# NightShade99/Self-Supervised-Vision

Hardware: AMD Instinct MI355X
Metric: images/sec (whole node) SimCLR ResNet-50 two-view train step (higher is better)
Workload: dtype f32; 1 GPU; SimCLR resnet50 (7x7/2 stem) synthetic 3x224x224, bs=512/GPU, global batch 512, NT-Xent(normalize, T=0.5) over the global batch, SGD-Nesterov; per_gpu_batch=512, global_batch=512, params=27971008, parallelism=single, view_streams=2, library=self-supervised-vision_amd/csrc/libssv_hip.so

## Files before the change

self-supervised-vision_amd/_lib.py:

```python
import ctypes as C
import os

import torch

_HERE = os.path.dirname(os.path.abspath(__file__))
LIB_PATH = os.environ.get("SSV_HIP_LIB") or os.path.join(_HERE, "csrc", "libssv_hip.so")

ABI_VERSION = 124
PROF_CLASSES = ("conv_fwd", "conv_dgrad", "conv_wgrad", "bn_fwd", "bn_bwd", "pool", "loss", "optim", "aug", "misc", "attn", "norm")


class SsvError(RuntimeError):
    pass


ARITH_F32_MFMA, ARITH_BF16X3 = 0, 6
BLUR_MAX_PIXELS, BLUR_MAX_SIGMA = 81920, 1000.0
KMEANS_MAX_K, KMEANS_MAX_D = 4096, 8192
KNN_MAX_K, KNN_MAX_D, KNN_MAX_CLASSES, KNN_MAX_TOPN = 1024, 8192, 4096, 8
NN_LOOKUP_MAX_M, NN_LOOKUP_FUSED_MAX_D, NN_LOOKUP_SLICE, NN_LOOKUP_MAX_SLICES = 8192, 1024, 512, 4096
WHITEN_MAX_D, WHITEN_MAX_W, WMSE_PERM_MAX_N, WMSE_PERM_MAX_VIEWS, WMSE_PERM_MAX_ITERS = 128, 1024, 4096, 8, 16
PROTO_NCE_MAX_M, PROTO_NCE_MAX_SEGS, PROTO_NCE_FUSED_MAX_D, PROTO_NCE_SLICE, PROTO_NCE_MAX_SLICES = 8192, 8, 128, 256, 32
DENSE_MATCH_MAX_S, DENSE_MATCH_MAX_C = 256, 8192
QUEUE_NCE_MAX_M, QUEUE_NCE_FUSED_MAX_D, QUEUE_NCE_SLICE, QUEUE_NCE_MAX_SLICES, QUEUE_NCE_TARGET_WGS = 131072, 128, 256, 32, 256
VICREG_MAX_D = KNN_MAX_D


class ConvDesc(C.Structure):
    _fields_ = [(n, C.c_int32) for n in ("N", "H", "W", "C", "K", "R", "S", "stride", "pad", "Ho", "Wo", "arithmetic", "reserved")] + [("w_planes", C.c_void_p)]


class BnGate(C.Structure):
    _fields_ = [(n, C.c_void_p) for n in ("x", "scale", "shift", "mask", "mean", "invstd", "psum_g", "psum_gx", "x2", "mean2", "invstd2", "psum_gx2")]


class BnDyin(C.Structure):
    _fields_ = [(n, C.c_void_p) for n in ("x", "coef")]


class AugCfg(C.Structure):
    _fields_ = [(n, C.c_double) for n in ("brightness", "contrast", "saturation", "hue", "p_jitter", "p_gray", "p_flip",
                                          "scale_min", "scale_max", "ratio_min", "ratio_max")]


_vp, _i32, _i64, _f32, _sz = C.c_void_p, C.c_int32, C.c_int64, C.c_float, C.c_size_t
_u64 = C.c_uint64
_f3 = C.POINTER(C.c_float)
_cd = C.POINTER(ConvDesc)

SIGNATURES = {
    "ssv_version": (C.c_int, []),
    "ssv_last_error": (C.c_char_p, []),
    "ssv_source_sha16": (C.c_char_p, []),
    "ssv_device_cus": (C.c_int, []),
    "ssv_conv2d_fwd": (C.c_int, [_cd, _vp, _vp, _vp, _vp, _vp, _vp]),
    "ssv_pad_channels": (C.c_int, [_i64, _i32, _i32, _vp, _vp, _i32, _vp]),
    "ssv_group_expand": (C.c_int, [_i32, _i32, _i32, _i32, _i32, _vp, _vp, _vp]),
    "ssv_group_extract": (C.c_int, [_i32, _i32, _i32, _i32, _i32, _vp, _vp, _i32, _vp]),
    "ssv_conv2d_fwd_stats_groups": (_i64, [_cd]),
    "ssv_conv2d_fwd_stats": (C.c_int, [_cd, _vp, _vp, _vp, _vp, _vp, _vp]),
    "ssv_conv2d_fwd_bnrelu_in_stats": (C.c_int, [_cd, _vp, _vp, _vp, _vp, _vp, _vp, _vp, _vp]),
    "ssv_conv2d_fwd_sumin_stats": (C.c_int, [_cd] + [_vp] * 13),
    "ssv_conv2d_wgrad_bnrelu_in": (C.c_int, [_cd, _vp, _vp, _vp, _vp, _vp, C.c_int, _vp, _sz, _vp]),
    "ssv_bn_stats_finalize": (C.c_int, [_i64, _i32, _vp, _vp, _i32, _vp, _vp, _f32, _f32, _vp, _vp, _vp, _vp, _vp, _vp, _vp, _vp, _sz, _vp]),
    "ssv_bn_apply": (C.c_int, [_i64, _i32, _vp, _vp, _vp, _vp, _vp, _vp, C.c_int, _vp, _vp, _vp]),
    "ssv_bn_relu_bwd_affine": (C.c_int, [_i64, _i32, _vp, _vp, _vp, _vp, _vp, _vp, _vp, _vp, _vp, _vp, C.c_int, _vp, _sz, _vp]),
    "ssv_bn_train_fwd_partials": (C.c_int, [_i64, _i32, _vp, _vp, _vp, _i32, _vp, _vp, _vp, C.c_int, _f32, _f32, _vp, _vp, _vp, _vp, _vp, _vp, _vp, _vp, _sz, _vp]),
    "ssv_filter_transpose": (C.c_int, [_i32, _i32, _i32, _i32, _vp, _vp, _vp]),
    "ssv_conv2d_dgrad": (C.c_int, [_cd, _vp, _vp, _vp, _vp, _vp]),
    "ssv_conv2d_fwd_gate_groups": (_i64, [_cd]),
    "ssv_conv2d_fwd_gated": (C.c_int, [_cd, _vp, _vp, _vp, _vp, C.POINTER(BnGate), _vp]),
    "ssv_conv2d_fwd_gated_s2add": (C.c_int, [_cd, _vp, _vp, _vp, _i32, _i32, _vp, C.POINTER(BnGate), _vp]),
    "ssv_conv2d_fwd_dyin_s2add": (C.c_int, [_cd, _vp, C.POINTER(BnDyin), _vp, _vp, _i32, _i32, _vp, C.POINTER(BnGate), _vp]),
    "ssv_conv2d_dgrad_gate_groups": (_i64, [_cd]),
    "ssv_conv2d_dgrad_gated": (C.c_int, [_cd, _vp, _vp, _vp, _vp, C.POINTER(BnGate), _vp]),
    "ssv_bn_bwd_from_partials": (C.c_int, [_i64, _i32, _vp, _vp, _vp, _vp, _vp, _vp, _vp, _i64, _vp, _vp, _vp, C.c_int, _vp, _sz, _vp]),
    "ssv_bn_bwd_coef": (C.c_int, [_i64, _i32, _vp, _vp, _vp, _vp, _vp, _i64, _vp, _vp, _vp, C.c_int, _vp, _sz, _vp]),
    "ssv_conv2d_fwd_dyin": (C.c_int, [_cd, _vp, C.POINTER(BnDyin), _vp, _vp, _vp, C.POINTER(BnGate), _vp]),
    "ssv_conv2d_wgrad_dyin": (C.c_int, [_cd, _vp, _vp, _vp, _vp, C.POINTER(BnDyin), _vp, C.c_int, _vp, _sz, _vp]),
    "ssv_conv2d_wgrad_workspace_bytes": (_sz, [_cd]),
    "ssv_conv2d_fwd_grouped": (C.c_int, [_cd, _i32, _vp, _vp, _vp, _vp, _vp, _vp]),
    "ssv_conv2d_dgrad_grouped": (C.c_int, [_cd, _i32, _vp, _vp, _vp, _vp, _vp]),
    "ssv_conv2d_wgrad_grouped_workspace_bytes": (_sz, [_cd, _i32]),
    "ssv_conv2d_wgrad_grouped": (C.c_int, [_cd, _i32, _vp, _vp, _vp, C.c_int, _vp, _sz, _vp]),
    "ssv_conv2d_wgrad": (C.c_int, [_cd, _vp, _vp, _vp, C.c_int, _vp, _sz, _vp]),
    "ssv_conv2d_wgrad_bias_workspace_bytes": (_sz, [_cd]),
    "ssv_conv2d_wgrad_bias": (C.c_int, [_cd, _vp, _vp, _vp, _vp, C.c_int, _vp, _sz, _vp]),
    "ssv_stem_conv_fwd": (C.c_int, [_cd, _vp, _vp, _vp, _vp, _vp, _vp]),
    "ssv_stem_conv_fwd_stats_rows_per_group": (_i64, [_cd]),
    "ssv_stem_conv_wgrad_rows_per_group": (_i64, [_cd]),
    "ssv_stem_conv_wgrad_workspace_bytes": (_sz, [_cd]),
    "ssv_stem_conv_wgrad": (C.c_int, [_cd, _vp, _vp, _vp, _vp, _sz, _vp]),
    "ssv_wino_tiles": (_i64, [_i32, _i32, _i32]),
    "ssv_wino_groups": (_i64, [_i32, _i32, _i32]),
    "ssv_wino_stats_rows_per_group": (_i32, [_i32, _i32, _i32]),
    "ssv_wino_filter_transform": (C.c_int, [_i32, _i32, _vp, _vp, _vp]),
    "ssv_wino_filter_grad": (C.c_int, [_i32, _i32, _vp, _vp, C.c_int, _vp]),
    "ssv_wino_input_transform": (C.c_int, [_i32, _i32, _i32, _i32, _vp, _vp, _vp, _vp, _vp]),
    "ssv_wino_dy_transform": (C.c_int, [_i32, _i32, _i32, _i32, _vp, _vp, _vp]),
    "ssv_wino_output_transform": (C.c_int, [_i32, _i32, _i32, _i32, _vp, _vp, _vp, _vp, C.POINTER(BnGate), _vp]),
    "ssv_wino44_tiles": (_i64, [_i32, _i32, _i32]),
    "ssv_wino44_groups": (_i64, [_i32, _i32, _i32, _i32]),
    "ssv_wino44_stats_rows_per_group": (_i64, [_i32, _i32, _i32]),
    "ssv_wino44_filter_transform": (C.c_int, [_i32, _i32, _vp, _vp, _vp]),
    "ssv_wino44_input_transform": (C.c_int, [_i32, _i32, _i32, _i32, _vp, _vp, _vp, _vp, _vp, _vp]),
    "ssv_wino44_output_transform": (C.c_int, [_i32, _i32, _i32, _i32, _vp, _vp, _vp, _vp, C.POINTER(BnGate), _vp]),
    "ssv_wino44_dy_transform": (C.c_int, [_i32, _i32, _i32, _i32, _vp, _vp, _vp]),
    "ssv_wino44_filter_grad": (C.c_int, [_i32, _i32, _vp, _vp, C.c_int, _vp]),
    "ssv_wino44_dy_transform_both": (C.c_int, [_i32, _i32, _i32, _i32, _vp, C.POINTER(BnDyin), _vp, _vp, _vp]),
    "ssv_gemm_batched": (C.c_int, [_i32, _i64, _i32, _i32, _vp, _vp, _vp, _vp]),
    "ssv_gemm_batched_split": (C.c_int, [_i32, _i64, _i32, _i32, _vp, _vp, _vp, _vp, _vp, _vp]),
    "ssv_gemm_batched_wgrad_split": (C.c_int, [_i32, _i64, _i32, _i32, _vp, _vp, _vp, _i32, _i32, _vp, _sz, _vp]),
    "ssv_split_planes": (C.c_int, [_i64, _vp, _vp, _vp]),
    "ssv_conv_arithmetic": (C.c_int, [_cd, _i32]),
    "ssv_gemm_batched_wgrad_workspace_bytes": (_sz, [_i32, _i64, _i32, _i32]),
    "ssv_gemm_batched_wgrad": (C.c_int, [_i32, _i64, _i32, _i32, _vp, _vp, _vp, _vp, _sz, _vp]),
    "ssv_gemm_batched_wgrad_blocked_workspace_bytes": (_sz, [_i32, _i64, _i32, _i32, _i32]),
    "ssv_gemm_batched_wgrad_blocked": (C.c_int, [_i32, _i64, _i32, _i32, _vp, _vp, _vp, _i32, _i32, _vp, _sz, _vp]),
    "ssv_bn_workspace_bytes": (_sz, [_i64, _i32]),
    "ssv_bn_train_fwd": (C.c_int, [_i64, _i32, _vp, _vp, _vp, _vp, C.c_int, _f32, _f32, _vp, _vp, _vp, _vp, _vp, _vp, _vp, _vp, _sz, _vp]),
    "ssv_bn_train_bwd": (C.c_int, [_i64, _i32, _vp, _vp, _vp, _vp, _vp, _vp, _vp, C.c_int, _vp, _vp, _vp, _vp, C.c_int, _vp, _sz, _vp]),
    "ssv_bn_relu_maxpool_fwd": (C.c_int, [_i32, _i32, _i32, _i32, _vp, _vp, _vp, _vp, _vp, _vp, _vp]),
    "ssv_bn_relu_maxpool_bwd": (C.c_int, [_i32, _i32, _i32, _i32, _vp, _vp, _vp, _vp, _vp, _vp, _vp, _vp, _vp, _vp, _vp, _vp, C.c_int, _vp, _sz, _vp]),
    "ssv_colsum": (C.c_int, [_i64, _i32, _vp, _vp, C.c_int, _vp, _sz, _vp]),
    "ssv_maxpool3x3s2_fwd": (C.c_int, [_i32, _i32, _i32, _i32, _vp, _vp, _vp, _vp]),
    "ssv_maxpool3x3s2_bwd": (C.c_int, [_i32, _i32, _i32, _i32, _vp, _vp, _vp, _vp]),
    "ssv_gap_fwd": (C.c_int, [_i32, _i32, _i32, _vp, _vp, _vp]),
    "ssv_gap_bwd": (C.c_int, [_i32, _i32, _i32, _vp, _vp, _vp]),
    "ssv_nchw_to_nhwc": (C.c_int, [_i32, _i32, _i32, _i32, _vp, _vp, _vp]),
    "ssv_nhwc_to_nchw": (C.c_int, [_i32, _i32, _i32, _i32, _vp, _vp, _vp]),
    "ssv_l2norm_fwd": (C.c_int, [_i32, _i32, _vp, _i32, _f32, _vp, _i32, _vp, _vp]),
    "ssv_l2norm_bwd": (C.c_int, [_i32, _i32, _vp, _i32, _vp, _vp, _i32, _i32, _vp, _vp]),
    "ssv_ntxent_fwd": (C.c_int, [_i32, _i32, _i32, _i32, _vp, _f32, _vp, _vp, _vp]),
    "ssv_ntxent_loss": (C.c_int, [_i32, _vp, _vp, _f32, _vp, _vp]),
    "ssv_ntxent_bwd": (C.c_int, [_i32, _i32, _i32, _i32, _vp, _vp, _f32, _f32, _vp, _vp]),
    "ssv_ntxent_default_splits": (_i64, [_i32, _i32]),
    "ssv_ntxent_split_workspace_bytes": (_sz, [_i32, _i32, _i32]),
    "ssv_ntxent_fwd_split": (C.c_int, [_i32, _i32, _i32, _i32, _vp, _f32, _vp, _vp, _i32, _vp, _sz, _vp]),
    "ssv_ntxent_bwd_split": (C.c_int, [_i32, _i32, _i32, _i32, _vp, _vp, _f32, _f32, _vp, _i32, _vp, _sz, _vp]),
    "ssv_ntxent_gram_fwd": (C.c_int, [_i32, _i32, _i32, _i32, _vp, _f32, _vp, _vp, _vp]),
    "ssv_ntxent_gram_weights": (C.c_int, [_i32, _i32, _i32, _i32, _vp, _vp, _f32, _f32, _vp]),
    "ssv_reduce_workspace_bytes": (_sz, [_i64]),
    "ssv_mse_pair_fwd_bwd": (C.c_int, [_i64, _vp, _vp, _vp, _vp, _f32, _vp, _vp, _vp, _vp, _sz, _vp]),
    "ssv_scale": (C.c_int, [_i64, _vp, _vp, _vp]),
    "ssv_barlow_cgrad": (C.c_int, [_i32, _vp, _f32, _f32, _vp, _vp, _vp, _sz, _vp]),
    "ssv_vicreg_workspace_bytes": (_sz, [_i32, _i32]),
    "ssv_vicreg_prep": (C.c_int, [_i32, _i32, _vp, _vp, _f32, _f32, _f32, _f32, _vp, _vp, _vp, _vp, _vp, _sz, _vp]),
    "ssv_vicreg_cgrad": (C.c_int, [_i32, _i32, _vp, _f32, _vp, _vp, _vp, _sz, _vp]),
    "ssv_sgd_nesterov": (C.c_int, [_i64, _vp, _vp, _vp, _vp, _f32, _f32, _f32, C.c_int, _vp]),
    "ssv_sgd_nesterov_dev": (C.c_int, [_i64, _vp, _vp, _vp, _vp, _vp, _vp]),
    "ssv_lars_chunk_floats": (_i64, []),
    "ssv_lars_plan_chunks": (_i64, [_i32, _vp]),
    "ssv_lars_plan_bytes": (_sz, [_i32, _vp]),
    "ssv_lars_plan_build": (C.c_int, [_i32, _vp, _vp, _vp, _vp, _vp, _sz]),
    "ssv_lars_workspace_bytes": (_sz, [_i64]),
    "ssv_lars_step": (C.c_int, [_i64, _i32, _i64, _vp, _vp, _vp, _vp, _vp, _vp, _vp, _vp, _sz, _vp]),
    "ssv_ema": (C.c_int, [_i64, _vp, _vp, _f32, _vp]),
    "ssv_fill": (C.c_int, [_i64, _vp, _f32, _vp]),
    "ssv_add": (C.c_int, [_i64, _vp, _vp, _vp]),
    "ssv_augment_params": (C.c_int, [_i32, _i32, _i32, _i32, C.POINTER(AugCfg), _u64, _u64, _vp, _i64, _vp, _vp]),
    "ssv_augment_workspace_bytes": (_sz, [_i32, _i32, _i32, _i32]),
    "ssv_augment_views": (C.c_int, [_i32, _i32, _i32, _i32, _i32, _i32, _vp, _vp, _vp, _f3, _f3, _vp, _vp, _sz, _vp]),
    "ssv_augment_params_blur": (C.c_int, [_i32, _i32, _i32, _i32, C.POINTER(AugCfg), _u64, _u64, _vp, _i64, C.c_double, C.c_double, C.c_double, _vp, _vp]),
    "ssv_augment_blur_workspace_bytes": (_sz, [_i32, _i32, _i32, _i32]),
    "ssv_augment_views_blur": (C.c_int, [_i32, _i32, _i32, _i32, _i32, _i32, _vp, _vp, _vp, _f3, _f3, _vp, _vp, _sz, _vp]),
    "ssv_blur_scalars": (C.c_int, [_i64, _vp, _vp, _vp]),
    "ssv_center_view": (C.c_int, [_i32, _i32, _i32, _i32, _i32, _vp, _vp, _f3, _f3, _vp, _vp]),
    "ssv_knn_workspace_bytes": (_sz, [_i64]),
    "ssv_knn_label_agreement": (C.c_int, [_i64, _i32, _vp, _vp, _i32, _vp, _vp, _sz, _vp]),
    "ssv_knn_workspace_bytes_arith": (_sz, [_i64, _i32, _i32]),
    "ssv_knn_label_agreement_arith": (C.c_int, [_i64, _i32, _vp, _vp, _i32, _vp, _i32, _vp, _sz, _vp]),
    "ssv_kmeans_prep_bytes": (_sz, [_i32, _i32]),
    "ssv_kmeans_workspace_bytes": (_sz, [_i64, _i32, _i32, _i32]),
    "ssv_kmeans_assign": (C.c_int, [_i64, _i32, _i32, _vp, _vp, _vp, _i32, _vp, _vp, _vp, _vp, _i32, _vp, _sz, _vp]),
    "ssv_kmeans_update": (C.c_int, [_i64, _i32, _i32, _vp, _vp, _vp, _vp, _vp, _i32, _vp, _sz, _vp]),
    "ssv_cluster_votes": (C.c_int, [_i64, _vp, _vp, _i32, _i32, _vp, _vp, _vp]),
    "ssv_knn_search_workspace_bytes": (_sz, [_i64, _i64, _i32, _i32, _i32, _i32, _i32]),
    "ssv_knn_search": (C.c_int, [_i64, _i64, _i32, _i32, _vp, _vp, _vp, _vp, _i32, _i32, _i32, _vp, _sz, _vp]),
    "ssv_knn_vote": (C.c_int, [_i64, _i32, _i64, _i32, _i32, _vp, _vp, _vp, _f32, _vp, _vp, _vp, _vp]),
    "ssv_nn_lookup_workspace_bytes": (_sz, [_i32, _i64, _i32, _i32]),
    "ssv_nn_lookup": (C.c_int, [_i32, _i64, _i32, _vp, _vp, _f32, _vp, _vp, _vp, _i32, _vp, _sz, _vp]),
    "ssv_whiten_workspace_bytes": (_sz, [_i32, _i32, _i32]),
    "ssv_whiten_fwd": (C.c_int, [_i32, _i32, _i32, _i64, _vp, _vp, _f32, _vp, _vp, _vp, _vp, _vp, _sz, _vp]),
    "ssv_whiten_bwd": (C.c_int, [_i32, _i32, _i32, _i64, _vp, _vp, _f32, _vp, _vp, _vp, _vp, _vp, _sz, _vp]),
    "ssv_wmse_perm": (C.c_int, [_i32, _i32, _i32, _u64, _u64, _vp, _vp, _vp]),
    "ssv_proto_nce_workspace_bytes": (_sz, [_i32, _i64, _i32, _i32, _i32]),
    "ssv_proto_nce": (C.c_int, [_i32, _i32, _i32, C.POINTER(C.c_int64), _vp, _vp, _vp, _vp, _vp, _vp, _vp, _vp, _i32, _vp, _sz, _vp]),
    "ssv_dense_match": (C.c_int, [_i32, _i32, _i32, _vp, _vp, _f32, _vp, _vp, _i32, _vp]),
    "ssv_queue_nce_workspace_bytes": (_sz, [_i32, _i64, _i32, _i32]),
    "ssv_queue_nce": (C.c_int, [_i32, _i32, _i64, _i64, _vp, _vp, _vp, _vp, _f32, _vp, _vp, _vp, _vp, _i32, _vp, _sz, _vp]),
    "ssv_vit_embed_fwd": (C.c_int, [_i32, _i32, _i32, _i32, _i32, _vp, _vp, _vp, _vp, _vp]),
    "ssv_vit_embed_bwd": (C.c_int, [_i32, _i32, _i32, _i32, _vp, _vp, _vp, _i32, _vp]),
    "ssv_layernorm_fwd": (C.c_int, [_i64, _i32, _vp, _vp, _vp, _vp, _f32, _vp, _vp, _vp, _vp]),
    "ssv_layernorm_workspace_bytes": (_sz, [_i64, _i32]),
    "ssv_layernorm_bwd": (C.c_int, [_i64, _i32, _vp, _vp, _vp, _vp, _vp, _vp, _vp, _vp, _vp, _i32, _vp, _sz, _vp]),
    "ssv_linear_gelu_fwd": (C.c_int, [_cd, _vp, _vp, _vp, _vp, _vp, _vp]),
    "ssv_conv2d_dgrad_gelu": (C.c_int, [_cd, _vp, _vp, _vp, _vp, _vp, _vp]),
    "ssv_linear_fwd_gelugrad": (C.c_int, [_cd, _vp, _vp, _vp, _vp, _vp, _vp]),
    "ssv_linear_gelu_fwd_dact": (C.c_int, [_cd, _vp, _vp, _vp, _vp, _vp, _vp]),
    "ssv_linear_fwd_mulgrad": (C.c_int, [_cd, _vp, _vp, _vp, _vp, _vp, _vp]),
    "ssv_gelu_fwd": (C.c_int, [_i64, _vp, _vp, _vp]),
    "ssv_gelu_bwd": (C.c_int, [_i64, _vp, _vp, _vp, _vp]),
    "ssv_attention_fwd": (C.c_int, [_i32, _i32, _i32, _i32, _vp, _vp, _vp, _i32, _f32, _vp, _i32, _vp, _vp]),
    "ssv_attention_fwd_arith": (C.c_int, [_i32, _i32, _i32, _i32, _vp, _vp, _vp, _i32, _f32, _vp, _i32, _vp, _i32, _vp]),
    "ssv_attention_bwd": (C.c_int, [_i32, _i32, _i32, _i32, _vp, _vp, _vp, _i32, _f32, _vp, _vp, _i32, _vp, _vp, _vp, _vp, _vp, _i32, _vp]),
    "ssv_weightnorm_fwd": (C.c_int, [_i32, _i32, _vp, _vp, _vp, _vp, _vp]),
    "ssv_weightnorm_bwd": (C.c_int, [_i32, _i32, _vp, _vp, _vp, _vp, _vp, _vp, _i32, _vp]),
    "ssv_dino_loss_workspace_bytes": (_sz, [_i32, _i32, _i32]),
    "ssv_dino_loss": (C.c_int, [_i32, _i32, _i32, _vp, _vp, _vp, _f32, _f32, _f32, _vp, _i32, _vp, _vp, _sz, _vp]),
    "ssv_dino_center_update": (C.c_int, [_i32, _i32, _vp, _i32, _vp, _f32, _vp, _vp]),
    "ssv_adamw": (C.c_int, [_i64, _vp, _vp, _vp, _vp, _vp, _f32, _f32, _f32, _f32, _f32, _i64, _f32, _vp]),
    "ssv_adamw_counted": (C.c_int, [_i64, _vp, _vp, _vp, _vp, _vp, _f32, _f32, _f32, _f32, _f32, _vp, _vp, _f32, _vp]),
    "ssv_adamw_counted_dev": (C.c_int, [_i64, _vp, _vp, _vp, _vp, _vp, _f32, _f32, _f32, _vp, _vp, _f32, _vp]),
    "ssv_multicrop_params": (C.c_int, [_i32, _i32, _i32, _i32, _i32, C.c_double, C.c_double, C.c_uint64, C.c_uint64, _vp, _i64, _vp, _vp]),
    "ssv_multicrop": (C.c_int, [_i32, _i32, _i32, _vp, _i32, _vp, _i32, _i32, _vp, _vp]),
    "ssv_negdot_pair_fwd_bwd": (C.c_int, [_i64, _vp, _vp, _vp, _vp, _f32, _vp, _vp, _vp, _vp, _sz, _vp]),
    "ssv_relic_kl_workspace_bytes": (_sz, [_i32]),
    "ssv_relic_kl_fwd_bwd": (C.c_int, [_i32, _i32, _vp, _vp, _vp, _f32, _f32, _vp, _i32, _vp, _vp, _vp, _vp, _sz, _vp]),
    "ssv_moco_loss_fwd_bwd": (C.c_int, [_i32, _i32, _i32, _i32, _vp, _vp, _vp, _f32, _vp, _vp, _vp, _sz, _vp]),
    "ssv_queue_push": (C.c_int, [_i32, _i32, _vp, _i32, _i32, _vp, _f32, _vp]),
    "ssv_queue_push_counted": (C.c_int, [_i32, _i32, _vp, _vp, _i32, _vp, _f32, _vp]),
    "ssv_pirl_default_splits": (_i64, [_i32, _i32]),
    "ssv_pirl_loss_workspace_bytes": (_sz, [_i32, _i32]),
    "ssv_pirl_loss_fwd_bwd": (C.c_int, [_i64, _i32, _i32, _i32, _vp, _vp, _vp, _vp, _vp, _i32, _f32, _f32, _i32, _vp, _vp, _vp, _vp, _sz, _vp]),
    "ssv_bank_momentum_update": (C.c_int, [_i64, _i32, _vp, _i32, _vp, _vp, _f32, _f32, _vp]),
    "ssv_patch_split": (C.c_int, [_i32, _i32, _i32, _i32, _i32, _vp, _vp, _vp]),
    "ssv_softmax_ce_workspace_bytes": (_sz, [_i32]),
    "ssv_softmax_ce_fwd_bwd": (C.c_int, [_i32, _i32, _i32, _vp, _vp, _vp, _vp, _vp, _sz, _vp]),
    "ssv_sgd": (C.c_int, [_i64, _vp, _vp, _vp, _f32, _f32, _f32, C.c_int, C.c_int, _vp]),
    "ssv_prof_enable": (C.c_int, [C.c_int]),
    "ssv_prof_reset": (C.c_int, []),
    "ssv_prof_collect": (C.c_int, [C.POINTER(C.c_double), C.POINTER(C.c_int64)]),
}

_lib = None


def load():
    global _lib
    if _lib is not None:
        return _lib
    if not os.path.exists(LIB_PATH):
        raise SsvError(f"{LIB_PATH} not found: build it with `python -c 'import __graft_entry__ as g; g.build()'` "
                       f"(or `make -C {os.path.dirname(LIB_PATH)}`); there is no CPU fallback")
    lib = C.CDLL(LIB_PATH)
    for name, (res, args) in SIGNATURES.items():
        fn = getattr(lib, name)
        fn.restype, fn.argtypes = res, args
    if lib.ssv_version() < ABI_VERSION:
        raise SsvError(f"{LIB_PATH} is ABI version {lib.ssv_version()}, this package binds version {ABI_VERSION}: rebuild it (make -C {os.path.dirname(LIB_PATH)})")
    _lib = lib
    return lib


def source_sha16():
    return load().ssv_source_sha16().decode()


def lib_sha16(path=None):
    import hashlib
    h = hashlib.sha256()
    with open(path or LIB_PATH, "rb") as fh:
        for chunk in iter(lambda: fh.read(1 << 20), b""):
            h.update(chunk)
    return h.hexdigest()[:16]


def _check(rc, what):
    if rc != 0:
        raise SsvError(f"{what} failed ({rc}): {load().ssv_last_error().decode()}")


def ptr(t):
    return 0 if t is None else t.data_ptr()


_raw_stream = getattr(torch._C, "_cuda_getCurrentRawStream", None)
_raw_device = getattr(torch._C, "_cuda_getDevice", None)


def stream():
    if _raw_stream is not None and _raw_device is not None:
        return _raw_stream(_raw_device())
    return torch.cuda.current_stream().cuda_stream


def _dev(*ts):
    for t in ts:
        if t is not None and not t.is_cuda:
            raise SsvError("libssv_hip operates on device tensors only (got a CPU tensor); there is no CPU fallback")


def call(name, *args):
    _check(getattr(load(), name)(*args), name)


class _Workspace:

    def __init__(self):
        self.buf = {}

    def get(self, nbytes, device):
        key = (device, (_raw_stream(device.index if device.index is not None else _raw_device()) if _raw_stream is not None else torch.cuda.current_stream(device).cuda_stream)
               if device.type == "cuda" else 0)
        b = self.buf.get(key)
        if b is None or b.numel() < nbytes:
            b = torch.empty(max(int(nbytes), 1 << 20), dtype=torch.uint8, device=device)
            self.buf[key] = b
        return b


workspace = _Workspace()


def prof_enable(on=True):
    call("ssv_prof_enable", int(bool(on)))


def prof_reset():
    call("ssv_prof_reset")


def prof_collect():
    ms = (C.c_double * len(PROF_CLASSES))()
    n = (C.c_int64 * len(PROF_CLASSES))()
    call("ssv_prof_collect", ms, n)
    return {k: (ms[i], n[i]) for i, k in enumerate(PROF_CLASSES)}
```

self-supervised-vision_amd/csrc/conv_mfma.hip:

```cpp
#include "common.h"
#include "split_bf16.h"
#include <string.h>
#include <type_traits>

namespace {

constexpr int GBK = 16;

__device__ __forceinline__ int xcd_remap(int orig, int nwg) {
  const int q = nwg >> 3, r = nwg & 7, xcd = orig & 7;
  return (xcd < r ? xcd * (q + 1) : r * (q + 1) + (xcd - r) * q) + (orig >> 3);
}

struct ConvKP {
  int N, H, W, C, K, R, S, stride, pad, Ho, Wo;
  int M;
  int RSC;
  FastDiv dHoWo, dWo, dC, dS, dWp;
  float* aux_out;
  float* aux_out2;
  const float* aux_in;
  const float* xf_scale;
  const float* xf_shift;
  ssv_bn_gate gate;
  const float* dyin_x;
  const float* dyin_coef;
  const float* sum_res; const float* sum_scale; const float* sum_shift; const float* sum_rscale; const float* sum_rshift;
  float* sum_out; uint8_t* sum_mask;
  long long bs_a, bs_b, bs_o;
  int add_H2, add_W2;
  int Cg, Kg;
  const unsigned short* w_planes;
  long long wp_stride;
};

__device__ __forceinline__ void group_span(int n0, int n1, int og, int ig, int bk, int ctot, int& lo, int& hi) {
  const int glo = n0 / og, ghi = (n1 - 1) / og;
  lo = glo * ig / bk * bk;
  hi = min(ctot, ((ghi + 1) * ig + bk - 1) / bk * bk);
}

constexpr int XF_MAXC = 1024;

__device__ __forceinline__ float gelu_f(float v) { return ssv_gelu(v); }
__device__ __forceinline__ float gelu_grad_f(float v) { return ssv_gelu_grad(v); }

using rsrc_t = __amdgpu_buffer_rsrc_t;
constexpr int OOB_OFF = (int)0x80000000u;
__device__ __forceinline__ rsrc_t make_rsrc(const void* base, unsigned bytes) {
  return __builtin_amdgcn_make_buffer_rsrc((void*)base, 0, bytes, 0x00020000);
}
__device__ __forceinline__ f32x4 bload4(rsrc_t rs, int voff_bytes, int soff_bytes) {
  typedef unsigned int u32x4_ __attribute__((ext_vector_type(4)));
  return __builtin_bit_cast(f32x4, (u32x4_)__builtin_amdgcn_raw_buffer_load_b128(rs, voff_bytes, soff_bytes, 0));
}

__device__ __forceinline__ int straddle_off(int off, int bytes, int& rot) {
  rot = 0;
  if (off == OOB_OFF) return OOB_OFF;
  if (off <= -16 || off >= bytes) return OOB_OFF;
  const int c = off < 0 ? 0 : (off > bytes - 16 ? bytes - 16 : off);
  rot = (off - c) >> 2;
  return c;
}
__device__ __forceinline__ f32x4 straddle_fix(f32x4 v, int rot) {
  f32x4 o;
#pragma unroll
  for (int e = 0; e < 4; ++e) {
    const int sidx = e + rot;
    float t = 0.f;
#pragma unroll
    for (int q = 0; q < 4; ++q) t = sidx == q ? v[q] : t;
    o[e] = t;
  }
  return o;
}

template <int TM, int TN, bool A_ROWK, bool B_ROWK, int LDA, int LDB, int BK>
__device__ __forceinline__ void mma_ktile(const float* __restrict__ As, const float* __restrict__ Bs,
                                          int wr0, int wc0, int lane, f32x16 (&acc)[TM][TN]) {
  const int l31 = lane & 31, h = lane >> 5;
#pragma unroll
  for (int ks = 0; ks < BK / 8; ++ks) {
    float a[TM][4], b[TN][4];
#pragma unroll
    for (int tm = 0; tm < TM; ++tm) {
      if constexpr (A_ROWK) {
        const f32x4 v = *reinterpret_cast<const f32x4*>(&As[(wr0 + tm * 32 + l31) * LDA + ks * 8 + 4 * h]);
        a[tm][0] = v[0]; a[tm][1] = v[1]; a[tm][2] = v[2]; a[tm][3] = v[3];
      } else {
#pragma unroll
        for (int t = 0; t < 4; ++t) a[tm][t] = As[(ks * 8 + 4 * h + t) * LDA + wr0 + tm * 32 + l31];
      }
    }
#pragma unroll
    for (int tn = 0; tn < TN; ++tn) {
      if constexpr (B_ROWK) {
        const f32x4 v = *reinterpret_cast<const f32x4*>(&Bs[(wc0 + tn * 32 + l31) * LDB + ks * 8 + 4 * h]);
        b[tn][0] = v[0]; b[tn][1] = v[1]; b[tn][2] = v[2]; b[tn][3] = v[3];
      } else {
#pragma unroll
        for (int t = 0; t < 4; ++t) b[tn][t] = Bs[(ks * 8 + 4 * h + t) * LDB + wc0 + tn * 32 + l31];
      }
    }
#pragma unroll
    for (int t = 0; t < 4; ++t)
#pragma unroll
      for (int tm = 0; tm < TM; ++tm)
#pragma unroll
        for (int tn = 0; tn < TN; ++tn)
          acc[tm][tn] = __builtin_amdgcn_mfma_f32_32x32x2f32(a[tm][t], b[tn][t], acc[tm][tn], 0, 0, 0);
  }
}

template <int TM, int TN>
__device__ __forceinline__ void zero_acc(f32x16 (&acc)[TM][TN]) {
#pragma unroll
  for (int i = 0; i < TM; ++i)
#pragma unroll
    for (int j = 0; j < TN; ++j)
#pragma unroll
      for (int r = 0; r < 16; ++r) acc[i][j][r] = 0.f;
}

template <int TM, int TN> struct Frags { float a[TM][4], b[TN][4]; };

template <int TM, int TN, bool A_ROWK, bool B_ROWK, int LDA, int LDB>
__device__ __forceinline__ void load_frags(Frags<TM, TN>& f, const float* __restrict__ As, const float* __restrict__ Bs,
                                           int wr0, int wc0, int lane, int ks) {
  const int l31 = lane & 31, h = lane >> 5;
#pragma unroll
  for (int tm = 0; tm < TM; ++tm) {
    if constexpr (A_ROWK) {
      const f32x4 v = *reinterpret_cast<const f32x4*>(&As[(wr0 + tm * 32 + l31) * LDA + ks * 8 + 4 * h]);
      f.a[tm][0] = v[0]; f.a[tm][1] = v[1]; f.a[tm][2] = v[2]; f.a[tm][3] = v[3];
    } else {
#pragma unroll
      for (int t = 0; t < 4; ++t) f.a[tm][t] = As[(ks * 8 + 4 * h + t) * LDA + wr0 + tm * 32 + l31];
    }
  }
#pragma unroll
  for (int tn = 0; tn < TN; ++tn) {
    if constexpr (B_ROWK) {
      const f32x4 v = *reinterpret_cast<const f32x4*>(&Bs[(wc0 + tn * 32 + l31) * LDB + ks * 8 + 4 * h]);
      f.b[tn][0] = v[0]; f.b[tn][1] = v[1]; f.b[tn][2] = v[2]; f.b[tn][3] = v[3];
    } else {
#pragma unroll
      for (int t = 0; t < 4; ++t) f.b[tn][t] = Bs[(ks * 8 + 4 * h + t) * LDB + wc0 + tn * 32 + l31];
    }
  }
}

template <int TM, int TN>
__device__ __forceinline__ void mma_frags(const Frags<TM, TN>& f, f32x16 (&acc)[TM][TN]) {
#pragma unroll
  for (int t = 0; t < 4; ++t)
#pragma unroll
    for (int tm = 0; tm < TM; ++tm)
#pragma unroll
      for (int tn = 0; tn < TN; ++tn)
        acc[tm][tn] = __builtin_amdgcn_mfma_f32_32x32x2f32(f.a[tm][t], f.b[tn][t], acc[tm][tn], 0, 0, 0);
}

#define SSV_INTERLEAVE(NMFMA, NMEM, MASK)                                            \
  do {                                                                               \
    _Pragma("unroll") for (int i_ = 0; i_ < (NMEM) && i_ < (NMFMA); ++i_) {         \
      __builtin_amdgcn_sched_group_barrier(0x8, 1, 0);                               \
      __builtin_amdgcn_sched_group_barrier((MASK), 1, 0);                            \
    }                                                                                \
    if ((NMFMA) > (NMEM)) __builtin_amdgcn_sched_group_barrier(0x8, (NMFMA) - (NMEM), 0); \
  } while (0)

struct NoXform { __device__ __forceinline__ void operator()() const {} };
template <int TM, int TN, bool A_ROWK, bool B_ROWK, int LDA, int LDB, int BK, int NLD, int FLUSH = 0, class LoadTile, class StoreTile, class Xform = NoXform>
__device__ __forceinline__ void k_loop(int nkt, const float* As, const float* Bs, int wr0, int wc0, int lane,
                                       f32x16 (&acc)[TM][TN], LoadTile&& load_tile, StoreTile&& store_tile, Xform&& xform_tile = NoXform()) {
  if (nkt <= 0) return;
  f32x16 hi[FLUSH > 0 ? TM : 1][FLUSH > 0 ? TN : 1];
  if constexpr (FLUSH > 0) zero_acc<TM, TN>(hi);
  constexpr int NS = BK / 8;
  constexpr int NM = 4 * TM * TN;
  load_tile();
  xform_tile();
  store_tile();
  __syncthreads();
  Frags<TM, TN> fr;
  for (int kt = 0; kt < nkt; ++kt) {
    __builtin_amdgcn_sched_barrier(0);
    load_frags<TM, TN, A_ROWK, B_ROWK, LDA, LDB>(fr, As, Bs, wr0, wc0, lane, 0);
    load_tile();
    mma_frags<TM, TN>(fr, acc);
    if (NLD > 0) {
      __builtin_amdgcn_sched_group_barrier(0x100, A_ROWK && B_ROWK ? TM + TN : (A_ROWK ? TM + 4 * TN : 4 * (TM + TN)), 0);
      SSV_INTERLEAVE(NM, NLD, 0x20);
    }
    __builtin_amdgcn_sched_barrier(0);
#pragma unroll
    for (int ks = 1; ks < NS; ++ks) {
      load_frags<TM, TN, A_ROWK, B_ROWK, LDA, LDB>(fr, As, Bs, wr0, wc0, lane, ks);
      mma_frags<TM, TN>(fr, acc);
    }
    if constexpr (FLUSH > 0) {
      if ((kt + 1) % FLUSH == 0) {
#pragma unroll
        for (int tm = 0; tm < TM; ++tm)
#pragma unroll
          for (int tn = 0; tn < TN; ++tn) {
            hi[tm][tn] += acc[tm][tn];
#pragma unroll
            for (int j = 0; j < 16; ++j) acc[tm][tn][j] = 0.f;
          }
      }
    }
    __syncthreads();
    if (kt + 1 < nkt) { xform_tile(); store_tile(); __syncthreads(); }
  }
  if constexpr (FLUSH > 0) {
#pragma unroll
    for (int tm = 0; tm < TM; ++tm)
#pragma unroll
      for (int tn = 0; tn < TN; ++tn) acc[tm][tn] = hi[tm][tn] + acc[tm][tn];
  }
}

template <int TM16, int TN16, bool KROWA, bool KROWB, int RBA, int RBB, int FLUSH = 0, int JSPLIT = 1, bool DUAL = false, class LoadTile, class StoreTile, class Xform = NoXform>
__device__ __forceinline__ void k_loop_split(int nkt, const unsigned char* As, int a_plane, const unsigned char* Bs, int b_plane, int wr0, int wc0, int lane,
                                             f32x4 (&acc)[TM16][TN16], LoadTile&& load_tile, StoreTile&& store_tile, Xform&& xform_tile = NoXform()) {
  if (nkt <= 0) return;
  f32x4 hi[FLUSH > 0 ? TM16 : 1][FLUSH > 0 ? TN16 : 1];
  if constexpr (FLUSH > 0) {
#pragma unroll
    for (int i = 0; i < TM16; ++i)
#pragma unroll
      for (int j = 0; j < TN16; ++j) hi[i][j] = f32x4{0.f, 0.f, 0.f, 0.f};
  }
  f32x4 lo[DUAL ? TM16 : 1][DUAL ? TN16 : 1];
  if constexpr (DUAL) {
#pragma unroll
    for (int i = 0; i < TM16; ++i)
#pragma unroll
      for (int j = 0; j < TN16; ++j) lo[i][j] = f32x4{0.f, 0.f, 0.f, 0.f};
  }
  load_tile();
  xform_tile();
  store_tile();
  __syncthreads();
  for (int kt = 0; kt < nkt; ++kt) {
    load_tile();
    constexpr int TJ = TN16 / JSPLIT;
    static_assert(TN16 % JSPLIT == 0, "column tiles per group");
#pragma unroll
    for (int jg = 0; jg < JSPLIT; ++jg) {
      bf16x8 fb[TJ][3];
#pragma unroll
      for (int j = 0; j < TJ; ++j)
#pragma unroll
        for (int q = 0; q < 3; ++q) {
          if constexpr (KROWB) fb[j][q] = splitbf::krow_frag<RBB>(Bs + q * b_plane, wc0 + 16 * (jg * TJ + j), lane);
          else fb[j][q] = splitbf::rowk_frag(Bs + q * b_plane, wc0 + 16 * (jg * TJ + j), lane);
        }
#pragma unroll
      for (int i = 0; i < TM16; ++i) {
        bf16x8 fa[3];
#pragma unroll
        for (int q = 0; q < 3; ++q) {
          if constexpr (KROWA) fa[q] = splitbf::krow_frag<RBA>(As + q * a_plane, wr0 + 16 * i, lane);
          else fa[q] = splitbf::rowk_frag(As + q * a_plane, wr0 + 16 * i, lane);
        }
#pragma unroll
        for (int j = 0; j < TJ; ++j) {
          if constexpr (DUAL) splitbf::mma6x2(acc[i][jg * TJ + j], lo[i][jg * TJ + j], fb[j], fa);
          else splitbf::mma6(acc[i][jg * TJ + j], fb[j], fa);
        }
      }
    }
    if constexpr (FLUSH > 0) {
      if ((kt + 1) % FLUSH == 0) {
#pragma unroll
        for (int i = 0; i < TM16; ++i)
#pragma unroll
          for (int j = 0; j < TN16; ++j) { hi[i][j] += acc[i][j]; acc[i][j] = f32x4{0.f, 0.f, 0.f, 0.f}; }
      }
    }
    __syncthreads();
    if (kt + 1 < nkt) { xform_tile(); store_tile(); __syncthreads(); }
  }
#pragma unroll
  for (int i = 0; i < TM16; ++i)
#pragma unroll
    for (int j = 0; j < TN16; ++j) {
      if constexpr (FLUSH > 0) acc[i][j] = hi[i][j] + acc[i][j];
      if constexpr (DUAL) acc[i][j] += lo[i][j];
    }
}

__device__ __forceinline__ void bstore4(rsrc_t rs, int voff_bytes, f32x4 v) {
  typedef unsigned int u32x4_ __attribute__((ext_vector_type(4)));
  __builtin_amdgcn_raw_buffer_store_b128(__builtin_bit_cast(u32x4_, v), rs, voff_bytes, 0, 0);
}

struct SameOff {};
template <int TM, int TN>
__device__ __forceinline__ void stage_slab(const f32x16 (&acc)[TM][TN], float* __restrict__ ep, int tm, int lane) {
  constexpr int LDE = TN * 32 + 4;
  const int l31 = lane & 31, h = lane >> 5;
#pragma unroll
  for (int tn = 0; tn < TN; ++tn)
#pragma unroll
    for (int j = 0; j < 16; ++j) ep[((j & 3) + 8 * (j >> 2) + 4 * h) * LDE + tn * 32 + l31] = acc[tm][tn][j];
}
template <int TM, int TN>
__device__ __forceinline__ void stage_slab(const f32x4 (&acc)[2 * TM][2 * TN], float* __restrict__ ep, int tm, int lane) {
  constexpr int LDE = TN * 32 + 4;
  const int fr = lane & 15, kg = lane >> 4;
#pragma unroll
  for (int ii = 0; ii < 2; ++ii)
#pragma unroll
    for (int jj = 0; jj < 2 * TN; ++jj) *reinterpret_cast<f32x4*>(&ep[(16 * ii + fr) * LDE + 16 * jj + 4 * kg]) = acc[2 * tm + ii][jj];
}
template <bool SP, class A, class B> __device__ __forceinline__ auto& sel_acc(A& a, B& b) { if constexpr (SP) return b; else return a; }

template <int TM, int TN, int EPI = 0, bool STATS = false, int GATE = 0, class Acc, class RowOff, class AddOff = SameOff>
__device__ __forceinline__ void epilogue_vec(const Acc& acc, float* __restrict__ ep, int lane, int col0, int ncols,
                                             const float* __restrict__ bias, const float* addend, float* out, long long out_elems, RowOff&& row_off,
                                             float* out_act = nullptr, const float* gate = nullptr,
                                             float* pmean = nullptr, float* pm2 = nullptr, int group_rows = 0,
                                             const ssv_bn_gate* bn = nullptr, long long group = 0, AddOff add_off = AddOff(), long long add_elems = 0) {
  constexpr int LDE = TN * 32 + 4, C4 = TN * 8, RPI = 64 / C4, NP = 32 / RPI;
  constexpr bool GMASK = GATE >= 2, GX2 = GATE == 3;
  constexpr int HB0 = GATE == 1 ? 2 : 4;
  constexpr int HB = NP < HB0 ? NP : HB0;
  const int r_in = lane / C4, c4 = lane % C4;
  const int gcol = col0 + c4 * 4;
  const bool cok = gcol < ncols && r_in < RPI;
  const unsigned bytes = (unsigned)(out_elems * 4);
  const rsrc_t r_out = make_rsrc(out, bytes);
  f32x4 b4 = {0.f, 0.f, 0.f, 0.f};
  f32x4 st_p = {0.f, 0.f, 0.f, 0.f}, st_s1 = {0.f, 0.f, 0.f, 0.f}, st_s2 = {0.f, 0.f, 0.f, 0.f};
  f32x4 g_mu = {0.f, 0.f, 0.f, 0.f}, g_is = {0.f, 0.f, 0.f, 0.f}, g_sc = {0.f, 0.f, 0.f, 0.f}, g_sh = {0.f, 0.f, 0.f, 0.f};
  f32x4 g_mu2 = {0.f, 0.f, 0.f, 0.f}, g_is2 = {0.f, 0.f, 0.f, 0.f}, st_s3 = {0.f, 0.f, 0.f, 0.f};
  if constexpr (GATE != 0) {
    if (cok) {
      g_mu = *reinterpret_cast<const f32x4*>(bn->mean + gcol); g_is = *reinterpret_cast<const f32x4*>(bn->invstd + gcol);
      if constexpr (GATE == 1) { g_sc = *reinterpret_cast<const f32x4*>(bn->scale + gcol); g_sh = *reinterpret_cast<const f32x4*>(bn->shift + gcol); }
      if constexpr (GX2) { g_mu2 = *reinterpret_cast<const f32x4*>(bn->mean2 + gcol); g_is2 = *reinterpret_cast<const f32x4*>(bn->invstd2 + gcol); }
    }
  }
  if (bias && cok) b4 = *reinterpret_cast<const f32x4*>(bias + gcol);

  const bool ADD = addend != nullptr;
  auto rows = [&](auto add_tag) {
    constexpr int ADDM = decltype(add_tag)::value;
    constexpr bool ADD_SAME = std::is_same<AddOff, SameOff>::value;
    const rsrc_t r_add = make_rsrc(ADD ? addend : out, ADD_SAME ? bytes : (unsigned)(add_elems * 4));
    const rsrc_t r_gx = make_rsrc(GATE != 0 ? bn->x : out, bytes);
    const rsrc_t r_gm = make_rsrc(GMASK ? reinterpret_cast<const float*>(bn->mask) : out, bytes / 16);
    const rsrc_t r_gx2 = make_rsrc(GX2 ? bn->x2 : out, bytes);
    const rsrc_t r_gate = make_rsrc((EPI == 2 || EPI == 5) ? gate : out, bytes);
    const rsrc_t r_act = make_rsrc((EPI == 1 || EPI == 4) ? out_act : out, bytes);
#pragma unroll
    for (int tm = 0; tm < TM; ++tm) {
      stage_slab<TM, TN>(acc, ep, tm, lane);
      if constexpr (STATS) { if (tm == 0) st_p = *reinterpret_cast<const f32x4*>(&ep[c4 * 4]); }
      constexpr int HP = HB;
      constexpr int NSTEP = NP / HP;
      int voff[1][HP];
      f32x4 av[1][HP], xv[1][HP], gv[1][HP], xv2[1][GX2 ? HP : 1];
      unsigned mb[1][HP];
      auto issue = [&](int st, int sl) {
#pragma unroll
        for (int i = 0; i < HP; ++i) {
          const long long off = row_off(tm * 32 + (st * HP + i) * RPI + r_in);
          voff[sl][i] = (off >= 0 && cok) ? (int)(off + gcol) * 4 : OOB_OFF;
          int aoff = voff[sl][i];
          if constexpr (!ADD_SAME) {
            const long long ao = add_off(tm * 32 + (st * HP + i) * RPI + r_in);
            aoff = (ao >= 0 && voff[sl][i] != OOB_OFF) ? (int)(ao + gcol) * 4 : OOB_OFF;
          }
          if constexpr (ADDM == 2) { if (ADD) av[sl][i] = bload4(r_add, aoff, 0); else av[sl][i] = f32x4{0.f, 0.f, 0.f, 0.f}; }
          else if constexpr (ADDM == 1) av[sl][i] = bload4(r_add, aoff, 0);
          else av[sl][i] = f32x4{0.f, 0.f, 0.f, 0.f};
          if constexpr (EPI == 2 || EPI == 5) gv[sl][i] = bload4(r_gate, voff[sl][i], 0);
          if constexpr (GATE != 0) xv[sl][i] = bload4(r_gx, voff[sl][i], 0);
          if constexpr (GMASK) mb[sl][i] = __builtin_amdgcn_raw_buffer_load_b8(r_gm, voff[sl][i] == OOB_OFF ? OOB_OFF : voff[sl][i] >> 4, 0, 0);
          if constexpr (GX2) xv2[sl][i] = bload4(r_gx2, voff[sl][i], 0);
        }
      };
      auto finish = [&](int st, int sl) {
#pragma unroll
        for (int i = 0; i < HP; ++i) {
          const int r = (st * HP + i) * RPI + r_in;
          f32x4 v = *reinterpret_cast<const f32x4*>(&ep[r * LDE + c4 * 4]);
          const bool ok = voff[sl][i] != OOB_OFF;
          if constexpr (STATS) {
            f32x4 dv = v - st_p;
            dv[0] = ok ? dv[0] : 0.f; dv[1] = ok ? dv[1] : 0.f; dv[2] = ok ? dv[2] : 0.f; dv[3] = ok ? dv[3] : 0.f;
            st_s1 += dv; st_s2 += dv * dv;
          }
          v += b4;
          if constexpr (EPI == 2) {
#pragma unroll
            for (int e = 0; e < 4; ++e) v[e] *= gelu_grad_f(gv[sl][i][e]);
          }
          if constexpr (EPI == 5) v *= gv[sl][i];
          v += av[sl][i];
          if constexpr (GATE != 0) {
            if constexpr (GATE == 1) {
#pragma unroll
              for (int e = 0; e < 4; ++e) v[e] = __builtin_fmaf(xv[sl][i][e], g_sc[e], g_sh[e]) > 0.f ? v[e] : 0.f;
            } else {
#pragma unroll
              for (int e = 0; e < 4; ++e) v[e] = (mb[sl][i] >> e) & 1u ? v[e] : 0.f;
            }
            f32x4 gvv = v;
            if constexpr (GATE == 1) { gvv[0] = ok ? v[0] : 0.f; gvv[1] = ok ? v[1] : 0.f; gvv[2] = ok ? v[2] : 0.f; gvv[3] = ok ? v[3] : 0.f; }
            st_s1 += gvv;
            st_s2 += gvv * ((xv[sl][i] - g_mu) * g_is);
            if constexpr (GX2) st_s3 += gvv * ((xv2[sl][i] - g_mu2) * g_is2);
          }
          if constexpr (EPI == 3) {
#pragma unroll
            for (int e = 0; e < 4; ++e) v[e] = gelu_f(v[e]);
          }
          if constexpr (EPI == 4) {
            f32x4 a;
#pragma unroll
            for (int e = 0; e < 4; ++e) {
              const float cdf = ssv_norm_cdf(v[e]);
              a[e] = 0.5f * v[e] * (2.f * cdf);
              v[e] = cdf + v[e] * ssv_norm_pdf(v[e]);
            }
            bstore4(r_act, voff[sl][i], a);
          }
          bstore4(r_out, voff[sl][i], v);
          if constexpr (EPI == 1) {
            f32x4 a;
#pragma unroll
            for (int e = 0; e < 4; ++e) a[e] = gelu_f(v[e]);
            bstore4(r_act, voff[sl][i], a);
          }
        }
      };
      {
#pragma unroll
        for (int st = 0; st < NSTEP; ++st) {
          __builtin_amdgcn_sched_barrier(0);
          issue(st, 0);
          finish(st, 0);
        }
      }
    }
  };
  if constexpr (GATE != 0 || EPI == 2 || EPI == 5) rows(std::integral_constant<int, 2>{});
  else if (ADD) rows(std::integral_constant<int, 1>{});
  else rows(std::integral_constant<int, 0>{});

  if constexpr (STATS) {
#pragma unroll
    for (int o = C4; o < 64; o <<= 1) {
#pragma unroll
      for (int e = 0; e < 4; ++e) { st_s1[e] += __shfl_xor(st_s1[e], o, 64); st_s2[e] += __shfl_xor(st_s2[e], o, 64); }
    }
    if (r_in == 0 && cok && group_rows > 0) {
      const float n = (float)group_rows;
      *reinterpret_cast<f32x4*>(pmean + gcol) = st_p + st_s1 / n;
      *reinterpret_cast<f32x4*>(pm2 + gcol) = st_s2 - st_s1 * st_s1 / n;
    }
  }
  if constexpr (GATE != 0) {
#pragma unroll
    for (int o = C4; o < 64; o <<= 1) {
#pragma unroll
      for (int e = 0; e < 4; ++e) {
        st_s1[e] += __shfl_xor(st_s1[e], o, 64); st_s2[e] += __shfl_xor(st_s2[e], o, 64);
        if constexpr (GX2) st_s3[e] += __shfl_xor(st_s3[e], o, 64);
      }
    }
    if (r_in == 0 && cok) {
      *reinterpret_cast<f32x4*>(bn->psum_g + group * ncols + gcol) = st_s1;
      *reinterpret_cast<f32x4*>(bn->psum_gx + group * ncols + gcol) = st_s2;
      if constexpr (GX2) *reinterpret_cast<f32x4*>(bn->psum_gx2 + group * ncols + gcol) = st_s3;
    }
  }
}

template <int BM, int BN, int WGM, int WGN, int BK, bool VEC, int EPI = 0, bool STATS = false, int C4 = 0, bool XF = false, int GATE = 0, int OPM = 0, bool ADDS2 = false, int SP = 0>
__global__ void __launch_bounds__(256, (SP ? (OPM != 0 || GATE == 3 || (SP == 2 && BN == 128))
                                          : (OPM == 2 || GATE == 3 || (OPM == 1 && !(BM == 128 && BN == 128)))) ? 2 : 3)
conv_fwd_k(ConvKP p, const float* __restrict__ x, const float* __restrict__ w, const float* __restrict__ bias,
           const float* addend, float* y) {
  constexpr int TM = BM / WGM / 32, TN = BN / WGN / 32;
  constexpr int LDT = BK + 4;
  constexpr int STAGE = (BM + BN) * LDT;
  static_assert(!XF || (VEC && C4 == 0), "the fused-input variant is the float4 path");
  constexpr bool DYF = OPM == 1, SUM = OPM == 2;
  static_assert(OPM == 0 || (VEC && C4 == 0 && !XF), "the formed-on-load operands are the float4 path");
  constexpr int EP_FLOATS = 4 * 32 * (TN * 32 + 4);
  static_assert(!SP || (VEC && C4 == 0 && BK == 32), "the bf16-piece variants are the float4 path with K-step 32");
  constexpr int SP_FLOATS = (BM + BN) * 48;
  constexpr int SMEM = SP ? (SP_FLOATS > EP_FLOATS ? SP_FLOATS : EP_FLOATS)
                          : ((VEC && (EPI || STATS || GATE != 0 || OPM != 0) && EP_FLOATS > STAGE) ? EP_FLOATS : STAGE);
  __shared__ __attribute__((aligned(16))) float smem[SMEM];
  __shared__ __attribute__((aligned(16))) float xfs[(XF && !SP) ? 2 * XF_MAXC : 4];
  float* As = smem;
  float* Bs = smem + BM * LDT;
  const int tid = threadIdx.x, lane = tid & 63, wave = tid >> 6;
  const int wr0 = (wave / WGN) * (BM / WGM), wc0 = (wave % WGN) * (BN / WGN);
  const int NT = (p.K + BN - 1) / BN;
  const int bid = xcd_remap(blockIdx.x, gridDim.x);
  const int mt = bid / NT, nt = bid - mt * NT;
  const int m0 = mt * BM, n0 = nt * BN;
  x += (size_t)blockIdx.y * p.bs_a; w += (size_t)blockIdx.y * p.bs_b; y += (size_t)blockIdx.y * p.bs_o;
  if (addend) addend += (size_t)blockIdx.y * p.bs_o;

  f32x16 acc[SP ? 1 : TM][SP ? 1 : TN];
  f32x4 acc16[SP ? 2 * TM : 1][SP ? 2 * TN : 1];
  if constexpr (SP) {
#pragma unroll
    for (int i = 0; i < 2 * TM; ++i)
#pragma unroll
      for (int j = 0; j < 2 * TN; ++j) acc16[i][j] = f32x4{0.f, 0.f, 0.f, 0.f};
  } else zero_acc<SP ? 1 : TM, SP ? 1 : TN>(acc);

  if constexpr (VEC && C4 == 2) {
    static_assert(BK == 24 && BM == 256, "one staged output row per thread, six float4 per row");
    constexpr int CHN = BK / 4;
    constexpr int BF = (BN * CHN + 255) / 256;
    const rsrc_t rx = make_rsrc(x, (unsigned)p.N * p.H * p.W * 12u);
    const rsrc_t rw = make_rsrc(w, (unsigned)p.K * p.R * BK * 4u);
    int hi0, rowbase;
    unsigned wmask = 0;
    {
      const int m = m0 + tid;
      const bool ok = m < p.M;
      const uint32_t mm = ok ? (uint32_t)m : 0u;
      const uint32_t n = fdiv(mm, p.dHoWo);
      const uint32_t rem = mm - n * (uint32_t)(p.Ho * p.Wo);
      const uint32_t ho = fdiv(rem, p.dWo);
      const uint32_t wo = rem - ho * (uint32_t)p.Wo;
      hi0 = ok ? (int)ho * p.stride - p.pad : -(1 << 20);
      const int wi0 = (int)wo * p.stride - p.pad;
      rowbase = ok ? (((int)n * p.H + hi0) * p.W + wi0) * 12 : 0;
#pragma unroll
      for (int px = 0; px < 8; ++px) wmask |= (unsigned)((px < p.S) & ((unsigned)(wi0 + px) < (unsigned)p.W)) << px;
    }
    int boff[BF];
#pragma unroll
    for (int i = 0; i < BF; ++i) {
      const int f = tid + 256 * i, kf = f / CHN, ch = f - kf * CHN;
      boff[i] = (f < BN * CHN && n0 + kf < p.K) ? ((n0 + kf) * p.R * BK + ch * 4) * 4 : OOB_OFF;
    }
    int lr = 0;
    f32x4 ra[CHN], rb[BF];
    const int xbytes = p.N * p.H * p.W * 12;
    int rots = 0;
    auto load_tile = [&]() {
      const bool hv = (unsigned)(hi0 + lr) < (unsigned)p.H;
      const int base = rowbase + lr * p.W * 12;
      rots = 0;
#pragma unroll
      for (int j = 0; j < CHN; ++j) {
        int rot;
        ra[j] = bload4(rx, straddle_off((hv && lr < p.R) ? base + j * 16 : OOB_OFF, xbytes, rot), 0);
        rots |= (rot != 0 ? rot + 8 : 0) << (4 * j);
      }
#pragma unroll
      for (int i = 0; i < BF; ++i) rb[i] = bload4(rw, (lr < p.R) ? boff[i] : OOB_OFF, lr * BK * 4);
      lr += 1;
    };
    auto xform_tile = [&]() {
      if (rots != 0) {
#pragma unroll
        for (int j = 0; j < CHN; ++j) { const int q = (rots >> (4 * j)) & 15; if (q) ra[j] = straddle_fix(ra[j], q - 8); }
      }
#pragma unroll
      for (int j = 0; j < CHN; ++j)
#pragma unroll
        for (int e = 0; e < 4; ++e) ra[j][e] = ((wmask >> ((4 * j + e) / 3)) & 1u) ? ra[j][e] : 0.f;
    };
    auto store_tile = [&]() {
#pragma unroll
      for (int j = 0; j < CHN; ++j) *reinterpret_cast<f32x4*>(&As[tid * LDT + 4 * j]) = ra[j];
#pragma unroll
      for (int i = 0; i < BF; ++i) {
        const int f = tid + 256 * i, kf = f / CHN, ch = f - kf * CHN;
        if (f < BN * CHN) *reinterpret_cast<f32x4*>(&Bs[kf * LDT + ch * 4]) = rb[i];
      }
    };
    k_loop<TM, TN, true, true, LDT, LDT, BK, CHN + BF>(p.R, As, Bs, wr0, wc0, lane, acc, load_tile, store_tile, xform_tile);
  } else if constexpr (VEC && C4 == 1) {
    constexpr int CH = BK / 4, RPP = 256 / CH;
    constexpr int AP = BM / RPP, BP = BN / RPP;
    const int tl = tid % CH, rsub = tid / CH;
    const rsrc_t rx = make_rsrc(x, (unsigned)p.N * p.H * p.W * 16u);
    const rsrc_t rw = make_rsrc(w, (unsigned)p.K * p.RSC * 4u);
    int hi0[AP], wi0[AP], aoff[AP];
#pragma unroll
    for (int i = 0; i < AP; ++i) {
      const int m = m0 + rsub + RPP * i;
      const bool ok = m < p.M;
      const uint32_t mm = ok ? (uint32_t)m : 0u;
      const uint32_t n = fdiv(mm, p.dHoWo);
      const uint32_t rem = mm - n * (uint32_t)(p.Ho * p.Wo);
      const uint32_t ho = fdiv(rem, p.dWo);
      const uint32_t wo = rem - ho * (uint32_t)p.Wo;
      hi0[i] = ok ? (int)ho * p.stride - p.pad : -(1 << 20);
      wi0[i] = (int)wo * p.stride - p.pad;
      aoff[i] = (((int)n * p.H + hi0[i]) * p.W + wi0[i]) * 16;
    }
    int boff[BP];
#pragma unroll
    for (int i = 0; i < BP; ++i) {
      const int ko = n0 + rsub + RPP * i;
      boff[i] = ko < p.K ? ko * p.RSC * 4 : OOB_OFF;
    }
    const int ntap = p.R * p.S;
    int lt = tl;
    f32x4 ra[AP], rb[BP];
    auto load_tile = [&]() {
      const bool tv = lt < ntap;
      const int r = (int)fdiv((uint32_t)(tv ? lt : 0), p.dS);
      const int sx = (tv ? lt : 0) - r * p.S;
      const int toff_x = (r * p.W + sx) * 16, toff_w = lt * 16;
#pragma unroll
      for (int i = 0; i < AP; ++i) {
        const bool ok = tv & ((unsigned)(hi0[i] + r) < (unsigned)p.H) & ((unsigned)(wi0[i] + sx) < (unsigned)p.W);
        ra[i] = bload4(rx, ok ? aoff[i] + toff_x : OOB_OFF, 0);
      }
#pragma unroll
      for (int i = 0; i < BP; ++i) rb[i] = bload4(rw, (tv && boff[i] != OOB_OFF) ? boff[i] + toff_w : OOB_OFF, 0);
      lt += CH;
    };
    auto store_tile = [&]() {
#pragma unroll
      for (int i = 0; i < AP; ++i) *reinterpret_cast<f32x4*>(&As[(rsub + RPP * i) * LDT + tl * 4]) = ra[i];
#pragma unroll
      for (int i = 0; i < BP; ++i) *reinterpret_cast<f32x4*>(&Bs[(rsub + RPP * i) * LDT + tl * 4]) = rb[i];
    };
    k_loop<TM, TN, true, true, LDT, LDT, BK, AP + BP>((ntap + CH - 1) / CH, As, Bs, wr0, wc0, lane, acc, load_tile, store_tile);
  } else if constexpr (VEC) {
    constexpr int CH = BK / 4, RPP = 256 / CH;
    constexpr int AP = BM / RPP, BP = BN / RPP;
    const int chunk = (tid % CH) * 4, rsub = tid / CH;
    const rsrc_t rx = make_rsrc(x, (unsigned)p.N * p.H * p.W * p.C * 4u);
    const rsrc_t rw = make_rsrc(w, (unsigned)p.K * p.RSC * 4u);
    int hi0[AP], wi0[AP], aoff[AP];
#pragma unroll
    for (int i = 0; i < AP; ++i) {
      const int m = m0 + rsub + RPP * i;
      const bool ok = m < p.M;
      const uint32_t mm = ok ? (uint32_t)m : 0u;
      const uint32_t n = fdiv(mm, p.dHoWo);
      const uint32_t rem = mm - n * (uint32_t)(p.Ho * p.Wo);
      const uint32_t ho = fdiv(rem, p.dWo);
      const uint32_t wo = rem - ho * (uint32_t)p.Wo;
      hi0[i] = ok ? (int)ho * p.stride - p.pad : -(1 << 20);
      wi0[i] = (int)wo * p.stride - p.pad;
      aoff[i] = ((((int)n * p.H + hi0[i]) * p.W + wi0[i]) * p.C + chunk) * 4;
      if (!ok) aoff[i] = OOB_OFF;
    }
    int boff[BP];
#pragma unroll
    for (int i = 0; i < BP; ++i) {
      const int ko = n0 + rsub + RPP * i;
      boff[i] = ko < p.K ? (ko * p.RSC + chunk) * 4 : OOB_OFF;
    }
    const bool inb = p.pad == 0 && p.R == 1 && p.S == 1;
    int lr = 0, ls = 0, lc0 = 0;
    int ktiles = p.RSC / BK;
    if constexpr (!XF && OPM == 0) {
      if (p.Kg != 0) {
        int c_hi;
        group_span(n0, min(n0 + BN, p.K), p.Kg, p.Cg, BK, p.C, lc0, c_hi);
        ktiles = p.R * p.S * ((c_hi - lc0) / BK);
      }
    }
    f32x4 ra[AP], rb[SP ? 1 : BP];
    f32x4 ra2[OPM ? AP : 1], co[(OPM || (XF && SP)) ? 4 : 1];
    constexpr int BPP = SP ? (BN * 4 + 255) / 256 : 1;
    u32x4 rbp[SP ? 3 : 1][BPP];
    int boffp[BPP], bldsp[BPP];
    const long long wplane = p.wp_stride;
    const rsrc_t rwp = make_rsrc(SP ? (const void*)(p.w_planes + (size_t)blockIdx.y * p.bs_b) : (const void*)w, SP ? (unsigned)((2 * wplane + (long long)p.K * p.RSC) * 2) : 16u);
    if constexpr (SP) {
#pragma unroll
      for (int i = 0; i < BPP; ++i) {
        const int idx = tid + 256 * i, br = idx >> 2, k8 = idx & 3;
        boffp[i] = (idx < BN * 4 && n0 + br < p.K) ? ((n0 + br) * p.RSC + k8 * 8) * 2 : OOB_OFF;
        bldsp[i] = splitbf::rowk_off(br, k8);
      }
    }
    const rsrc_t rxs0 = make_rsrc((XF && SP) ? p.xf_scale : x, (XF && SP) ? (unsigned)p.C * 4u : 16u), rxs1 = make_rsrc((XF && SP) ? p.xf_shift : x, (XF && SP) ? (unsigned)p.C * 4u : 16u);
    const rsrc_t rx2 = make_rsrc(DYF ? p.dyin_x : (SUM ? p.sum_res : x), (unsigned)p.N * p.H * p.W * p.C * 4u);
    const rsrc_t rco = make_rsrc(DYF ? p.dyin_coef : x, DYF ? (unsigned)p.C * 16u : 16u);
    const rsrc_t rs0 = make_rsrc(SUM ? p.sum_scale : x, (unsigned)p.C * 4u), rs1 = make_rsrc(SUM ? p.sum_shift : x, (unsigned)p.C * 4u);
    const bool raff = SUM && p.sum_rscale != nullptr;
    const rsrc_t rs2 = make_rsrc(raff ? p.sum_rscale : x, (unsigned)p.C * 4u), rs3 = make_rsrc(raff ? p.sum_rshift : x, (unsigned)p.C * 4u);
    const rsrc_t rso = make_rsrc(SUM ? p.sum_out : y, (unsigned)p.N * p.H * p.W * p.C * 4u);
    const rsrc_t rsm = make_rsrc(SUM && p.sum_mask ? reinterpret_cast<float*>(p.sum_mask) : y, (unsigned)p.N * p.H * p.W * (p.C / 4));
    int st_off = 0;
    int xf_ok = 0, xf_c = 0;
    if constexpr (XF && !SP) {
      for (int c = tid; c < p.C; c += 256) { xfs[c] = p.xf_scale[c]; xfs[XF_MAXC + c] = p.xf_shift[c]; }
      __syncthreads();
    }
    auto load_tile = [&]() {
      const int toff_x = ((lr * p.W + ls) * p.C + lc0) * 4;
      const int toff_w = ((lr * p.S + ls) * p.C + lc0) * 4;
      if constexpr (XF) { xf_ok = 0; xf_c = lc0 + chunk; }
      if constexpr (XF && SP) { co[0] = bload4(rxs0, chunk * 4, lc0 * 4); co[1] = bload4(rxs1, chunk * 4, lc0 * 4); }
#pragma unroll
      for (int i = 0; i < AP; ++i) {
        const bool ok = inb | (((unsigned)(hi0[i] + lr) < (unsigned)p.H) & ((unsigned)(wi0[i] + ls) < (unsigned)p.W));
        ra[i] = bload4(rx, ok ? aoff[i] + toff_x : OOB_OFF, 0);
        if constexpr (OPM != 0) ra2[i] = bload4(rx2, ok ? aoff[i] + toff_x : OOB_OFF, 0);
        if constexpr (XF) xf_ok |= (int)ok << i;
      }
      if constexpr (DYF) {
#pragma unroll
        for (int j = 0; j < 4; ++j) co[j] = bload4(rco, (j * p.C + chunk) * 4, lc0 * 4);
      }
      if constexpr (SUM) {
        st_off = toff_x;
        co[0] = bload4(rs0, chunk * 4, lc0 * 4); co[1] = bload4(rs1, chunk * 4, lc0 * 4);
        if (raff) { co[2] = bload4(rs2, chunk * 4, lc0 * 4); co[3] = bload4(rs3, chunk * 4, lc0 * 4); }
        else { co[2] = f32x4{1.f, 1.f, 1.f, 1.f}; co[3] = f32x4{0.f, 0.f, 0.f, 0.f}; }
      }
      if constexpr (SP) {
#pragma unroll
        for (int q = 0; q < 3; ++q)
#pragma unroll
          for (int i = 0; i < BPP; ++i)
            rbp[q][i] = (u32x4)__builtin_amdgcn_raw_buffer_load_b128(rwp, boffp[i] == OOB_OFF ? OOB_OFF : boffp[i] + q * (int)(wplane * 2), toff_w >> 1, 0);
      } else {
#pragma unroll
        for (int i = 0; i < BP; ++i) rb[i] = bload4(rw, boff[i], toff_w);
      }
      ls += 1;
      const bool w1 = ls == p.S;
      ls = w1 ? 0 : ls;
      lr += w1 ? 1 : 0;
      const bool w2 = lr == p.R;
      lr = w2 ? 0 : lr;
      lc0 += w2 ? BK : 0;
    };
    auto xform_tile = [&]() {
      if constexpr (XF) {
        f32x4 sc, sh;
        if constexpr (SP) { sc = co[0]; sh = co[1]; }
        else { sc = *reinterpret_cast<const f32x4*>(&xfs[xf_c]); sh = *reinterpret_cast<const f32x4*>(&xfs[XF_MAXC + xf_c]); }
#pragma unroll
        for (int i = 0; i < AP; ++i) {
          const float cap = (inb || ((xf_ok >> i) & 1)) ? __builtin_inff() : 0.f;
#pragma unroll
          for (int e = 0; e < 4; ++e) ra[i][e] = __builtin_amdgcn_fmed3f(__builtin_fmaf(ra[i][e], sc[e], sh[e]), 0.f, cap);
        }
      } else if constexpr (DYF) {
#pragma unroll
        for (int i = 0; i < AP; ++i) {
#pragma unroll
          for (int e = 0; e < 4; ++e) ra[i][e] = __builtin_fmaf(ra[i][e], co[0][e], __builtin_fmaf(ra2[i][e] - co[1][e], co[2][e], co[3][e]));
        }
      } else if constexpr (SUM) {
        const bool wr = nt == 0;
#pragma unroll
        for (int i = 0; i < AP; ++i) {
          f32x4 v;
          unsigned bits = 0;
#pragma unroll
          for (int e = 0; e < 4; ++e) {
            v[e] = __builtin_fmaf(ra[i][e], co[0][e], co[1][e]) + __builtin_fmaf(ra2[i][e], co[2][e], co[3][e]);
            bits |= (v[e] > 0.f ? 1u : 0u) << e;
            v[e] = fmaxf(v[e], 0.f);
          }
          ra[i] = v;
          if (wr) {
            const int off = aoff[i] == OOB_OFF ? OOB_OFF : aoff[i] + st_off;
            bstore4(rso, off, v);
            if (p.sum_mask) __builtin_amdgcn_raw_buffer_store_b8((unsigned char)bits, rsm, off == OOB_OFF ? OOB_OFF : off >> 4, 0, 0);
          }
        }
      }
    };
    constexpr int A_PLANE = BM * splitbf::ROWB, B_PLANE = BN * splitbf::ROWB;
    unsigned char* const Asb = reinterpret_cast<unsigned char*>(smem);
    unsigned char* const Bsb = Asb + 3 * A_PLANE;
    auto store_tile = [&]() {
      if constexpr (SP) {
#pragma unroll
        for (int i = 0; i < AP; ++i) splitbf::rowk_store(Asb, A_PLANE, rsub + RPP * i, tid % CH, ra[i]);
#pragma unroll
        for (int q = 0; q < 3; ++q)
#pragma unroll
          for (int i = 0; i < BPP; ++i)
            if (BN * 4 % 256 == 0 || tid + 256 * i < BN * 4) *reinterpret_cast<u32x4*>(Bsb + q * B_PLANE + bldsp[i]) = rbp[q][i];
        return;
      }
#pragma unroll
      for (int i = 0; i < AP; ++i) *reinterpret_cast<f32x4*>(&As[(rsub + RPP * i) * LDT + chunk]) = ra[i];
#pragma unroll
      for (int i = 0; i < BP; ++i) *reinterpret_cast<f32x4*>(&Bs[(rsub + RPP * i) * LDT + chunk]) = rb[i];
    };
    if constexpr (SP) k_loop_split<2 * TM, 2 * TN, false, false, 128, 128, 0, 1, SP == 2>(ktiles, Asb, A_PLANE, Bsb, B_PLANE, wr0, wc0, lane, acc16, load_tile, store_tile, xform_tile);
    else k_loop<TM, TN, true, true, LDT, LDT, BK, AP + BP + (OPM ? AP + 4 : 0)>(ktiles, As, Bs, wr0, wc0, lane, acc, load_tile, store_tile, xform_tile);
  } else {
    static_assert(BK == GBK, "generic path is BK=16");
    constexpr int AE = BM / 16, BE = BN / 16;
    const int kk = tid & 15, rsub = tid >> 4;
    int hw0[AE];
    int nimg[AE];
#pragma unroll
    for (int i = 0; i < AE; ++i) {
      const int m = m0 + rsub + 16 * i;
      if (m < p.M) {
        const uint32_t n = fdiv((uint32_t)m, p.dHoWo);
        const uint32_t rem = (uint32_t)m - n * (uint32_t)(p.Ho * p.Wo);
        const uint32_t ho = fdiv(rem, p.dWo);
        const uint32_t wo = rem - ho * (uint32_t)p.Wo;
        const int h0 = (int)ho * p.stride - p.pad, w0 = (int)wo * p.stride - p.pad;
        hw0[i] = (h0 & 0xffff) | (w0 << 16);
        nimg[i] = (int)n;
      } else { hw0[i] = 0; nimg[i] = -1; }
    }
    float ra[AE], rb[BE];
    int lk = kk;
    auto load_tile = [&]() {
      const bool kok = lk < p.RSC;
      const uint32_t tap = fdiv((uint32_t)(kok ? lk : 0), p.dC);
      const int c = (kok ? lk : 0) - (int)tap * p.C;
      const uint32_t r = fdiv(tap, p.dS);
      const int s = (int)tap - (int)r * p.S;
#pragma unroll
      for (int i = 0; i < AE; ++i) {
        const int hi = (int)(short)(hw0[i] & 0xffff) + (int)r, wi = (hw0[i] >> 16) + s;
        float v = 0.f;
        if (kok && nimg[i] >= 0 && (unsigned)hi < (unsigned)p.H && (unsigned)wi < (unsigned)p.W)
          v = x[(((size_t)nimg[i] * p.H + hi) * p.W + wi) * p.C + c];
        ra[i] = v;
      }
#pragma unroll
      for (int i = 0; i < BE; ++i) {
        const int ko = n0 + rsub + 16 * i;
        rb[i] = (kok && ko < p.K) ? w[(size_t)ko * p.RSC + lk] : 0.f;
      }
      lk += BK;
    };
    auto store_tile = [&]() {
#pragma unroll
      for (int i = 0; i < AE; ++i) As[(rsub + 16 * i) * LDT + kk] = ra[i];
#pragma unroll
      for (int i = 0; i < BE; ++i) Bs[(rsub + 16 * i) * LDT + kk] = rb[i];
    };
    const int nkt = (p.RSC + BK - 1) / BK;
    load_tile();
    store_tile();
    __syncthreads();
    for (int kt = 0; kt < nkt; ++kt) {
      const bool more = kt + 1 < nkt;
      if (more) load_tile();
      mma_ktile<TM, TN, true, true, LDT, LDT, BK>(As, Bs, wr0, wc0, lane, acc);
      __syncthreads();
      if (more) { store_tile(); __syncthreads(); }
    }
  }

  static_assert(!(EPI || STATS) || (VEC && EP_FLOATS <= SMEM), "the fused-activation / statistics forward needs the vectorised epilogue");
  if constexpr (VEC && EP_FLOATS <= SMEM) {
    if ((p.K & 3) == 0) {
      const int rbase = m0 + wr0;
      if constexpr (STATS) {
        constexpr int GR = TM * 32;
        const int g = rbase / GR;
        const int valid = min(GR, p.M - rbase);
        epilogue_vec<TM, TN, 0, true>(sel_acc<(SP != 0)>(acc, acc16), smem + wave * (32 * (TN * 32 + 4)), lane, n0 + wc0, p.K, bias, addend, y, (long long)p.M * p.K,
                                          [&](int r) -> long long { const int m = rbase + r; return m < p.M ? (long long)m * p.K : -1; },
                                          nullptr, nullptr, p.aux_out + (size_t)g * p.K, p.aux_out2 + (size_t)g * p.K, valid > 0 ? valid : 0);
      } else if constexpr (GATE != 0) {
        static_assert(BM / WGM == 64, "gate partials are per 64 output rows");
        auto row_off = [&](int r) -> long long { const int m = rbase + r; return m < p.M ? (long long)m * p.K : -1; };
        if constexpr (ADDS2) {
          static_assert(GATE != 0, "the compact stride-2 addend rides on the gated epilogues");
          auto add_off = [&](int r) -> long long {
            const int m = rbase + r;
            if (m >= p.M) return -1;
            const uint32_t n = fdiv((uint32_t)m, p.dHoWo);
            const uint32_t rem = (uint32_t)m - n * (uint32_t)(p.Ho * p.Wo);
            const uint32_t ho = fdiv(rem, p.dWo);
            const uint32_t wo = rem - ho * (uint32_t)p.Wo;
            if ((ho | wo) & 1u) return -1;
            return ((long long)((int)n * p.add_H2 + (int)(ho >> 1)) * p.add_W2 + (int)(wo >> 1)) * p.K;
          };
          epilogue_vec<TM, TN, 0, false, GATE>(sel_acc<(SP != 0)>(acc, acc16), smem + wave * (32 * (TN * 32 + 4)), lane, n0 + wc0, p.K, bias, addend, y, (long long)p.M * p.K, row_off,
                                                   nullptr, nullptr, nullptr, nullptr, 0, &p.gate, (long long)(rbase / 64), add_off,
                                                   (long long)p.N * p.add_H2 * p.add_W2 * p.K);
        } else {
          epilogue_vec<TM, TN, 0, false, GATE>(sel_acc<(SP != 0)>(acc, acc16), smem + wave * (32 * (TN * 32 + 4)), lane, n0 + wc0, p.K, bias, addend, y, (long long)p.M * p.K, row_off,
                                                   nullptr, nullptr, nullptr, nullptr, 0, &p.gate, (long long)(rbase / 64));
        }
      } else {
        epilogue_vec<TM, TN, EPI>(sel_acc<(SP != 0)>(acc, acc16), smem + wave * (32 * (TN * 32 + 4)), lane, n0 + wc0, p.K, bias, addend, y, (long long)p.M * p.K,
                                  [&](int r) -> long long { const int m = rbase + r; return m < p.M ? (long long)m * p.K : -1; },
                                  (EPI == 1 || EPI == 4) ? p.aux_out : nullptr, (EPI == 2 || EPI == 5) ? p.aux_in : nullptr);
      }
      return;
    }
  }
  static_assert(GATE == 0 || (VEC && EP_FLOATS <= SMEM), "the gated epilogue is the vectorised one");
  if constexpr (SP) return;
  const int l31 = lane & 31, h = lane >> 5;
#pragma unroll
  for (int tn = 0; tn < TN; ++tn) {
    const int col = n0 + wc0 + tn * 32 + l31;
    if (col >= p.K) continue;
    const float bv = bias ? bias[col] : 0.f;
#pragma unroll
    for (int tm = 0; tm < TM; ++tm) {
#pragma unroll
      for (int j = 0; j < 16; ++j) {
        const int row = m0 + wr0 + tm * 32 + (j & 3) + 8 * (j >> 2) + 4 * h;
        if (row < p.M) {
          const size_t o = (size_t)row * p.K + col;
          float v = acc[tm][tn][j] + bv;
          if (addend) v += addend[o];
          y[o] = v;
        }
      }
    }
  }
}

template <int BM, int BN, int WGM, int WGN, int BK, bool EPI = false, int GATE = 0, bool SP = false>
__global__ void __launch_bounds__(256, SP ? 2 : 3)
conv_dgrad_k(ConvKP p, const float* __restrict__ dy, const float* __restrict__ w, const float* addend, float* dx) {
  constexpr int TM = BM / WGM / 32, TN = BN / WGN / 32;
  constexpr int LDT = BK + 4;
  static_assert(!SP || (BK == 32 && BN == 128), "the bf16-piece data gradient: K-step 32, 128 input channels per tile");
  constexpr int A_FLOATS = BM * LDT, B_FLOATS = BK * BN, STAGE = SP ? 48 * (BM + BN) : A_FLOATS + B_FLOATS;
  __shared__ __attribute__((aligned(16))) float smem[STAGE];
  __shared__ unsigned rowpix[BM];
  __shared__ int taps[64 * 3];
  __shared__ int ntaps_s;
  float* As = smem;
  float* Bs = smem + A_FLOATS;
  const int tid = threadIdx.x, lane = tid & 63, wave = tid >> 6;
  const int wr0 = (wave / WGN) * (BM / WGM), wc0 = (wave % WGN) * (BN / WGN);
  const int st = p.stride;
  const int ph = blockIdx.y / st, pw = blockIdx.y - ph * st;
  const int Hq = ph < p.H ? (p.H - ph + st - 1) / st : 0;
  const int Wq = pw < p.W ? (p.W - pw + st - 1) / st : 0;
  const int Mc = p.N * Hq * Wq;
  const int NT = (p.C + BN - 1) / BN;
  const int bid = xcd_remap(blockIdx.x, gridDim.x);
  const int mt = bid / NT, nt = bid - mt * NT;
  const int m0 = mt * BM, n0 = nt * BN;
  if (m0 >= Mc) {
    if constexpr (GATE != 0) {
      const long long grp = ((long long)blockIdx.y * (gridDim.x / NT) + mt) * (BM / 64) + (wr0 / 64);
      const int col = n0 + wc0 + lane;
      for (int c = col; c < min(n0 + wc0 + BN / WGN, p.C); c += 64) { p.gate.psum_g[grp * p.C + c] = 0.f; p.gate.psum_gx[grp * p.C + c] = 0.f; }
    }
    return;
  }

  if (tid == 0) {
    int n = 0;
    for (int r = 0; r < p.R; ++r) {
      const int dr = ph + p.pad - r;
      if (((dr % st) + st) % st != 0) continue;
      for (int s = 0; s < p.S; ++s) {
        const int ds = pw + p.pad - s;
        if (((ds % st) + st) % st != 0) continue;
        taps[3 * n + 0] = dr >= 0 ? dr / st : -((-dr) / st);
        taps[3 * n + 1] = ds >= 0 ? ds / st : -((-ds) / st);
        taps[3 * n + 2] = (r * p.S + s) * p.C;
        ++n;
      }
    }
    ntaps_s = n;
  }
  for (int r = tid; r < BM; r += 256) {
    const int m = m0 + r;
    unsigned pix = 0xffffffffu;
    if (m < Mc) {
      const int n = m / (Hq * Wq);
      const int rem = m - n * Hq * Wq;
      const int hq = rem / Wq, wq = rem - hq * Wq;
      pix = (unsigned)((n * p.H + hq * st + ph) * p.W + wq * st + pw);
    }
    rowpix[r] = pix;
  }
  __syncthreads();
  const int ntaps = ntaps_s;

  f32x16 acc[SP ? 1 : TM][SP ? 1 : TN];
  f32x4 acc16[SP ? 2 * TM : 1][SP ? 2 * TN : 1];
  if constexpr (SP) {
#pragma unroll
    for (int i = 0; i < 2 * TM; ++i)
#pragma unroll
      for (int j = 0; j < 2 * TN; ++j) acc16[i][j] = f32x4{0.f, 0.f, 0.f, 0.f};
  } else zero_acc<SP ? 1 : TM, SP ? 1 : TN>(acc);

  constexpr int CH = BK / 4, RPP = 256 / CH;
  constexpr int AP = BM / RPP;
  constexpr int BCV = BN / 4;
  constexpr int BRP = 256 / BCV;
  constexpr int BP = BK / BRP;
  const int chunk = (tid % CH) * 4, rsub = tid / CH;
  const rsrc_t rdy = make_rsrc(dy, (unsigned)p.N * p.Ho * p.Wo * p.K * 4u);
  const rsrc_t rw = make_rsrc(w, (unsigned)p.K * p.RSC * 4u);
  int hq_[AP], wq_[AP], aoff[AP];
#pragma unroll
  for (int i = 0; i < AP; ++i) {
    const int m = m0 + rsub + RPP * i;
    const bool ok = m < Mc;
    const int mm = ok ? m : 0;
    const int n = mm / (Hq * Wq);
    const int rem = mm - n * Hq * Wq;
    hq_[i] = ok ? rem / Wq : -(1 << 20);
    wq_[i] = rem - (rem / Wq) * Wq;
    aoff[i] = ok ? (((n * p.Ho + hq_[i]) * p.Wo + wq_[i]) * p.K + chunk) * 4 : OOB_OFF;
  }
  const int bcol = (tid % BCV) * 4, brow = tid / BCV;
  const int boff = n0 + bcol < p.C ? (brow * p.RSC + n0 + bcol) * 4 : OOB_OFF;
  const bool inb = p.pad == 0 && p.R == 1 && p.S == 1;

  int ti = 0, lk0 = 0;
  int kspan = p.K;
  if (p.Cg != 0) {
    int k_hi;
    group_span(n0, min(n0 + BN, p.C), p.Cg, p.Kg, BK, p.K, lk0, k_hi);
    kspan = k_hi - lk0;
  }
  int dho = 0, dwo = 0, tapoff = 0;
  if (ntaps > 0) { dho = taps[0]; dwo = taps[1]; tapoff = taps[2]; }
  f32x4 ra[AP], rb[SP ? 1 : BP];
  constexpr int BPP = SP ? 32 * (BN / 8) / 256 : 1;
  u32x4 rbp[SP ? 3 : 1][BPP];
  int boffp[BPP], bldsp[BPP];
  const rsrc_t rwp = make_rsrc(SP ? (const void*)p.w_planes : (const void*)w, SP ? (unsigned)(3 * p.wp_stride * 2) : 16u);
  if constexpr (SP) {
#pragma unroll
    for (int i = 0; i < BPP; ++i) {
      const int idx = tid + 256 * i, kr = idx / (BN / 8), c8 = idx % (BN / 8);
      boffp[i] = n0 + c8 * 8 < p.C ? (kr * p.RSC + n0 + c8 * 8) * 2 : OOB_OFF;
      bldsp[i] = splitbf::krow_off<BN * 2>(kr, c8);
    }
  }
  auto load_tile = [&]() {
    const int toff_a = ((dho * p.Wo + dwo) * p.K + lk0) * 4;
    const int toff_b = (lk0 * p.RSC + tapoff) * 4;
#pragma unroll
    for (int i = 0; i < AP; ++i) {
      const bool ok = inb | (((unsigned)(hq_[i] + dho) < (unsigned)p.Ho) & ((unsigned)(wq_[i] + dwo) < (unsigned)p.Wo));
      ra[i] = bload4(rdy, ok ? aoff[i] + toff_a : OOB_OFF, 0);
    }
    if constexpr (SP) {
#pragma unroll
      for (int q = 0; q < 3; ++q)
#pragma unroll
        for (int i = 0; i < BPP; ++i)
          rbp[q][i] = (u32x4)__builtin_amdgcn_raw_buffer_load_b128(rwp, boffp[i] == OOB_OFF ? OOB_OFF : boffp[i] + q * (int)(p.wp_stride * 2), toff_b >> 1, 0);
    } else {
#pragma unroll
      for (int i = 0; i < BP; ++i) rb[i] = bload4(rw, boff + BRP * i * p.RSC * 4, toff_b);
    }
    ti += 1;
    const bool w1 = ti >= ntaps;
    ti = w1 ? 0 : ti;
    lk0 += w1 ? BK : 0;
    dho = taps[3 * ti]; dwo = taps[3 * ti + 1]; tapoff = taps[3 * ti + 2];
  };
  constexpr int A_PLANE = BM * splitbf::ROWB, B_PLANE = 32 * BN * 2;
  unsigned char* const Asb = reinterpret_cast<unsigned char*>(smem);
  unsigned char* const Bsb = Asb + 3 * A_PLANE;
  auto store_tile = [&]() {
    if constexpr (SP) {
#pragma unroll
      for (int i = 0; i < AP; ++i) splitbf::rowk_store(Asb, A_PLANE, rsub + RPP * i, tid % CH, ra[i]);
#pragma unroll
      for (int q = 0; q < 3; ++q)
#pragma unroll
        for (int i = 0; i < BPP; ++i) *reinterpret_cast<u32x4*>(Bsb + q * B_PLANE + bldsp[i]) = rbp[q][i];
      return;
    }
#pragma unroll
    for (int i = 0; i < AP; ++i) *reinterpret_cast<f32x4*>(&As[(rsub + RPP * i) * LDT + chunk]) = ra[i];
#pragma unroll
    for (int i = 0; i < BP; ++i) *reinterpret_cast<f32x4*>(&Bs[(brow + BRP * i) * BN + bcol]) = rb[i];
  };
  if constexpr (SP) k_loop_split<2 * TM, 2 * TN, false, true, 128, BN * 2>(ntaps * (kspan / BK), Asb, A_PLANE, Bsb, B_PLANE, wr0, wc0, lane, acc16, load_tile, store_tile);
  else k_loop<TM, TN, true, false, LDT, BN, BK, AP + BP>(ntaps * (kspan / BK), As, Bs, wr0, wc0, lane, acc, load_tile, store_tile);

  constexpr int EP_FLOATS = 4 * 32 * (TN * 32 + 4);
  static_assert(!EPI || EP_FLOATS <= STAGE, "the fused-activation dgrad needs the vectorised epilogue");
  static_assert(GATE == 0 || (EP_FLOATS <= STAGE && BM / WGM == 64), "the gated epilogue is the vectorised one, partials per 64 rows");
  if constexpr (EP_FLOATS <= STAGE) {
    if constexpr (GATE != 0) {
      const long long grp = ((long long)blockIdx.y * (gridDim.x / NT) + mt) * (BM / 64) + (wr0 / 64);
      epilogue_vec<TM, TN, 0, false, GATE>(sel_acc<SP>(acc, acc16), smem + wave * (32 * (TN * 32 + 4)), lane, n0 + wc0, p.C, nullptr, addend, dx, (long long)p.N * p.H * p.W * p.C,
                                               [&](int r) -> long long { const unsigned pix = rowpix[wr0 + r]; return pix != 0xffffffffu ? (long long)pix * p.C : -1; },
                                               nullptr, nullptr, nullptr, nullptr, 0, &p.gate, grp);
    } else {
      epilogue_vec<TM, TN, EPI ? 2 : 0>(sel_acc<SP>(acc, acc16), smem + wave * (32 * (TN * 32 + 4)), lane, n0 + wc0, p.C, nullptr, addend, dx, (long long)p.N * p.H * p.W * p.C,
                                        [&](int r) -> long long { const unsigned pix = rowpix[wr0 + r]; return pix != 0xffffffffu ? (long long)pix * p.C : -1; },
                                        nullptr, EPI ? p.aux_in : nullptr);
    }
    return;
  }
  if constexpr (SP) return;
  const int l31 = lane & 31, h = lane >> 5;
#pragma unroll
  for (int tn = 0; tn < TN; ++tn) {
    const int col = n0 + wc0 + tn * 32 + l31;
    if (col >= p.C) continue;
#pragma unroll
    for (int tm = 0; tm < TM; ++tm) {
#pragma unroll
      for (int j = 0; j < 16; ++j) {
        const unsigned pix = rowpix[wr0 + tm * 32 + (j & 3) + 8 * (j >> 2) + 4 * h];
        if (pix != 0xffffffffu) {
          const size_t o = (size_t)pix * p.C + col;
          float v = acc[tm][tn][j];
          if (addend) v += addend[o];
          dx[o] = v;
        }
      }
    }
  }
}

template <int BM, int BN, int WGM, int WGN, int BK, bool VECB, int GATHER, bool XF = false, bool DYF = false, bool BIAS = false, int FLUSH = 0, bool SP = false>
__global__ void __launch_bounds__(256, (SP && BM == 128 && BN == 128) ? 2 : 1)
conv_wgrad_k(ConvKP p, const float* __restrict__ x, const float* __restrict__ dy, float* __restrict__ partial, int chunk_rows, int tiles) {
  constexpr int TM = BM / WGM / 32, TN = BN / WGN / 32;
  static_assert(!SP || (VECB && GATHER != 3 && BK == 32), "the bf16-piece variants: float4 gathers, K-step 32");
  constexpr int STAGE = SP ? 48 * (BM + BN) : BK * (BM + BN);
  constexpr int EP_FLOATS = 4 * 32 * (TN * 32 + 4);
  static_assert(!XF || VECB, "the fused-input variant is the float4 path");
  static_assert(!DYF || (VECB && GATHER == 1), "the BatchNorm-backward operand: 1x1 / stride 1 layers");
  __shared__ __attribute__((aligned(16))) float smem[STAGE > EP_FLOATS ? STAGE : EP_FLOATS];
  float* As = smem;
  float* Bs = smem + BK * BM;
  const int tid = threadIdx.x, lane = tid & 63, wave = tid >> 6;
  const int wr0 = (wave / WGN) * (BM / WGM), wc0 = (wave % WGN) * (BN / WGN);
  const int NCOL = GATHER == 3 ? p.R * 24 : p.RSC;
  const int JT = (NCOL + BN - 1) / BN;
  const int bid = xcd_remap(blockIdx.x, gridDim.x);
  const int split = bid / tiles, tile = bid - split * tiles;
  const int it = tile / JT, jt = tile - it * JT;
  const int i0 = it * BM, j0 = jt * BN;
  const int ms = split * chunk_rows;
  const int me = min(ms + chunk_rows, p.M);
  x += (size_t)blockIdx.y * p.bs_a; dy += (size_t)blockIdx.y * p.bs_b; partial += (size_t)blockIdx.y * p.bs_o;
  if constexpr (GATHER != 3) {
    if (p.Kg != 0 && j0 / p.C == (min(j0 + BN, NCOL) - 1) / p.C) {
      const int c0 = j0 % p.C, c1 = c0 + min(BN, NCOL - j0);
      if ((min(i0 + BM, p.K) - 1) / p.Kg < c0 / p.Cg || (c1 - 1) / p.Cg < i0 / p.Kg) return;
    }
  }

  f32x16 acc[SP ? 1 : TM][SP ? 1 : TN];
  f32x4 acc16[SP ? 2 * TM : 1][SP ? 2 * TN : 1];
  if constexpr (SP) {
#pragma unroll
    for (int i = 0; i < 2 * TM; ++i)
#pragma unroll
      for (int j = 0; j < 2 * TN; ++j) acc16[i][j] = f32x4{0.f, 0.f, 0.f, 0.f};
  } else zero_acc<SP ? 1 : TM, SP ? 1 : TN>(acc);

  constexpr int ACV = BM / 4, ARP = 256 / ACV, AP = BK / ARP;
  const int acol = (tid % ACV) * 4, arow = tid / ACV;
  const bool acok = i0 + acol < p.K;
  constexpr int BCV = VECB ? BN / 4 : BN, BRP = GATHER == 3 ? 1 : 256 / BCV, BP = GATHER == 3 ? (BK * BCV + 255) / 256 : BK / BRP;
  const int bcol = VECB ? (tid % BCV) * 4 : (tid % BCV), brow = tid / BCV;
  const int j = j0 + bcol;
  const bool jok = j < p.RSC;
  const uint32_t tap = fdiv((uint32_t)(jok ? j : 0), p.dC);
  const int cj = (jok ? j : 0) - (int)tap * p.C;
  const int rj = (int)fdiv(tap, p.dS);
  const int sj = (int)tap - rj * p.S;

  const rsrc_t rdy = make_rsrc(dy, (unsigned)p.M * p.K * 4u);
  const rsrc_t rx = make_rsrc(x, (unsigned)p.N * p.H * p.W * p.C * 4u);
  int mcur = ms;
  f32x4 ra[AP];
  f32x4 bsum = {0.f, 0.f, 0.f, 0.f};
  f32x4 rbv[VECB ? BP : 1];
  float rbs[VECB ? 1 : BP];
  int avoff[AP], bvoff[BP];
  f32x4 ra2[DYF ? AP : 1], dco[DYF ? 4 : 1];
  const rsrc_t rdx = make_rsrc(DYF ? p.dyin_x : dy, (unsigned)p.M * p.K * 4u);
  int a_ok = 0;
  if constexpr (DYF) {
#pragma unroll
    for (int j = 0; j < 4; ++j) dco[j] = acok ? *reinterpret_cast<const f32x4*>(p.dyin_coef + (size_t)j * p.K + i0 + acol) : f32x4{0.f, 0.f, 0.f, 0.f};
  }
  int xf_ok = 0;
  f32x4 xsc = {0.f, 0.f, 0.f, 0.f}, xsh = {0.f, 0.f, 0.f, 0.f};
  if constexpr (XF) { if (jok) { xsc = *reinterpret_cast<const f32x4*>(p.xf_scale + cj); xsh = *reinterpret_cast<const f32x4*>(p.xf_shift + cj); } }
#pragma unroll
  for (int i = 0; i < AP; ++i) avoff[i] = acok ? ((arow + ARP * i) * p.K + i0 + acol) * 4 : OOB_OFF;
#pragma unroll
  for (int i = 0; i < BP; ++i) bvoff[i] = jok ? ((brow + BRP * i) * p.C + cj) * 4 : OOB_OFF;
  int s1_ho[BP], s1_wo[BP], s1_base[BP];
  const int s1_qw = BK / p.Wo, s1_rw = BK - s1_qw * p.Wo;
  if constexpr (GATHER == 2) {
#pragma unroll
    for (int i = 0; i < BP; ++i) {
      const uint32_t mm = (uint32_t)min(ms + brow + BRP * i, p.M - 1);
      const uint32_t n = fdiv(mm, p.dHoWo);
      const uint32_t rem = mm - n * (uint32_t)(p.Ho * p.Wo);
      s1_ho[i] = (int)fdiv(rem, p.dWo);
      s1_wo[i] = (int)rem - s1_ho[i] * p.Wo;
      s1_base[i] = ((brow + BRP * i + (rj - p.pad) * p.W + (sj - p.pad)) * p.C + cj) * 4;
    }
  }
  int rw_row[GATHER == 3 ? BP : 1], rw_r[GATHER == 3 ? BP : 1], rw_e0[GATHER == 3 ? BP : 1];
  unsigned rw_mask[GATHER == 3 ? BP : 1];
  int rw_rot[GATHER == 3 ? BP : 1];
  if constexpr (GATHER == 3) {
#pragma unroll
    for (int i = 0; i < BP; ++i) {
      const int f = tid + 256 * i, col = j0 + (f % BCV) * 4;
      rw_row[i] = f / BCV;
      rw_r[i] = col / 24;
      rw_e0[i] = col - rw_r[i] * 24;
      if (f >= BK * BCV || col >= NCOL) rw_r[i] = -1;
      rw_mask[i] = 0;
      rw_rot[i] = 0;
    }
  }
  auto load_tile = [&]() {
    const int soff_a = mcur * p.K * 4;
#pragma unroll
    for (int i = 0; i < AP; ++i) ra[i] = bload4(rdy, avoff[i], soff_a);
    if constexpr (GATHER == 3) {
#pragma unroll
      for (int i = 0; i < BP; ++i) {
        const int m = mcur + rw_row[i];
        bool ok = rw_r[i] >= 0 && m < p.M;
        const uint32_t mm = ok ? (uint32_t)m : 0u;
        const uint32_t n = fdiv(mm, p.dHoWo);
        const uint32_t rem = mm - n * (uint32_t)(p.Ho * p.Wo);
        const uint32_t ho = fdiv(rem, p.dWo);
        const uint32_t wo = rem - ho * (uint32_t)p.Wo;
        const int hi = (int)ho * p.stride - p.pad + rw_r[i], wi0 = (int)wo * p.stride - p.pad;
        ok = ok & ((unsigned)hi < (unsigned)p.H);
        int rot;
        rbv[i] = bload4(rx, straddle_off(ok ? (((int)n * p.H + hi) * p.W + wi0) * 12 + rw_e0[i] * 4 : OOB_OFF, p.N * p.H * p.W * 12, rot), 0);
        rw_rot[i] = rot;
        unsigned mk = 0;
#pragma unroll
        for (int e = 0; e < 4; ++e) { const int px = (rw_e0[i] + e) / 3; mk |= (unsigned)((px < p.S) & ((unsigned)(wi0 + px) < (unsigned)p.W)) << e; }
        rw_mask[i] = mk;
      }
      mcur += BK;
      return;
    }
    if constexpr (DYF) {
      a_ok = 0;
#pragma unroll
      for (int i = 0; i < AP; ++i) { ra2[i] = bload4(rdx, avoff[i], soff_a); a_ok |= (int)(mcur + arow + ARP * i < p.M) << i; }
    }
    if constexpr (GATHER == 1) {
      const int soff_b = mcur * p.C * 4;
#pragma unroll
      for (int i = 0; i < BP; ++i) {
        if constexpr (VECB) rbv[i] = bload4(rx, bvoff[i], soff_b);
        else rbs[i] = __builtin_bit_cast(float, __builtin_amdgcn_raw_buffer_load_b32(rx, bvoff[i], soff_b, 0));
      }
    } else if constexpr (GATHER == 2) {
      const int moff = mcur * p.C * 4;
      if constexpr (XF) xf_ok = 0;
#pragma unroll
      for (int i = 0; i < BP; ++i) {
        const int m = mcur + brow + BRP * i;
        const bool ok = jok & (m < p.M) & ((unsigned)(s1_ho[i] + rj - p.pad) < (unsigned)p.H) & ((unsigned)(s1_wo[i] + sj - p.pad) < (unsigned)p.W);
        if constexpr (XF) xf_ok |= (int)ok << i;
        const int off = ok ? s1_base[i] + moff : OOB_OFF;
        if constexpr (VECB) rbv[i] = bload4(rx, off, 0);
        else rbs[i] = __builtin_bit_cast(float, __builtin_amdgcn_raw_buffer_load_b32(rx, off, 0, 0));
        int wo = s1_wo[i] + s1_rw;
        const int carry = wo >= p.Wo ? 1 : 0;
        wo -= carry ? p.Wo : 0;
        int ho = s1_ho[i] + s1_qw + carry;
        ho -= ho >= p.Ho ? p.Ho : 0;
        s1_wo[i] = wo; s1_ho[i] = ho;
      }
    } else {
      if constexpr (XF) xf_ok = 0;
#pragma unroll
      for (int i = 0; i < BP; ++i) {
        const int m = mcur + brow + BRP * i;
        bool ok = jok & (m < p.M);
        const uint32_t mm = ok ? (uint32_t)m : 0u;
        const uint32_t n = fdiv(mm, p.dHoWo);
        const uint32_t rem = mm - n * (uint32_t)(p.Ho * p.Wo);
        const uint32_t ho = fdiv(rem, p.dWo);
        const uint32_t wo = rem - ho * (uint32_t)p.Wo;
        const int hi = (int)ho * p.stride - p.pad + rj, wi = (int)wo * p.stride - p.pad + sj;
        ok = ok & ((unsigned)hi < (unsigned)p.H) & ((unsigned)wi < (unsigned)p.W);
        if constexpr (XF) xf_ok |= (int)ok << i;
        const int off = ok ? ((((int)n * p.H + hi) * p.W + wi) * p.C + cj) * 4 : OOB_OFF;
        if constexpr (VECB) rbv[i] = bload4(rx, off, 0);
        else rbs[i] = __builtin_bit_cast(float, __builtin_amdgcn_raw_buffer_load_b32(rx, off, 0, 0));
      }
    }
    mcur += BK;
  };
  auto xform_tile = [&]() {
    if constexpr (GATHER == 3) {
#pragma unroll
      for (int i = 0; i < BP; ++i) {
        if (rw_rot[i] != 0) rbv[i] = straddle_fix(rbv[i], rw_rot[i]);
#pragma unroll
        for (int e = 0; e < 4; ++e) rbv[i][e] = ((rw_mask[i] >> e) & 1u) ? rbv[i][e] : 0.f;
      }
    }
    if constexpr (DYF) {
#pragma unroll
      for (int i = 0; i < AP; ++i) {
        const bool ok = (a_ok >> i) & 1;
#pragma unroll
        for (int e = 0; e < 4; ++e) ra[i][e] = ok ? __builtin_fmaf(ra[i][e], dco[0][e], __builtin_fmaf(ra2[i][e] - dco[1][e], dco[2][e], dco[3][e])) : 0.f;
      }
    }
    if constexpr (XF) {
#pragma unroll
      for (int i = 0; i < BP; ++i) {
        const float cap = (GATHER == 1 || ((xf_ok >> i) & 1)) ? __builtin_inff() : 0.f;
#pragma unroll
        for (int e = 0; e < 4; ++e) rbv[i][e] = __builtin_amdgcn_fmed3f(__builtin_fmaf(rbv[i][e], xsc[e], xsh[e]), 0.f, cap);
      }
    }
  };
  constexpr int A_PLANE = 32 * BM * 2, B_PLANE = 32 * BN * 2;
  unsigned char* const Asb = reinterpret_cast<unsigned char*>(smem);
  unsigned char* const Bsb = Asb + 3 * A_PLANE;
  auto store_tile = [&]() {
#pragma unroll
    for (int i = 0; i < AP; ++i) {
      if constexpr (SP) splitbf::krow_store<BM * 2>(Asb, A_PLANE, arow + ARP * i, acol, ra[i]);
      else *reinterpret_cast<f32x4*>(&As[(arow + ARP * i) * BM + acol]) = ra[i];
    }
    if constexpr (BIAS) {
      if (jt == 0) {
#pragma unroll
        for (int i = 0; i < AP; ++i) bsum += ra[i];
      }
    }
#pragma unroll
    for (int i = 0; i < BP; ++i) {
      if constexpr (GATHER == 3) {
        const int f = tid + 256 * i;
        if (f < BK * BCV) *reinterpret_cast<f32x4*>(&Bs[(f / BCV) * BN + (f % BCV) * 4]) = rbv[i];
      } else if constexpr (SP) splitbf::krow_store<BN * 2>(Bsb, B_PLANE, brow + BRP * i, bcol, rbv[i]);
      else if constexpr (VECB) *reinterpret_cast<f32x4*>(&Bs[(brow + BRP * i) * BN + bcol]) = rbv[i];
      else Bs[(brow + BRP * i) * BN + bcol] = rbs[i];
    }
  };
  if constexpr (SP) k_loop_split<2 * TM, 2 * TN, true, true, BM * 2, BN * 2, FLUSH, 1, true>((me - ms + BK - 1) / BK, Asb, A_PLANE, Bsb, B_PLANE, wr0, wc0, lane, acc16, load_tile, store_tile, xform_tile);
  else k_loop<TM, TN, false, false, BM, BN, BK, (VECB ? AP + BP + (DYF ? AP : 0) : 0), FLUSH>((me - ms + BK - 1) / BK, As, Bs, wr0, wc0, lane, acc, load_tile, store_tile, xform_tile);

  if constexpr (BIAS) {
    static_assert(STAGE >= (256 / (BM / 4)) * BM, "the bias partials are folded through the stage buffer");
    if (jt == 0) {
      __syncthreads();
      *reinterpret_cast<f32x4*>(&smem[arow * BM + acol]) = bsum;
      __syncthreads();
      if (tid < BM && i0 + tid < p.K) {
        float t = 0.f;
#pragma unroll
        for (int r = 0; r < ARP; ++r) t += smem[r * BM + tid];
        p.aux_out[(size_t)split * p.K + i0 + tid] = t;
      }
      __syncthreads();
    }
  }
  float* out = partial + (size_t)split * p.K * NCOL;
  if ((NCOL & 3) == 0) {
    const int rbase = i0 + wr0;
    epilogue_vec<TM, TN>(sel_acc<SP>(acc, acc16), smem + wave * (32 * (TN * 32 + 4)), lane, j0 + wc0, NCOL, nullptr, nullptr, out, (long long)p.K * NCOL,
                         [&](int r) -> long long { const int row = rbase + r; return row < p.K ? (long long)row * NCOL : -1; });
    return;
  }
  if constexpr (SP) return;
  const int l31 = lane & 31, h = lane >> 5;
#pragma unroll
  for (int tn = 0; tn < TN; ++tn) {
    const int col = j0 + wc0 + tn * 32 + l31;
    if (col >= p.RSC) continue;
#pragma unroll
    for (int tm = 0; tm < TM; ++tm) {
#pragma unroll
      for (int jj = 0; jj < 16; ++jj) {
        const int row = i0 + wr0 + tm * 32 + (jj & 3) + 8 * (jj >> 2) + 4 * h;
        if (row < p.K) out[(size_t)row * p.RSC + col] = acc[tm][tn][jj];
      }
    }
  }
}

__global__ void __launch_bounds__(256)
wgrad_reduce_k(const float* __restrict__ partial, int nsplit, int64_t n, float* __restrict__ dw, int accumulate) {
  __shared__ float sm[4][64];
  const int e = threadIdx.x & 63, grp = threadIdx.x >> 6;
  const int64_t i = (int64_t)blockIdx.x * 64 + e;
  partial += (size_t)blockIdx.y * nsplit * n; dw += (size_t)blockIdx.y * n;
  const int per = (nsplit + 3) / 4;
  const int k0 = grp * per, k1 = min(k0 + per, nsplit);
  float s = 0.f;
  if (i < n) {
    int k = k0;
    for (; k + 3 < k1; k += 4) {
      const float a = partial[(size_t)k * n + i], b = partial[(size_t)(k + 1) * n + i];
      const float c = partial[(size_t)(k + 2) * n + i], d = partial[(size_t)(k + 3) * n + i];
      s += (a + b) + (c + d);
    }
    for (; k < k1; ++k) s += partial[(size_t)k * n + i];
  }
  sm[grp][e] = s;
  __syncthreads();
  if (grp == 0 && i < n) dw[i] = (accumulate ? dw[i] : 0.f) + ((sm[0][e] + sm[1][e]) + (sm[2][e] + sm[3][e]));
}

int check_desc(const ssv_conv_desc* d, const char* who) {
  SSV_REQUIRE(d != nullptr, "%s: null descriptor", who);
  SSV_REQUIRE(d->N > 0 && d->H > 0 && d->W > 0 && d->C > 0 && d->K > 0 && d->R > 0 && d->S > 0 && d->stride > 0 && d->pad >= 0,
              "%s: non-positive dimension", who);
  const int Ho = (d->H + 2 * d->pad - d->R) / d->stride + 1, Wo = (d->W + 2 * d->pad - d->S) / d->stride + 1;
  SSV_REQUIRE(Ho == d->Ho && Wo == d->Wo, "%s: Ho/Wo (%d,%d) inconsistent with input/filter/stride/pad (expect %d,%d)", who, d->Ho, d->Wo, Ho, Wo);
  SSV_REQUIRE((int64_t)d->N * d->H * d->W < (1ll << 31) && (int64_t)d->N * d->Ho * d->Wo < (1ll << 31), "%s: too many pixels", who);
  SSV_REQUIRE((int64_t)d->R * d->S * d->C < (1 << 24) && d->R * d->S <= 64 && d->H < 32768 && d->W < 32768, "%s: filter too large", who);
  SSV_REQUIRE((int64_t)d->N * d->H * d->W * d->C < (1ll << 29) - (1 << 22) && (int64_t)d->N * d->Ho * d->Wo * d->K < (1ll << 29) - (1 << 22) &&
              (int64_t)d->K * d->R * d->S * d->C < (1ll << 29), "%s: tensor of 2 GiB or more - split the batch", who);
  return SSV_OK;
}

ConvKP make_kp(const ssv_conv_desc* d) {
  ConvKP p;
  p.N = d->N; p.H = d->H; p.W = d->W; p.C = d->C; p.K = d->K; p.R = d->R; p.S = d->S;
  p.stride = d->stride; p.pad = d->pad; p.Ho = d->Ho; p.Wo = d->Wo;
  p.M = d->N * d->Ho * d->Wo;
  p.RSC = d->R * d->S * d->C;
  p.dHoWo = make_fastdiv((uint32_t)(d->Ho * d->Wo));
  p.dWo = make_fastdiv((uint32_t)d->Wo);
  p.dC = make_fastdiv((uint32_t)d->C);
  p.dS = make_fastdiv((uint32_t)d->S);
  p.dWp = make_fastdiv((uint32_t)d->W + 2u);
  p.aux_out = nullptr; p.aux_out2 = nullptr; p.aux_in = nullptr; p.xf_scale = nullptr; p.xf_shift = nullptr;
  memset(&p.gate, 0, sizeof(p.gate));
  p.dyin_x = nullptr; p.dyin_coef = nullptr;
  p.sum_res = p.sum_scale = p.sum_shift = p.sum_rscale = p.sum_rshift = nullptr; p.sum_out = nullptr; p.sum_mask = nullptr;
  p.bs_a = p.bs_b = p.bs_o = 0;
  p.add_H2 = p.add_W2 = 0;
  p.Cg = p.Kg = 0;
  p.w_planes = (const unsigned short*)d->w_planes;
  p.wp_stride = (long long)d->K * p.RSC;
  return p;
}

struct RowSplit { int nsplit, chunk; };
RowSplit wgrad_row_split(int bm, int64_t tiles, int64_t rows, int max_chunk = 0) {
  const int slots = bm == 128 ? 768 : 1024;
  int64_t ns = slots / tiles;
  const int64_t max_by_rows = cdiv64(rows, 256);
  if (ns > max_by_rows) ns = max_by_rows;
  if (ns < 1) ns = 1;
  int64_t chunk = cdiv64(cdiv64(rows, ns), 32) * 32;
  if (max_chunk > 0 && chunk > max_chunk) {
    const int64_t nb = cdiv64(rows, (int64_t)max_chunk);
    chunk = cdiv64(cdiv64(rows, nb), 32) * 32;
  }
  return {(int)cdiv64(rows, chunk), (int)chunk};
}

struct WgradPlan { int bm, bn, it, jt, nsplit, chunk; };
WgradPlan plan_wgrad(const ssv_conv_desc* d, int groups = 0) {
  WgradPlan w;
  const int RSC = d->R * d->S * d->C;
  const int64_t M = (int64_t)d->N * d->Ho * d->Wo;
  const bool bd = groups > 1 && d->C % 64 == 0;
  w.bm = (d->K >= 128 && !bd) ? 128 : 64;
  w.bn = (RSC <= 64 || bd) ? 64 : 128;
  w.it = cdiv(d->K, w.bm);
  w.jt = cdiv(RSC, w.bn);
  int tiles = w.it * w.jt;
  if (bd) {
    const int cg = d->C / groups, kg = d->K / groups;
    const int per_row = cdiv((cdiv(w.bm, kg) + 1) * cg, w.bn) + 1;
    tiles = w.it * d->R * d->S * (per_row < d->C / w.bn ? per_row : d->C / w.bn);
  }
  const RowSplit rs = wgrad_row_split(w.bm, tiles, M);
  w.chunk = rs.chunk; w.nsplit = rs.nsplit;
  return w;
}

}

namespace {

template <int V> using ic = std::integral_constant<int, V>;
template <int V0, int... Vs, class F>
inline void for_value(int v, F&& f) {
  if constexpr (sizeof...(Vs) == 0) f(ic<V0>{});
  else if (v == V0) f(ic<V0>{});
  else for_value<Vs...>(v, f);
}

inline bool sp_planes_fit(const ssv_conv_desc* d) {
  return (int64_t)d->K * d->R * d->S * d->C * 6 < (1ll << 31);
}
inline bool sp_fwd_ok(const ssv_conv_desc* d) {
  return d->arithmetic == SSV_ARITH_BF16X3 && d->w_planes != nullptr && (((uintptr_t)d->w_planes) & 15) == 0 && d->C % 32 == 0 && d->K % 4 == 0 &&
         sp_planes_fit(d);
}
constexpr int SP_DUAL_FROM = 1152;
inline int sp_fwd_mode(const ssv_conv_desc* d) {
  if (!sp_fwd_ok(d)) return 0;
  return (int64_t)d->R * d->S * d->C > SP_DUAL_FROM ? 2 : 1;
}
inline bool sp_dgrad_ok(const ssv_conv_desc* d) {
  return d->arithmetic == SSV_ARITH_BF16X3 && d->w_planes != nullptr && (((uintptr_t)d->w_planes) & 15) == 0 && d->K % 32 == 0 && d->C >= 128 && d->C % 8 == 0 &&
         sp_planes_fit(d);
}
inline bool sp_wgrad_ok(const ssv_conv_desc* d) {
  return d->arithmetic == SSV_ARITH_BF16X3 && d->C % 4 == 0 && d->K % 4 == 0;
}

struct FwdTile { int bm, bn, sp; unsigned grid_x; };
inline FwdTile fwd_tile(const ssv_conv_desc* d, int groups = 0) {
  FwdTile t;
  t.sp = sp_fwd_mode(d);
  const bool wide = d->K >= 128 && groups <= 1;
  t.bm = (wide || t.sp) ? 128 : 256;
  t.bn = wide ? 128 : 64;
  t.grid_x = (unsigned)(cdiv64((int64_t)d->N * d->Ho * d->Wo, t.bm) * cdiv(d->K, t.bn));
  return t;
}

enum { ARITH_ANY, ARITH_F32, ARITH_SPLIT };

struct FwdArgs { FwdTile t; unsigned batch; hipStream_t s; const ConvKP* p; const float* x; const float* w; const float* bias; const float* addend; float* y; };

template <int BK, int EPI = 0, bool STATS = false, int C4 = 0, bool XF = false, int GATE = 0, int OPM = 0, bool ADDS2 = false,
          int ARITH = (C4 != 0 || BK != 32) ? ARITH_F32 : ARITH_ANY>
inline void fwd_launch(const FwdArgs& a) {
  constexpr bool wide_only = ADDS2 || EPI != 0;
  auto arith = [&](auto SP) {
    auto tile = [&](auto BM, auto BN, auto WGM, auto WGN) {
      hipLaunchKernelGGL((conv_fwd_k<decltype(BM)::value, decltype(BN)::value, decltype(WGM)::value, decltype(WGN)::value, BK, true, EPI, STATS, C4, XF, GATE, OPM, ADDS2, decltype(SP)::value>),
                         dim3(a.t.grid_x, a.batch), dim3(256), 0, a.s, *a.p, a.x, a.w, a.bias, a.addend, a.y);
    };
    if (wide_only || a.t.bn == 128) tile(ic<128>{}, ic<128>{}, ic<2>{}, ic<2>{});
    else if constexpr (wide_only) {}
    else if constexpr (decltype(SP)::value != 0) tile(ic<128>{}, ic<64>{}, ic<2>{}, ic<2>{});
    else tile(ic<256>{}, ic<64>{}, ic<4>{}, ic<1>{});
  };
  if constexpr (ARITH == ARITH_F32) for_value<0>(a.t.sp, arith);
  else if constexpr (ARITH == ARITH_SPLIT) for_value<2, 1>(a.t.sp, arith);
  else for_value<2, 1, 0>(a.t.sp, arith);
}

int launch_fwd(const ssv_conv_desc* d, const float* x, const float* w, const float* bias, const float* addend, float* y,
               float* pmean, float* pm2, const float* in_scale, const float* in_shift, hipStream_t s, const ssv_bn_gate* gate = nullptr,
               int add_H2 = 0, int add_W2 = 0, int groups = 0) {
  ConvKP p = make_kp(d);
  p.add_H2 = add_H2; p.add_W2 = add_W2;
  p.aux_out = pmean; p.aux_out2 = pm2; p.xf_scale = in_scale; p.xf_shift = in_shift;
  if (groups > 1) { p.Cg = d->C / groups; p.Kg = d->K / groups; }
  if (gate) p.gate = *gate;
  const bool stats = pmean != nullptr, xf = in_scale != nullptr;
  const FwdArgs a = {fwd_tile(d, groups), 1, s, &p, x, w, bias, addend, y};
  if (gate) {
    const int gm = gate->x2 ? 3 : (gate->mask ? 2 : 1);
    if (add_H2 > 0) for_value<3, 2>(gm, [&](auto G) { fwd_launch<32, 0, false, 0, false, decltype(G)::value, 0, true>(a); });
    else for_value<3, 2, 1>(gm, [&](auto G) { fwd_launch<32, 0, false, 0, false, decltype(G)::value>(a); });
  }
  else if (stats && d->C == 4) fwd_launch<32, 0, true, 1>(a);
  else if (stats && xf) fwd_launch<32, 0, true, 0, true>(a);
  else if (stats) fwd_launch<32, 0, true>(a);
  else if (xf) fwd_launch<32, 0, false, 0, true>(a);
  else if (d->C == 4) fwd_launch<32, 0, false, 1>(a);
  else if (d->C % 32 == 0) fwd_launch<32>(a);
  else if (d->C % 16 == 0) fwd_launch<16>(a);
  else {
    const unsigned g2 = (unsigned)(cdiv(p.M, 128) * cdiv(d->K, 64));
    hipLaunchKernelGGL((conv_fwd_k<128, 64, 2, 2, GBK, false>), dim3(g2), dim3(256), 0, s, p, x, w, bias, addend, y);
  }
  return SSV_OK;
}

}

extern "C" int ssv_conv2d_fwd(const ssv_conv_desc* d, const float* x, const float* w, const float* bias,
                              const float* addend, float* y, void* stream) {
  if (int rc = check_desc(d, "ssv_conv2d_fwd")) return rc;
  SSV_REQUIRE(x && w && y, "ssv_conv2d_fwd: null pointer");
  SSV_REQUIRE((((uintptr_t)x | (uintptr_t)w | (uintptr_t)y) & 15) == 0, "ssv_conv2d_fwd: pointers must be 16-byte aligned");
  hipStream_t s = (hipStream_t)stream;
  ProfScope ps(SSV_PROF_CONV_FWD, s);
  launch_fwd(d, x, w, bias, addend, y, nullptr, nullptr, nullptr, nullptr, s);
  SSV_CHECK_LAUNCH("ssv_conv2d_fwd");
  return SSV_OK;
}

namespace {
int check_groups(const ssv_conv_desc* d, int groups, const char* who) {
  SSV_REQUIRE(groups >= 1 && d->C % groups == 0 && d->K % groups == 0, "%s: groups = %d must divide C = %d and K = %d", who, groups, d->C, d->K);
  return SSV_OK;
}
}

extern "C" int ssv_conv2d_fwd_grouped(const ssv_conv_desc* d, int32_t groups, const float* x, const float* wd, const float* bias,
                                      const float* addend, float* y, void* stream) {
  if (int rc = check_desc(d, "ssv_conv2d_fwd_grouped")) return rc;
  if (int rc = check_groups(d, groups, "ssv_conv2d_fwd_grouped")) return rc;
  SSV_REQUIRE(x && wd && y, "ssv_conv2d_fwd_grouped: null pointer");
  SSV_REQUIRE((((uintptr_t)x | (uintptr_t)wd | (uintptr_t)y) & 15) == 0, "ssv_conv2d_fwd_grouped: pointers must be 16-byte aligned");
  hipStream_t s = (hipStream_t)stream;
  ProfScope ps(SSV_PROF_CONV_FWD, s);
  launch_fwd(d, x, wd, bias, addend, y, nullptr, nullptr, nullptr, nullptr, s, nullptr, 0, 0, groups);
  SSV_CHECK_LAUNCH("ssv_conv2d_fwd_grouped");
  return SSV_OK;
}

namespace {
int check_gate(const ssv_bn_gate* g, const char* who) {
  SSV_REQUIRE(g && g->x && g->mean && g->invstd && g->psum_g && g->psum_gx, "%s: incomplete gate", who);
  SSV_REQUIRE((g->mask != nullptr) != (g->scale != nullptr && g->shift != nullptr) && (g->scale == nullptr) == (g->shift == nullptr),
              "%s: a gate carries either the byte mask or scale + shift", who);
  SSV_REQUIRE((((uintptr_t)g->x | (uintptr_t)g->mean | (uintptr_t)g->invstd | (uintptr_t)g->psum_g | (uintptr_t)g->psum_gx | (uintptr_t)g->scale | (uintptr_t)g->shift) & 15) == 0,
              "%s: gate pointers must be 16-byte aligned", who);
  if (g->x2 || g->mean2 || g->invstd2 || g->psum_gx2) {
    SSV_REQUIRE(g->x2 && g->mean2 && g->invstd2 && g->psum_gx2 && g->mask, "%s: the second reduction target needs x2, mean2, invstd2, psum_gx2 and the byte-mask gate", who);
    SSV_REQUIRE((((uintptr_t)g->x2 | (uintptr_t)g->mean2 | (uintptr_t)g->invstd2 | (uintptr_t)g->psum_gx2) & 15) == 0, "%s: gate pointers must be 16-byte aligned", who);
  }
  return SSV_OK;
}
}

extern "C" int64_t ssv_conv2d_fwd_gate_groups(const ssv_conv_desc* d) {
  if (!d || d->K <= 0) return 0;
  const int64_t M = (int64_t)d->N * d->Ho * d->Wo;
  const int bm = fwd_tile(d).bm;
  return cdiv64(M, bm) * (bm / 64);
}

extern "C" int ssv_conv2d_fwd_gated(const ssv_conv_desc* d, const float* x, const float* w, const float* addend, float* y,
                                    const ssv_bn_gate* gate, void* stream) {
  if (int rc = check_desc(d, "ssv_conv2d_fwd_gated")) return rc;
  if (int rc = check_gate(gate, "ssv_conv2d_fwd_gated")) return rc;
  SSV_REQUIRE(x && w && y, "ssv_conv2d_fwd_gated: null pointer");
  SSV_REQUIRE((((uintptr_t)x | (uintptr_t)w | (uintptr_t)y | (uintptr_t)addend) & 15) == 0, "ssv_conv2d_fwd_gated: pointers must be 16-byte aligned");
  SSV_REQUIRE(d->C % 32 == 0 && d->K % 4 == 0, "ssv_conv2d_fwd_gated: needs C %% 32 == 0 and K %% 4 == 0 (got C=%d K=%d)", d->C, d->K);
  hipStream_t s = (hipStream_t)stream;
  ProfScope ps(SSV_PROF_CONV_FWD, s);
  launch_fwd(d, x, w, nullptr, addend, y, nullptr, nullptr, nullptr, nullptr, s, gate);
  SSV_CHECK_LAUNCH("ssv_conv2d_fwd_gated");
  return SSV_OK;
}

extern "C" int ssv_conv2d_fwd_gated_s2add(const ssv_conv_desc* d, const float* x, const float* w, const float* addend, int32_t H2, int32_t W2, float* y,
                                          const ssv_bn_gate* gate, void* stream) {
  if (int rc = check_desc(d, "ssv_conv2d_fwd_gated_s2add")) return rc;
  if (int rc = check_gate(gate, "ssv_conv2d_fwd_gated_s2add")) return rc;
  SSV_REQUIRE(x && w && y && addend, "ssv_conv2d_fwd_gated_s2add: null pointer");
  SSV_REQUIRE((((uintptr_t)x | (uintptr_t)w | (uintptr_t)y | (uintptr_t)addend) & 15) == 0, "ssv_conv2d_fwd_gated_s2add: pointers must be 16-byte aligned");
  SSV_REQUIRE(d->C % 32 == 0 && d->K % 4 == 0 && d->K >= 128 && gate->mask, "ssv_conv2d_fwd_gated_s2add: needs C %% 32 == 0, K %% 4 == 0, K >= 128 and the byte-mask gate (got C=%d K=%d)", d->C, d->K);
  SSV_REQUIRE(H2 == (d->Ho + 1) / 2 && W2 == (d->Wo + 1) / 2, "ssv_conv2d_fwd_gated_s2add: the compact addend must be ceil(Ho/2) x ceil(Wo/2) (got %d x %d for %d x %d)", H2, W2, d->Ho, d->Wo);
  hipStream_t s = (hipStream_t)stream;
  ProfScope ps(SSV_PROF_CONV_FWD, s);
  launch_fwd(d, x, w, nullptr, addend, y, nullptr, nullptr, nullptr, nullptr, s, gate, H2, W2);
  SSV_CHECK_LAUNCH("ssv_conv2d_fwd_gated_s2add");
  return SSV_OK;
}

namespace {
int fwd_dyin_impl(const ssv_conv_desc* d, const float* g, const ssv_bn_dyin* dyin, const float* w, const float* addend, int add_H2, int add_W2, float* y,
                  const ssv_bn_gate* gate, void* stream) {
  if (int rc = check_desc(d, "ssv_conv2d_fwd_dyin")) return rc;
  if (gate) { if (int rc = check_gate(gate, "ssv_conv2d_fwd_dyin")) return rc; }
  SSV_REQUIRE(g && w && y && dyin && dyin->x && dyin->coef, "ssv_conv2d_fwd_dyin: null pointer");
  SSV_REQUIRE((((uintptr_t)g | (uintptr_t)w | (uintptr_t)y | (uintptr_t)addend | (uintptr_t)dyin->x | (uintptr_t)dyin->coef) & 15) == 0,
              "ssv_conv2d_fwd_dyin: pointers must be 16-byte aligned");
  SSV_REQUIRE(d->R == 1 && d->S == 1 && d->stride == 1 && d->pad == 0 && d->C % 32 == 0 && d->K % 4 == 0,
              "ssv_conv2d_fwd_dyin: a 1x1 / stride-1 / unpadded convolution with C %% 32 == 0 and K %% 4 == 0 (got %dx%d s%d p%d C=%d K=%d)",
              d->R, d->S, d->stride, d->pad, d->C, d->K);
  hipStream_t s = (hipStream_t)stream;
  ProfScope ps(SSV_PROF_CONV_FWD, s);
  ConvKP p = make_kp(d);
  p.dyin_x = dyin->x; p.dyin_coef = dyin->coef;
  p.add_H2 = add_H2; p.add_W2 = add_W2;
  if (gate) p.gate = *gate;
  const FwdArgs a = {fwd_tile(d), 1, s, &p, g, w, nullptr, addend, y};
  const int gm = gate ? (gate->x2 ? 3 : (gate->mask ? 2 : 1)) : 0;
  if (add_H2 > 0) for_value<3, 2>(gm, [&](auto G) { fwd_launch<32, 0, false, 0, false, decltype(G)::value, 1, true>(a); });
  else for_value<3, 2, 1, 0>(gm, [&](auto G) { fwd_launch<32, 0, false, 0, false, decltype(G)::value, 1>(a); });
  SSV_CHECK_LAUNCH("ssv_conv2d_fwd_dyin");
  return SSV_OK;
}
}

extern "C" int ssv_conv2d_fwd_dyin(const ssv_conv_desc* d, const float* g, const ssv_bn_dyin* dyin, const float* w, const float* addend, float* y,
                                   const ssv_bn_gate* gate, void* stream) {
  return fwd_dyin_impl(d, g, dyin, w, addend, 0, 0, y, gate, stream);
}

extern "C" int ssv_conv2d_fwd_dyin_s2add(const ssv_conv_desc* d, const float* g, const ssv_bn_dyin* dyin, const float* w, const float* addend,
                                         int32_t H2, int32_t W2, float* y, const ssv_bn_gate* gate, void* stream) {
  SSV_REQUIRE(d && gate && gate->mask && addend && d->K >= 128, "ssv_conv2d_fwd_dyin_s2add: needs the compact addend, the byte-mask gate and K >= 128");
  SSV_REQUIRE(H2 == (d->Ho + 1) / 2 && W2 == (d->Wo + 1) / 2, "ssv_conv2d_fwd_dyin_s2add: the compact addend must be ceil(Ho/2) x ceil(Wo/2) (got %d x %d for %d x %d)", H2, W2, d->Ho, d->Wo);
  return fwd_dyin_impl(d, g, dyin, w, addend, H2, W2, y, gate, stream);
}

extern "C" int ssv_conv2d_fwd_sumin_stats(const ssv_conv_desc* d, const float* x, const float* res, const float* scale, const float* shift,
                                          const float* rscale, const float* rshift, const float* w, float* y, float* pmean, float* pm2,
                                          float* a_out, uint8_t* mask_out, void* stream) {
  if (int rc = check_desc(d, "ssv_conv2d_fwd_sumin_stats")) return rc;
  SSV_REQUIRE(x && res && scale && shift && w && y && pmean && pm2 && a_out, "ssv_conv2d_fwd_sumin_stats: null pointer");
  SSV_REQUIRE((rscale == nullptr) == (rshift == nullptr), "ssv_conv2d_fwd_sumin_stats: rscale / rshift must both be given or both NULL");
  SSV_REQUIRE((((uintptr_t)x | (uintptr_t)res | (uintptr_t)scale | (uintptr_t)shift | (uintptr_t)rscale | (uintptr_t)rshift | (uintptr_t)w | (uintptr_t)y |
                (uintptr_t)pmean | (uintptr_t)pm2 | (uintptr_t)a_out) & 15) == 0, "ssv_conv2d_fwd_sumin_stats: pointers must be 16-byte aligned");
  SSV_REQUIRE(d->R == 1 && d->S == 1 && d->stride == 1 && d->pad == 0 && d->C % 32 == 0 && d->K % 4 == 0,
              "ssv_conv2d_fwd_sumin_stats: a 1x1 / stride-1 / unpadded convolution with C %% 32 == 0 and K %% 4 == 0 (got %dx%d s%d p%d C=%d K=%d)",
              d->R, d->S, d->stride, d->pad, d->C, d->K);
  hipStream_t s = (hipStream_t)stream;
  ProfScope ps(SSV_PROF_CONV_FWD, s);
  ConvKP p = make_kp(d);
  p.aux_out = pmean; p.aux_out2 = pm2;
  p.sum_res = res; p.sum_scale = scale; p.sum_shift = shift; p.sum_rscale = rscale; p.sum_rshift = rshift; p.sum_out = a_out; p.sum_mask = mask_out;
  fwd_launch<32, 0, true, 0, false, 0, 2>({fwd_tile(d), 1, s, &p, x, w, nullptr, nullptr, y});
  SSV_CHECK_LAUNCH("ssv_conv2d_fwd_sumin_stats");
  return SSV_OK;
}

extern "C" int64_t ssv_conv2d_fwd_stats_groups(const ssv_conv_desc* d) {
  return d ? cdiv64((int64_t)d->N * d->Ho * d->Wo, 64) : 0;
}

extern "C" int ssv_conv2d_fwd_stats(const ssv_conv_desc* d, const float* x, const float* w, float* y, float* pmean, float* pm2, void* stream) {
  return ssv_conv2d_fwd_bnrelu_in_stats(d, x, nullptr, nullptr, w, y, pmean, pm2, stream);
}

extern "C" int ssv_conv2d_fwd_bnrelu_in_stats(const ssv_conv_desc* d, const float* x, const float* in_scale, const float* in_shift,
                                              const float* w, float* y, float* pmean, float* pm2, void* stream) {
  if (int rc = check_desc(d, "ssv_conv2d_fwd_bnrelu_in_stats")) return rc;
  SSV_REQUIRE(x && w && y, "ssv_conv2d_fwd_bnrelu_in_stats: null pointer");
  SSV_REQUIRE((pmean == nullptr) == (pm2 == nullptr), "ssv_conv2d_fwd_bnrelu_in_stats: pmean / pm2 must both be given or both NULL");
  SSV_REQUIRE((in_scale == nullptr) == (in_shift == nullptr), "ssv_conv2d_fwd_bnrelu_in_stats: in_scale / in_shift must both be given or both NULL");
  SSV_REQUIRE(pmean || in_scale, "ssv_conv2d_fwd_bnrelu_in_stats: neither statistics nor a fused input requested - call ssv_conv2d_fwd");
  SSV_REQUIRE((((uintptr_t)x | (uintptr_t)w | (uintptr_t)y | (uintptr_t)pmean | (uintptr_t)pm2 | (uintptr_t)in_scale | (uintptr_t)in_shift) & 15) == 0,
              "ssv_conv2d_fwd_bnrelu_in_stats: pointers must be 16-byte aligned");
  SSV_REQUIRE((d->C % 32 == 0 || (d->C == 4 && !in_scale)) && d->K % 4 == 0,
              "ssv_conv2d_fwd_bnrelu_in_stats: needs C %% 32 == 0 (or the 4-channel stem, statistics only) and K %% 4 == 0 (got C=%d K=%d)", d->C, d->K);
  SSV_REQUIRE(!in_scale || d->C <= XF_MAXC, "ssv_conv2d_fwd_bnrelu_in_stats: a fused input supports at most %d channels (got %d)", XF_MAXC, d->C);
  hipStream_t s = (hipStream_t)stream;
  ProfScope ps(SSV_PROF_CONV_FWD, s);
  launch_fwd(d, x, w, nullptr, nullptr, y, pmean, pm2, in_scale, in_shift, s);
  SSV_CHECK_LAUNCH("ssv_conv2d_fwd_bnrelu_in_stats");
  return SSV_OK;
}

namespace {
struct DgradTile { int bm, bn, bk; bool sp; int64_t row_tiles; dim3 grid; };
inline DgradTile dgrad_tile(const ssv_conv_desc* d, int groups = 0) {
  DgradTile t;
  const bool wide = d->C >= 128 && groups <= 1;
  t.bm = wide ? 128 : 256;
  t.bn = wide ? 128 : 64;
  t.bk = d->K % 32 == 0 ? 32 : 16;
  t.sp = wide && t.bk == 32 && sp_dgrad_ok(d);
  const int st = d->stride;
  t.row_tiles = cdiv64((int64_t)d->N * cdiv(d->H, st) * cdiv(d->W, st), t.bm);
  t.grid = dim3((unsigned)(t.row_tiles * cdiv(d->C, t.bn)), (unsigned)(st * st));
  return t;
}

template <bool EPI, int GATE>
inline void dgrad_launch(const DgradTile& t, hipStream_t s, const ConvKP& p, const float* dy, const float* w, const float* addend, float* dx) {
  auto go = [&](auto BM, auto BN, auto WGM, auto WGN, auto BK, auto SP) {
    hipLaunchKernelGGL((conv_dgrad_k<decltype(BM)::value, decltype(BN)::value, decltype(WGM)::value, decltype(WGN)::value, decltype(BK)::value, EPI, GATE, decltype(SP)::value>),
                       t.grid, dim3(256), 0, s, p, dy, w, addend, dx);
  };
  if (t.bn == 128) {
    if (t.bk == 32 && !t.sp) go(ic<128>{}, ic<128>{}, ic<2>{}, ic<2>{}, ic<32>{}, std::false_type{});
    else if constexpr (!EPI) {
      if (t.sp) go(ic<128>{}, ic<128>{}, ic<2>{}, ic<2>{}, ic<32>{}, std::true_type{});
      else if constexpr (GATE == 0) go(ic<128>{}, ic<128>{}, ic<2>{}, ic<2>{}, ic<16>{}, std::false_type{});
    }
  } else if constexpr (!EPI) {
    if (t.bk == 32) go(ic<256>{}, ic<64>{}, ic<4>{}, ic<1>{}, ic<32>{}, std::false_type{});
    else if constexpr (GATE == 0) go(ic<256>{}, ic<64>{}, ic<4>{}, ic<1>{}, ic<16>{}, std::false_type{});
  }
}
}

extern "C" int ssv_linear_gelu_fwd(const ssv_conv_desc* d, const float* x, const float* w, const float* bias, float* h, float* act, void* stream) {
  if (int rc = check_desc(d, "ssv_linear_gelu_fwd")) return rc;
  SSV_REQUIRE(x && w && act, "ssv_linear_gelu_fwd: null pointer");
  SSV_REQUIRE((((uintptr_t)x | (uintptr_t)w | (uintptr_t)h | (uintptr_t)act) & 15) == 0, "ssv_linear_gelu_fwd: pointers must be 16-byte aligned");
  SSV_REQUIRE(d->C % 32 == 0 && d->K >= 128 && d->K % 4 == 0, "ssv_linear_gelu_fwd: needs C %% 32 == 0, K >= 128, K %% 4 == 0 (got C=%d K=%d)", d->C, d->K);
  hipStream_t s = (hipStream_t)stream;
  ProfScope ps(SSV_PROF_CONV_FWD, s);
  ConvKP p = make_kp(d);
  p.aux_out = act;
  if (h) fwd_launch<32, 1>({fwd_tile(d), 1, s, &p, x, w, bias, nullptr, h});
  else   fwd_launch<32, 3>({fwd_tile(d), 1, s, &p, x, w, bias, nullptr, act});
  SSV_CHECK_LAUNCH("ssv_linear_gelu_fwd");
  return SSV_OK;
}

extern "C" int ssv_conv2d_dgrad_gelu(const ssv_conv_desc* d, const float* dy, const float* w, const float* h, const float* addend,
                                     float* dx, void* stream) {
  if (int rc = check_desc(d, "ssv_conv2d_dgrad_gelu")) return rc;
  SSV_REQUIRE(dy && w && h && dx, "ssv_conv2d_dgrad_gelu: null pointer");
  SSV_REQUIRE((((uintptr_t)dy | (uintptr_t)w | (uintptr_t)h | (uintptr_t)dx) & 15) == 0, "ssv_conv2d_dgrad_gelu: pointers must be 16-byte aligned");
  SSV_REQUIRE(d->K % 32 == 0 && d->C % 4 == 0 && d->C >= 128 && d->stride == 1 && d->R == 1 && d->S == 1,
              "ssv_conv2d_dgrad_gelu: a Linear layer with K %% 32 == 0, C %% 4 == 0, C >= 128 (got K=%d C=%d)", d->K, d->C);
  hipStream_t s = (hipStream_t)stream;
  ProfScope ps(SSV_PROF_CONV_DGRAD, s);
  ConvKP p = make_kp(d);
  p.aux_in = h;
  DgradTile t = dgrad_tile(d);
  t.sp = false;
  dgrad_launch<true, 0>(t, s, p, dy, w, addend, dx);
  SSV_CHECK_LAUNCH("ssv_conv2d_dgrad_gelu");
  return SSV_OK;
}

extern "C" int ssv_linear_fwd_gelugrad(const ssv_conv_desc* d, const float* dy, const float* wt, const float* h, const float* addend,
                                       float* dh, void* stream) {
  if (int rc = check_desc(d, "ssv_linear_fwd_gelugrad")) return rc;
  SSV_REQUIRE(dy && wt && h && dh, "ssv_linear_fwd_gelugrad: null pointer");
  SSV_REQUIRE((((uintptr_t)dy | (uintptr_t)wt | (uintptr_t)h | (uintptr_t)dh | (uintptr_t)addend) & 15) == 0, "ssv_linear_fwd_gelugrad: pointers must be 16-byte aligned");
  SSV_REQUIRE(d->C % 32 == 0 && d->K % 4 == 0 && d->K >= 128 && d->stride == 1 && d->R == 1 && d->S == 1 && d->pad == 0,
              "ssv_linear_fwd_gelugrad: a Linear layer with C %% 32 == 0, K %% 4 == 0, K >= 128 (got C=%d K=%d)", d->C, d->K);
  hipStream_t s = (hipStream_t)stream;
  ProfScope ps(SSV_PROF_CONV_DGRAD, s);
  ConvKP p = make_kp(d);
  p.aux_in = h;
  fwd_launch<32, 2>({fwd_tile(d), 1, s, &p, dy, wt, nullptr, addend, dh});
  SSV_CHECK_LAUNCH("ssv_linear_fwd_gelugrad");
  return SSV_OK;
}

extern "C" int ssv_linear_gelu_fwd_dact(const ssv_conv_desc* d, const float* x, const float* w, const float* bias, float* dact, float* act, void* stream) {
  if (int rc = check_desc(d, "ssv_linear_gelu_fwd_dact")) return rc;
  SSV_REQUIRE(x && w && dact && act, "ssv_linear_gelu_fwd_dact: null pointer");
  SSV_REQUIRE((((uintptr_t)x | (uintptr_t)w | (uintptr_t)dact | (uintptr_t)act) & 15) == 0, "ssv_linear_gelu_fwd_dact: pointers must be 16-byte aligned");
  SSV_REQUIRE(d->C % 32 == 0 && d->K >= 128 && d->K % 4 == 0, "ssv_linear_gelu_fwd_dact: needs C %% 32 == 0, K >= 128, K %% 4 == 0 (got C=%d K=%d)", d->C, d->K);
  hipStream_t s = (hipStream_t)stream;
  ProfScope ps(SSV_PROF_CONV_FWD, s);
  ConvKP p = make_kp(d);
  p.aux_out = act;
  fwd_launch<32, 4>({fwd_tile(d), 1, s, &p, x, w, bias, nullptr, dact});
// ... 617 lines not shown
```

self-supervised-vision_amd/ops.py:

```python
import ctypes as C
import math
import os

import torch

from . import _lib
from ._lib import ConvDesc, call, ptr, stream, workspace

BN_EPS = 1e-5
BN_MOMENTUM = 0.1


def _empty(shape, like):
    return torch.empty(shape, dtype=torch.float32, device=like.device)


ARITHMETIC = os.environ.get("SSV_ARITHMETIC", "bf16x3")
if ARITHMETIC not in ("bf16x3", "f32"):
    raise _lib.SsvError(f"SSV_ARITHMETIC must be bf16x3 or f32 (got {ARITHMETIC!r})")


class arithmetic:

    def __init__(self, name):
        if name not in ("bf16x3", "f32"):
            raise _lib.SsvError(f"arithmetic must be bf16x3 or f32 (got {name!r})")
        self.name = name

    def __enter__(self):
        global ARITHMETIC
        self.prev, ARITHMETIC = ARITHMETIC, self.name
        invalidate_weight_caches()
        return self

    def __exit__(self, *exc):
        global ARITHMETIC
        ARITHMETIC = self.prev
        invalidate_weight_caches()
        return False


def conv_desc(x_shape, w_shape, stride, pad, w=None):
    n, h, w_, c = x_shape
    k, ci, r, s = w_shape
    if ci != c:
        raise _lib.SsvError(f"conv: input has {c} channels, filter expects {ci}")
    ho, wo = (h + 2 * pad - r) // stride + 1, (w_ + 2 * pad - s) // stride + 1
    d = ConvDesc(n, h, w_, c, k, r, s, stride, pad, ho, wo)
    if ARITHMETIC == "bf16x3":
        d.arithmetic = _lib.ARITH_BF16X3
        if w is not None and w.numel() % 8 == 0 and (c % 32 == 0 or k % 32 == 0):
            d.w_planes = ptr(_planes(w))
    return d


def _ohwi(w):
    if w.dim() == 2:
        if not w.is_contiguous():
            raise _lib.SsvError("linear weight must be contiguous")
        return w, (w.shape[0], w.shape[1], 1, 1)
    if not w.is_contiguous(memory_format=torch.channels_last):
        raise _lib.SsvError("conv filter must be in channels_last (OHWI) memory format")
    return w, tuple(w.shape)


_MAX_ELEMS = (1 << 29) - (1 << 22)


def _batch_chunks(n, per_sample_elems, rows_per_sample=None):
    worst = max(per_sample_elems)
    if n * worst < _MAX_ELEMS:
        return [(0, n)]
    nc = (_MAX_ELEMS - 1) // worst
    if nc < 1:
        raise _lib.SsvError("a single sample exceeds the 2 GiB per-launch tensor limit of the convolution kernels")
    if rows_per_sample is not None:
        q = 64 // math.gcd(rows_per_sample, 64)
        if nc // q * q < 1:
            raise _lib.SsvError(f"the statistics epilogue needs chunks of a multiple of {q} samples ({rows_per_sample} output rows per sample) but only "
                                f"{nc} sample(s) fit below the 2 GiB per-launch tensor limit: run this layer without the fused statistics "
                                f"(SSV_NO_BN_STATS_FUSION=1) or with smaller images")
        nc = nc // q * q
    return [(s0, min(s0 + nc, n)) for s0 in range(0, n, nc)]


def _sub(t, n0, n1):
    return None if t is None else t[n0:n1]


def conv2d_fwd(x, w, stride=1, pad=0, bias=None, addend=None, groups=1):
    _lib._dev(x, w, bias, addend)
    w, wshape = _ohwi(w)
    d = conv_desc(x.shape, wshape, stride, pad)
    y = _empty((d.N, d.Ho, d.Wo, d.K), x)
    for n0, n1 in _batch_chunks(d.N, (d.H * d.W * d.C, d.Ho * d.Wo * d.K)):
        dc = conv_desc((n1 - n0,) + tuple(x.shape[1:]), wshape, stride, pad, w=w)
        if groups > 1:
            call("ssv_conv2d_fwd_grouped", C.byref(dc), int(groups), ptr(x[n0:n1]), ptr(w), ptr(bias), ptr(_sub(addend, n0, n1)), ptr(y[n0:n1]), stream())
        else:
            call("ssv_conv2d_fwd", C.byref(dc), ptr(x[n0:n1]), ptr(w), ptr(bias), ptr(_sub(addend, n0, n1)), ptr(y[n0:n1]), stream())
    return y


def conv2d_fwd_stats(x, w, stride=1, pad=0, keep_v=False):
    _lib._dev(x, w)
    _, wshape = _ohwi(w)
    if (wshape[1] % 32 and wshape[1] != 4) or wshape[0] % 4:
        return None
    d = conv_desc(x.shape, wshape, stride, pad)
    try:
        _batch_chunks(d.N, (d.H * d.W * d.C, d.Ho * d.Wo * d.K), rows_per_sample=d.Ho * d.Wo)
    except _lib.SsvError:
        return None
    y, part = conv2d_fwd_fused(x, w, stride, pad, in_affine=None, want_stats=True, keep_v=keep_v)
    return (y,) + tuple(part)


def conv2d_fwd_fused(x, w, stride=1, pad=0, in_affine=None, want_stats=True, keep_v=False):
    _lib._dev(x, w)
    w, wshape = _ohwi(w)
    d = conv_desc(x.shape, wshape, stride, pad)
    if use_winograd(wshape, stride, pad, x.shape, want_stats):
        y, part, v = wino_conv2d_fwd(x, w, in_affine=in_affine, want_stats=want_stats, keep_v=keep_v)
        if v is not None:
            y._wino_v = v
        return y, part
    if in_affine is None and not want_stats:
        return conv2d_fwd(x, w, stride, pad), None
    y = _empty((d.N, d.Ho, d.Wo, d.K), x)
    lib = _lib.load()
    groups = int(lib.ssv_conv2d_fwd_stats_groups(C.byref(d)))
    part = _empty((2, groups, d.K), x) if want_stats else None
    sc, sh = in_affine if in_affine is not None else (None, None)
    g0 = 0
    for n0, n1 in _batch_chunks(d.N, (d.H * d.W * d.C, d.Ho * d.Wo * d.K), rows_per_sample=d.Ho * d.Wo if want_stats else None):
        dc = conv_desc((n1 - n0,) + tuple(x.shape[1:]), wshape, stride, pad, w=w)
        gc = int(lib.ssv_conv2d_fwd_stats_groups(C.byref(dc)))
        call("ssv_conv2d_fwd_bnrelu_in_stats", C.byref(dc), ptr(x[n0:n1]), ptr(sc), ptr(sh), ptr(w), ptr(y[n0:n1]),
             ptr(part[0][g0:g0 + gc]) if want_stats else None, ptr(part[1][g0:g0 + gc]) if want_stats else None, stream())
        g0 += gc
    return y, (None if part is None else (part[0], part[1]))


def can_form_closing_sum(w_shape, stride, pad, groups=1):
    k, c, r, s_ = w_shape
    return groups == 1 and r == 1 and s_ == 1 and stride == 1 and pad == 0 and c % 32 == 0 and k % 4 == 0


def conv2d_fwd_sumin(x, res, scale, shift, res_affine, w, want_mask=True):
    _lib._dev(x, res, w)
    w, wshape = _ohwi(w)
    d = conv_desc(x.shape, wshape, 1, 0)
    y = _empty((d.N, d.Ho, d.Wo, d.K), x)
    a = torch.empty_like(x)
    m, c = _rows(x)
    mask = torch.empty((m * c // 4,), dtype=torch.uint8, device=x.device) if want_mask else None
    lib = _lib.load()
    groups = int(lib.ssv_conv2d_fwd_stats_groups(C.byref(d)))
    part = _empty((2, groups, d.K), x)
    rs, rh = res_affine if res_affine is not None else (None, None)
    per = d.H * d.W * d.C
    g0 = 0
    for n0, n1 in _batch_chunks(d.N, (per, d.Ho * d.Wo * d.K), rows_per_sample=d.Ho * d.Wo):
        dc = conv_desc((n1 - n0,) + tuple(x.shape[1:]), wshape, 1, 0, w=w)
        gc = int(lib.ssv_conv2d_fwd_stats_groups(C.byref(dc)))
        call("ssv_conv2d_fwd_sumin_stats", C.byref(dc), ptr(x[n0:n1]), ptr(res[n0:n1]), ptr(scale), ptr(shift), ptr(rs), ptr(rh), ptr(w), ptr(y[n0:n1]),
             ptr(part[0][g0:g0 + gc]), ptr(part[1][g0:g0 + gc]), ptr(a[n0:n1]), None if mask is None else ptr(mask[n0 * per // 4:n1 * per // 4]), stream())
        g0 += gc
    return y, (part[0], part[1]), a, mask


def can_fuse_conv_input(cin, cout, groups=1):
    return groups == 1 and cin % 32 == 0 and cin <= 1024 and cout % 4 == 0


_WT_CACHE = {}
_WINO_U = {}
_PLANES = {}


def invalidate_weight_caches():
    _WT_CACHE.clear()
    _WINO_U.clear()
    _PLANES.clear()


def _planes(w):
    n = w.numel()
    key = (w.data_ptr(), stream(), n, w._version)
    hit = _PLANES.get(key)
    if hit is not None:
        return hit[1]
    if n % 8:
        raise _lib.SsvError(f"_planes: operand of {n} elements (needs a multiple of 8)")
    pl = torch.empty((3, n), dtype=torch.int16, device=w.device)
    call("ssv_split_planes", n, ptr(w), ptr(pl), stream())
    _PLANES[key] = (w.untyped_storage(), pl)
    return pl


def drop_planes(t):
    lo, hi = t.data_ptr(), t.data_ptr() + t.element_size() * t.numel()
    for key in [k for k in _PLANES if lo <= k[0] < hi]:
        del _PLANES[key]


def _transposed_filter(w, wshape):
    key = (w.data_ptr(), stream(), wshape, w._version)
    hit = _WT_CACHE.get(key)
    if hit is not None:
        return hit[1]
    k, c, r, s_ = wshape
    wt = torch.empty((c, r, s_, k), dtype=torch.float32, device=w.device)
    call("ssv_filter_transpose", k, r, s_, c, ptr(w), ptr(wt), stream())
    _WT_CACHE[key] = (w.untyped_storage(), wt)
    return wt


class BnGateCtx:
    __slots__ = ("x", "mean", "invstd", "mask", "scale", "shift", "x2", "mean2", "invstd2")

    def __init__(self, x, mean, invstd, mask=None, scale=None, shift=None, second=None):
        self.x, self.mean, self.invstd, self.mask, self.scale, self.shift = x, mean, invstd, mask, scale, shift
        self.x2, self.mean2, self.invstd2 = second if second is not None else (None, None, None)


class LazyGrad:
    __slots__ = ("g", "x", "coef", "wino_vd")

    def __init__(self, g, x, coef):
        self.g, self.x, self.coef = g, x, coef
        self.wino_vd = None

    @property
    def shape(self):
        return self.g.shape


class StridedGrad:
    __slots__ = ("t", "full_shape")

    def __init__(self, t, full_shape):
        self.t, self.full_shape = t, tuple(full_shape)

    @property
    def shape(self):
        return self.full_shape

    def materialize(self):
        full = fill_(torch.empty(self.full_shape, dtype=torch.float32, device=self.t.device), 0.0)
        full[:, ::2, ::2, :].copy_(self.t)
        return full


def compact_s2_dgrad(dy, w, x_shape):
    n, h, w_, c = x_shape
    ho, wo = dy.shape[1], dy.shape[2]
    if (ho, wo) != ((h + 1) // 2, (w_ + 1) // 2):
        raise _lib.SsvError("compact_s2_dgrad: output grid does not match a 1x1 / stride-2 convolution")
    return StridedGrad(conv2d_dgrad(dy, w, (n, ho, wo, c), 1, 0), x_shape)


def can_lazy_dy(w_shape, stride, pad):
    k, c, r, s_ = w_shape
    return r == 1 and s_ == 1 and stride == 1 and pad == 0 and k % 32 == 0 and c % 4 == 0


def _dyin_struct(lg, n0, n1):
    return _lib.BnDyin(ptr(lg.x[n0:n1]), ptr(lg.coef))


def _gate_struct(gate, groups, channels, like, second=False):
    part = _empty((3 if second else 2, groups, channels), like)
    st = _lib.BnGate(ptr(gate.x), ptr(gate.scale), ptr(gate.shift), ptr(gate.mask), ptr(gate.mean), ptr(gate.invstd), ptr(part[0]), ptr(part[1]),
                     ptr(gate.x2) if second else None, ptr(gate.mean2) if second else None, ptr(gate.invstd2) if second else None, ptr(part[2]) if second else None)
    return st, part


def _gate_sub(gate, n0, n1):
    return BnGateCtx(gate.x[n0:n1], gate.mean, gate.invstd, mask=None if gate.mask is None else gate.mask[n0 * gate.x[0].numel() // 4:n1 * gate.x[0].numel() // 4],
                     scale=gate.scale, shift=gate.shift, second=None if gate.x2 is None else (gate.x2[n0:n1], gate.mean2, gate.invstd2))


def conv2d_dgrad(dy, w, x_shape, stride=1, pad=0, addend=None, out=None, gate=None, groups=1):
    if groups > 1 and (gate is not None or isinstance(dy, LazyGrad) or isinstance(addend, StridedGrad)):
        raise _lib.SsvError("conv2d_dgrad: the grouped data gradient takes no gate / lazy operand")
    lazy = dy if isinstance(dy, LazyGrad) else None
    if lazy is not None:
        dy = lazy.g
    compact = addend if isinstance(addend, StridedGrad) else None
    if compact is not None:
        _, wsh = _ohwi(w)
        fits = (gate is not None and gate.mask is not None and stride == 1 and wsh[2] == 1 and wsh[3] == 1 and pad == 0 and wsh[1] >= 128
                and wsh[0] % 32 == 0 and wsh[1] % 4 == 0 and tuple(gate.x.shape) == tuple(x_shape) and dy[0].numel() * dy.shape[0] < _MAX_ELEMS
                and x_shape[0] * x_shape[1] * x_shape[2] * x_shape[3] < _MAX_ELEMS)
        if not fits:
            addend, compact = compact.materialize(), None
            out = addend
        else:
            addend, out = compact.t, None
    _lib._dev(dy, w, addend)
    w, wshape = _ohwi(w)
    k, c, r, s_ = wshape
    if lazy is not None and lazy.wino_vd is not None:
        if not (addend is None and out is None and (gate is None or gate.x2 is None) and groups == 1):
            raise _lib.SsvError("conv2d_dgrad: a LazyGrad of a Winograd layer reached a data gradient with an addend / second gate target (nn.conv marks such layers only "
                                "behind a fused input chain, where neither exists)")
        return wino44_conv2d_dgrad(lazy, w, gate=gate)
    if lazy is not None and not can_lazy_dy(wshape, stride, pad):
        raise _lib.SsvError("conv2d_dgrad: a LazyGrad reached a convolution that cannot form it (the producer must check ops.can_lazy_dy)")
    dx = out if out is not None else _empty(tuple(x_shape), dy)
    dx.__dict__.pop("_gate_partials", None)
    dx.__dict__.pop("_gate_partials_res", None)
    if gate is not None and (k % 32 or c % 4 or tuple(gate.x.shape) != tuple(dx.shape)):
        gate = None
    lib = _lib.load()
    n = dy.shape[0]
    if (lazy is None and addend is None and out is None and (gate is None or gate.x2 is None) and groups == 1
            and use_winograd((c, k, r, s_), stride, pad, dy.shape, False)):
        return wino_conv2d_dgrad(dy, w, gate=gate)
    chunks = _batch_chunks(n, (dy[0].numel(), dx[0].numel()))
    as_fwd = stride == 1 and r == s_ and r - 1 - pad >= 0 and k % 16 == 0 and c % 4 == 0
    if gate is not None and not as_fwd and stride > 8:
        gate = None
    wt = _transposed_filter(w, wshape) if as_fwd else None
    second = gate is not None and as_fwd and gate.x2 is not None and gate.mask is not None and tuple(gate.x2.shape) == tuple(dx.shape)
    parts = []
    for n0, n1 in chunks:
        dyc, dxc, adc = dy[n0:n1], dx[n0:n1], _sub(addend, n0, n1)
        if as_fwd:
            d = conv_desc(dyc.shape, (c, k, r, s_), 1, r - 1 - pad, w=wt)
            if (d.Ho, d.Wo) != (x_shape[1], x_shape[2]):
                raise _lib.SsvError("conv2d_dgrad: input shape does not match the stride-1 geometry")
            if compact is not None:
                h2, w2 = compact.t.shape[1], compact.t.shape[2]
                groups = int(lib.ssv_conv2d_fwd_gate_groups(C.byref(d)))
                st, part = _gate_struct(gate, groups, c, dy, second)
                parts.append(part)
                if lazy is not None:
                    dyin = _dyin_struct(lazy, n0, n1)
                    call("ssv_conv2d_fwd_dyin_s2add", C.byref(d), ptr(dyc), C.byref(dyin), ptr(wt), ptr(compact.t), h2, w2, ptr(dxc), C.byref(st), stream())
                else:
                    call("ssv_conv2d_fwd_gated_s2add", C.byref(d), ptr(dyc), ptr(wt), ptr(compact.t), h2, w2, ptr(dxc), C.byref(st), stream())
            elif lazy is not None:
                st = None
                if gate is not None:
                    groups = int(lib.ssv_conv2d_fwd_gate_groups(C.byref(d)))
                    st, part = _gate_struct(_gate_sub(gate, n0, n1), groups, c, dy, second)
                    parts.append(part)
                dyin = _dyin_struct(lazy, n0, n1)
                call("ssv_conv2d_fwd_dyin", C.byref(d), ptr(dyc), C.byref(dyin), ptr(wt), ptr(adc), ptr(dxc), None if st is None else C.byref(st), stream())
# ... 1335 lines not shown
```

Baseline: 2891 images/sec.

## Keep the input panel resident in LDS across output-channel tiles for narrow 1x1 convs

```diff
diff --git a/self-supervised-vision_amd/_lib.py b/self-supervised-vision_amd/_lib.py
--- a/self-supervised-vision_amd/_lib.py
+++ b/self-supervised-vision_amd/_lib.py
@@ -24,6 +24,9 @@
 DENSE_MATCH_MAX_S, DENSE_MATCH_MAX_C = 256, 8192
 QUEUE_NCE_MAX_M, QUEUE_NCE_FUSED_MAX_D, QUEUE_NCE_SLICE, QUEUE_NCE_MAX_SLICES, QUEUE_NCE_TARGET_WGS = 131072, 128, 256, 32, 256
 VICREG_MAX_D = KNN_MAX_D
+
+
+FWD_FORM_LIBRARY, FWD_FORM_PER_TILE = 0, 1
 
 
 class ConvDesc(C.Structure):
diff --git a/self-supervised-vision_amd/csrc/conv_mfma.hip b/self-supervised-vision_amd/csrc/conv_mfma.hip
--- a/self-supervised-vision_amd/csrc/conv_mfma.hip
+++ b/self-supervised-vision_amd/csrc/conv_mfma.hip
@@ -223,6 +223,38 @@
   }
 }
 
+template <int TM16, int TN16, bool KROWA, bool KROWB, int RBA, int RBB, int JSPLIT, bool DUAL, int LM, int LN>
+__device__ __forceinline__ void mma_ktile_split(const unsigned char* As, int a_plane, const unsigned char* Bs, int b_plane, int wr0, int wc0, int lane,
+                                                f32x4 (&acc)[TM16][TN16], f32x4 (&lo)[LM][LN]) {
+  constexpr int TJ = TN16 / JSPLIT;
+  static_assert(TN16 % JSPLIT == 0, "column tiles per group");
+#pragma unroll
+  for (int jg = 0; jg < JSPLIT; ++jg) {
+    bf16x8 fb[TJ][3];
+#pragma unroll
+    for (int j = 0; j < TJ; ++j)
+#pragma unroll
+      for (int q = 0; q < 3; ++q) {
+        if constexpr (KROWB) fb[j][q] = splitbf::krow_frag<RBB>(Bs + q * b_plane, wc0 + 16 * (jg * TJ + j), lane);
+        else fb[j][q] = splitbf::rowk_frag(Bs + q * b_plane, wc0 + 16 * (jg * TJ + j), lane);
+      }
+#pragma unroll
+    for (int i = 0; i < TM16; ++i) {
+      bf16x8 fa[3];
+#pragma unroll
+      for (int q = 0; q < 3; ++q) {
+        if constexpr (KROWA) fa[q] = splitbf::krow_frag<RBA>(As + q * a_plane, wr0 + 16 * i, lane);
+        else fa[q] = splitbf::rowk_frag(As + q * a_plane, wr0 + 16 * i, lane);
+      }
+#pragma unroll
+      for (int j = 0; j < TJ; ++j) {
+        if constexpr (DUAL) splitbf::mma6x2(acc[i][jg * TJ + j], lo[i][jg * TJ + j], fb[j], fa);
+        else splitbf::mma6(acc[i][jg * TJ + j], fb[j], fa);
+      }
+    }
+  }
+}
+
 template <int TM16, int TN16, bool KROWA, bool KROWB, int RBA, int RBB, int FLUSH = 0, int JSPLIT = 1, bool DUAL = false, class LoadTile, class StoreTile, class Xform = NoXform>
 __device__ __forceinline__ void k_loop_split(int nkt, const unsigned char* As, int a_plane, const unsigned char* Bs, int b_plane, int wr0, int wc0, int lane,
                                              f32x4 (&acc)[TM16][TN16], LoadTile&& load_tile, StoreTile&& store_tile, Xform&& xform_tile = NoXform()) {
@@ -247,33 +279,7 @@
   __syncthreads();
   for (int kt = 0; kt < nkt; ++kt) {
     load_tile();
-    constexpr int TJ = TN16 / JSPLIT;
-    static_assert(TN16 % JSPLIT == 0, "column tiles per group");
-#pragma unroll
-    for (int jg = 0; jg < JSPLIT; ++jg) {
-      bf16x8 fb[TJ][3];
-#pragma unroll
-      for (int j = 0; j < TJ; ++j)
-#pragma unroll
-        for (int q = 0; q < 3; ++q) {
-          if constexpr (KROWB) fb[j][q] = splitbf::krow_frag<RBB>(Bs + q * b_plane, wc0 + 16 * (jg * TJ + j), lane);
-          else fb[j][q] = splitbf::rowk_frag(Bs + q * b_plane, wc0 + 16 * (jg * TJ + j), lane);
-        }
-#pragma unroll
-      for (int i = 0; i < TM16; ++i) {
-        bf16x8 fa[3];
-#pragma unroll
-        for (int q = 0; q < 3; ++q) {
-          if constexpr (KROWA) fa[q] = splitbf::krow_frag<RBA>(As + q * a_plane, wr0 + 16 * i, lane);
-          else fa[q] = splitbf::rowk_frag(As + q * a_plane, wr0 + 16 * i, lane);
-        }
-#pragma unroll
-        for (int j = 0; j < TJ; ++j) {
-          if constexpr (DUAL) splitbf::mma6x2(acc[i][jg * TJ + j], lo[i][jg * TJ + j], fb[j], fa);
-          else splitbf::mma6(acc[i][jg * TJ + j], fb[j], fa);
-        }
-      }
-    }
+    mma_ktile_split<TM16, TN16, KROWA, KROWB, RBA, RBB, JSPLIT, DUAL>(As, a_plane, Bs, b_plane, wr0, wc0, lane, acc, lo);
     if constexpr (FLUSH > 0) {
       if ((kt + 1) % FLUSH == 0) {
 #pragma unroll
@@ -300,8 +306,14 @@
 }
 
 struct SameOff {};
-template <int TM, int TN>
+template <int TN, bool EPS>
+__device__ __forceinline__ int ep_off(int row, int c4) {
+  if constexpr (EPS) { static_assert(TN == 2, "16 pieces per row"); return row * (TN * 32) + ((c4 ^ (row & 15)) << 2); }
+  else return row * (TN * 32 + 4) + c4 * 4;
+}
+template <int TM, int TN, bool EPS = false>
 __device__ __forceinline__ void stage_slab(const f32x16 (&acc)[TM][TN], float* __restrict__ ep, int tm, int lane) {
+  static_assert(!EPS, "the swizzled slab takes the 16 x 16 tiles");
   constexpr int LDE = TN * 32 + 4;
   const int l31 = lane & 31, h = lane >> 5;
 #pragma unroll
@@ -309,24 +321,23 @@
 #pragma unroll
     for (int j = 0; j < 16; ++j) ep[((j & 3) + 8 * (j >> 2) + 4 * h) * LDE + tn * 32 + l31] = acc[tm][tn][j];
 }
-template <int TM, int TN>
+template <int TM, int TN, bool EPS = false>
 __device__ __forceinline__ void stage_slab(const f32x4 (&acc)[2 * TM][2 * TN], float* __restrict__ ep, int tm, int lane) {
-  constexpr int LDE = TN * 32 + 4;
   const int fr = lane & 15, kg = lane >> 4;
 #pragma unroll
   for (int ii = 0; ii < 2; ++ii)
 #pragma unroll
-    for (int jj = 0; jj < 2 * TN; ++jj) *reinterpret_cast<f32x4*>(&ep[(16 * ii + fr) * LDE + 16 * jj + 4 * kg]) = acc[2 * tm + ii][jj];
+    for (int jj = 0; jj < 2 * TN; ++jj) *reinterpret_cast<f32x4*>(&ep[ep_off<TN, EPS>(16 * ii + fr, 4 * jj + kg)]) = acc[2 * tm + ii][jj];
 }
 template <bool SP, class A, class B> __device__ __forceinline__ auto& sel_acc(A& a, B& b) { if constexpr (SP) return b; else return a; }
 
-template <int TM, int TN, int EPI = 0, bool STATS = false, int GATE = 0, class Acc, class RowOff, class AddOff = SameOff>
+template <int TM, int TN, int EPI = 0, bool STATS = false, int GATE = 0, bool EPS = false, class Acc, class RowOff, class AddOff = SameOff>
 __device__ __forceinline__ void epilogue_vec(const Acc& acc, float* __restrict__ ep, int lane, int col0, int ncols,
                                              const float* __restrict__ bias, const float* addend, float* out, long long out_elems, RowOff&& row_off,
                                              float* out_act = nullptr, const float* gate = nullptr,
                                              float* pmean = nullptr, float* pm2 = nullptr, int group_rows = 0,
                                              const ssv_bn_gate* bn = nullptr, long long group = 0, AddOff add_off = AddOff(), long long add_elems = 0) {
-  constexpr int LDE = TN * 32 + 4, C4 = TN * 8, RPI = 64 / C4, NP = 32 / RPI;
+  constexpr int C4 = TN * 8, RPI = 64 / C4, NP = 32 / RPI;
   constexpr bool GMASK = GATE >= 2, GX2 = GATE == 3;
   constexpr int HB0 = GATE == 1 ? 2 : 4;
   constexpr int HB = NP < HB0 ? NP : HB0;
@@ -360,8 +371,8 @@
     const rsrc_t r_act = make_rsrc((EPI == 1 || EPI == 4) ? out_act : out, bytes);
 #pragma unroll
     for (int tm = 0; tm < TM; ++tm) {
-      stage_slab<TM, TN>(acc, ep, tm, lane);
-      if constexpr (STATS) { if (tm == 0) st_p = *reinterpret_cast<const f32x4*>(&ep[c4 * 4]); }
+      stage_slab<TM, TN, EPS>(acc, ep, tm, lane);
+      if constexpr (STATS) { if (tm == 0) st_p = *reinterpret_cast<const f32x4*>(&ep[ep_off<TN, EPS>(0, c4)]); }
       constexpr int HP = HB;
       constexpr int NSTEP = NP / HP;
       int voff[1][HP];
@@ -390,7 +401,7 @@
 #pragma unroll
         for (int i = 0; i < HP; ++i) {
           const int r = (st * HP + i) * RPI + r_in;
-          f32x4 v = *reinterpret_cast<const f32x4*>(&ep[r * LDE + c4 * 4]);
+          f32x4 v = *reinterpret_cast<const f32x4*>(&ep[ep_off<TN, EPS>(r, c4)]);
           const bool ok = voff[sl][i] != OOB_OFF;
           if constexpr (STATS) {
             f32x4 dv = v - st_p;
@@ -484,9 +495,9 @@
   }
 }
 
-template <int BM, int BN, int WGM, int WGN, int BK, bool VEC, int EPI = 0, bool STATS = false, int C4 = 0, bool XF = false, int GATE = 0, int OPM = 0, bool ADDS2 = false, int SP = 0>
-__global__ void __launch_bounds__(256, (SP ? (OPM != 0 || GATE == 3 || (SP == 2 && BN == 128))
-                                          : (OPM == 2 || GATE == 3 || (OPM == 1 && !(BM == 128 && BN == 128)))) ? 2 : 3)
+template <int BM, int BN, int WGM, int WGN, int BK, bool VEC, int EPI = 0, bool STATS = false, int C4 = 0, bool XF = false, int GATE = 0, int OPM = 0, bool ADDS2 = false, int SP = 0, int PKT = 0>
+__global__ void __launch_bounds__(256, (PKT > 0 || (SP ? (OPM != 0 || GATE == 3 || (SP == 2 && BN == 128))
+                                                       : (OPM == 2 || GATE == 3 || (OPM == 1 && !(BM == 128 && BN == 128))))) ? 2 : 3)
 conv_fwd_k(ConvKP p, const float* __restrict__ x, const float* __restrict__ w, const float* __restrict__ bias,
            const float* addend, float* y) {
   constexpr int TM = BM / WGM / 32, TN = BN / WGN / 32;
@@ -498,7 +509,13 @@
   constexpr int EP_FLOATS = 4 * 32 * (TN * 32 + 4);
   static_assert(!SP || (VEC && C4 == 0 && BK == 32), "the bf16-piece variants are the float4 path with K-step 32");
   constexpr int SP_FLOATS = (BM + BN) * 48;
-  constexpr int SMEM = SP ? (SP_FLOATS > EP_FLOATS ? SP_FLOATS : EP_FLOATS)
+  constexpr bool PANEL = PKT > 0;
+  static_assert(!PANEL || (SP == 1 && BM == 128 && BN == 128 && WGM == 2 && WGN == 2 && EPI == 0 && OPM != 2 && !ADDS2),
+                "the panel-resident form: bf16 pieces with one accumulator on the 128 x 128 tile");
+  constexpr int PANEL_A = PKT * BM * 48;
+  constexpr int PANEL_EP = 4 * 32 * (TN * 32);
+  constexpr int SMEM = PANEL ? PANEL_A + (PANEL_EP > BN * 48 ? PANEL_EP : BN * 48)
+                     : SP ? (SP_FLOATS > EP_FLOATS ? SP_FLOATS : EP_FLOATS)
                           : ((VEC && (EPI || STATS || GATE != 0 || OPM != 0) && EP_FLOATS > STAGE) ? EP_FLOATS : STAGE);
   __shared__ __attribute__((aligned(16))) float smem[SMEM];
   __shared__ __attribute__((aligned(16))) float xfs[(XF && !SP) ? 2 * XF_MAXC : 4];
@@ -508,8 +525,9 @@
   const int wr0 = (wave / WGN) * (BM / WGM), wc0 = (wave % WGN) * (BN / WGN);
   const int NT = (p.K + BN - 1) / BN;
   const int bid = xcd_remap(blockIdx.x, gridDim.x);
-  const int mt = bid / NT, nt = bid - mt * NT;
-  const int m0 = mt * BM, n0 = nt * BN;
+  const int mt = PANEL ? bid : bid / NT, nt = PANEL ? 0 : bid - mt * NT;
+  const int m0 = mt * BM;
+  int n0 = nt * BN;
   x += (size_t)blockIdx.y * p.bs_a; w += (size_t)blockIdx.y * p.bs_b; y += (size_t)blockIdx.y * p.bs_o;
   if (addend) addend += (size_t)blockIdx.y * p.bs_o;
 
@@ -521,6 +539,75 @@
 #pragma unroll
       for (int j = 0; j < 2 * TN; ++j) acc16[i][j] = f32x4{0.f, 0.f, 0.f, 0.f};
   } else zero_acc<SP ? 1 : TM, SP ? 1 : TN>(acc);
+
+  static_assert(!(EPI || STATS) || (VEC && EP_FLOATS <= SMEM), "the fused-activation / statistics forward needs the vectorised epilogue");
+  static_assert(GATE == 0 || (VEC && EP_FLOATS <= SMEM), "the gated epilogue is the vectorised one");
+  auto epilogue = [&](float* eps) {
+    if constexpr (VEC && EP_FLOATS <= SMEM) {
+      if ((p.K & 3) == 0) {
+        float* const ep = eps + wave * (32 * (TN * 32 + (PANEL ? 0 : 4)));
+        const int rbase = m0 + wr0;
+        if constexpr (STATS) {
+          constexpr int GR = TM * 32;
+          const int g = rbase / GR;
+          const int valid = min(GR, p.M - rbase);
+          epilogue_vec<TM, TN, 0, true, 0, PANEL>(sel_acc<(SP != 0)>(acc, acc16), ep, lane, n0 + wc0, p.K, bias, addend, y, (long long)p.M * p.K,
+                                                  [&](int r) -> long long { const int m = rbase + r; return m < p.M ? (long long)m * p.K : -1; },
+                                                  nullptr, nullptr, p.aux_out + (size_t)g * p.K, p.aux_out2 + (size_t)g * p.K, valid > 0 ? valid : 0);
+        } else if constexpr (GATE != 0) {
+          static_assert(BM / WGM == 64, "gate partials are per 64 output rows");
+          auto row_off = [&](int r) -> long long { const int m = rbase + r; return m < p.M ? (long long)m * p.K : -1; };
+          if constexpr (ADDS2) {
+            static_assert(GATE != 0, "the compact stride-2 addend rides on the gated epilogues");
+            auto add_off = [&](int r) -> long long {
+              const int m = rbase + r;
+              if (m >= p.M) return -1;
+              const uint32_t n = fdiv((uint32_t)m, p.dHoWo);
+              const uint32_t rem = (uint32_t)m - n * (uint32_t)(p.Ho * p.Wo);
+              const uint32_t ho = fdiv(rem, p.dWo);
+              const uint32_t wo = rem - ho * (uint32_t)p.Wo;
+              if ((ho | wo) & 1u) return -1;
+              return ((long long)((int)n * p.add_H2 + (int)(ho >> 1)) * p.add_W2 + (int)(wo >> 1)) * p.K;
+            };
+            epilogue_vec<TM, TN, 0, false, GATE, PANEL>(sel_acc<(SP != 0)>(acc, acc16), ep, lane, n0 + wc0, p.K, bias, addend, y, (long long)p.M * p.K, row_off,
+                                                        nullptr, nullptr, nullptr, nullptr, 0, &p.gate, (long long)(rbase / 64), add_off,
+                                                        (long long)p.N * p.add_H2 * p.add_W2 * p.K);
+          } else {
+            epilogue_vec<TM, TN, 0, false, GATE, PANEL>(sel_acc<(SP != 0)>(acc, acc16), ep, lane, n0 + wc0, p.K, bias, addend, y, (long long)p.M * p.K, row_off,
+                                                        nullptr, nullptr, nullptr, nullptr, 0, &p.gate, (long long)(rbase / 64));
+          }
+        } else {
+          epilogue_vec<TM, TN, EPI, false, 0, PANEL>(sel_acc<(SP != 0)>(acc, acc16), ep, lane, n0 + wc0, p.K, bias, addend, y, (long long)p.M * p.K,
+                                                     [&](int r) -> long long { const int m = rbase + r; return m < p.M ? (long long)m * p.K : -1; },
+                                                     (EPI == 1 || EPI == 4) ? p.aux_out : nullptr, (EPI == 2 || EPI == 5) ? p.aux_in : nullptr);
+        }
+        return;
+      }
+    }
+    if constexpr (SP) return;
+    else {
+      const int l31 = lane & 31, h = lane >> 5;
+#pragma unroll
+      for (int tn = 0; tn < TN; ++tn) {
+        const int col = n0 + wc0 + tn * 32 + l31;
+        if (col >= p.K) continue;
+        const float bv = bias ? bias[col] : 0.f;
+#pragma unroll
+        for (int tm = 0; tm < TM; ++tm) {
+#pragma unroll
+          for (int j = 0; j < 16; ++j) {
+            const int row = m0 + wr0 + tm * 32 + (j & 3) + 8 * (j >> 2) + 4 * h;
+            if (row < p.M) {
+              const size_t o = (size_t)row * p.K + col;
+              float v = acc[tm][tn][j] + bv;
+              if (addend) v += addend[o];
+              y[o] = v;
+            }
+          }
+        }
+      }
+    }
+  };
 
   if constexpr (VEC && C4 == 2) {
     static_assert(BK == 24 && BM == 256, "one staged output row per thread, six float4 per row");
@@ -675,21 +762,29 @@
         ktiles = p.R * p.S * ((c_hi - lc0) / BK);
       }
     }
-    f32x4 ra[AP], rb[SP ? 1 : BP];
-    f32x4 ra2[OPM ? AP : 1], co[(OPM || (XF && SP)) ? 4 : 1];
+    struct AStage {
+      f32x4 ra[AP];
+      f32x4 ra2[OPM ? AP : 1], co[(OPM || (XF && SP)) ? 4 : 1];
+      int st_off;
+      int xf_ok, xf_c;
+    };
+    AStage sa;
+    sa.st_off = 0; sa.xf_ok = 0; sa.xf_c = 0;
+    f32x4 rb[SP ? 1 : BP];
     constexpr int BPP = SP ? (BN * 4 + 255) / 256 : 1;
     u32x4 rbp[SP ? 3 : 1][BPP];
     int boffp[BPP], bldsp[BPP];
     const long long wplane = p.wp_stride;
     const rsrc_t rwp = make_rsrc(SP ? (const void*)(p.w_planes + (size_t)blockIdx.y * p.bs_b) : (const void*)w, SP ? (unsigned)((2 * wplane + (long long)p.K * p.RSC) * 2) : 16u);
-    if constexpr (SP) {
+    auto set_b_cols = [&]() {
 #pragma unroll
       for (int i = 0; i < BPP; ++i) {
         const int idx = tid + 256 * i, br = idx >> 2, k8 = idx & 3;
         boffp[i] = (idx < BN * 4 && n0 + br < p.K) ? ((n0 + br) * p.RSC + k8 * 8) * 2 : OOB_OFF;
         bldsp[i] = splitbf::rowk_off(br, k8);
       }
-    }
+    };
+    if constexpr (SP) set_b_cols();
     const rsrc_t rxs0 = make_rsrc((XF && SP) ? p.xf_scale : x, (XF && SP) ? (unsigned)p.C * 4u : 16u), rxs1 = make_rsrc((XF && SP) ? p.xf_shift : x, (XF && SP) ? (unsigned)p.C * 4u : 16u);
     const rsrc_t rx2 = make_rsrc(DYF ? p.dyin_x : (SUM ? p.sum_res : x), (unsigned)p.N * p.H * p.W * p.C * 4u);
     const rsrc_t rco = make_rsrc(DYF ? p.dyin_coef : x, DYF ? (unsigned)p.C * 16u : 16u);
@@ -698,34 +793,34 @@
     const rsrc_t rs2 = make_rsrc(raff ? p.sum_rscale : x, (unsigned)p.C * 4u), rs3 = make_rsrc(raff ? p.sum_rshift : x, (unsigned)p.C * 4u);
     const rsrc_t rso = make_rsrc(SUM ? p.sum_out : y, (unsigned)p.N * p.H * p.W * p.C * 4u);
     const rsrc_t rsm = make_rsrc(SUM && p.sum_mask ? reinterpret_cast<float*>(p.sum_mask) : y, (unsigned)p.N * p.H * p.W * (p.C / 4));
-    int st_off = 0;
-    int xf_ok = 0, xf_c = 0;
     if constexpr (XF && !SP) {
       for (int c = tid; c < p.C; c += 256) { xfs[c] = p.xf_scale[c]; xfs[XF_MAXC + c] = p.xf_shift[c]; }
       __syncthreads();
     }
-    auto load_tile = [&]() {
+    auto load_a = [&](AStage& a) {
       const int toff_x = ((lr * p.W + ls) * p.C + lc0) * 4;
-      const int toff_w = ((lr * p.S + ls) * p.C + lc0) * 4;
-      if constexpr (XF) { xf_ok = 0; xf_c = lc0 + chunk; }
-      if constexpr (XF && SP) { co[0] = bload4(rxs0, chunk * 4, lc0 * 4); co[1] = bload4(rxs1, chunk * 4, lc0 * 4); }
+      if constexpr (XF) { a.xf_ok = 0; a.xf_c = lc0 + chunk; }
+      if constexpr (XF && SP) { a.co[0] = bload4(rxs0, chunk * 4, lc0 * 4); a.co[1] = bload4(rxs1, chunk * 4, lc0 * 4); }
 #pragma unroll
       for (int i = 0; i < AP; ++i) {
         const bool ok = inb | (((unsigned)(hi0[i] + lr) < (unsigned)p.H) & ((unsigned)(wi0[i] + ls) < (unsigned)p.W));
-        ra[i] = bload4(rx, ok ? aoff[i] + toff_x : OOB_OFF, 0);
-        if constexpr (OPM != 0) ra2[i] = bload4(rx2, ok ? aoff[i] + toff_x : OOB_OFF, 0);
-        if constexpr (XF) xf_ok |= (int)ok << i;
+        a.ra[i] = bload4(rx, ok ? aoff[i] + toff_x : OOB_OFF, 0);
+        if constexpr (OPM != 0) a.ra2[i] = bload4(rx2, ok ? aoff[i] + toff_x : OOB_OFF, 0);
+        if constexpr (XF) a.xf_ok |= (int)ok << i;
       }
       if constexpr (DYF) {
 #pragma unroll
-        for (int j = 0; j < 4; ++j) co[j] = bload4(rco, (j * p.C + chunk) * 4, lc0 * 4);
+        for (int j = 0; j < 4; ++j) a.co[j] = bload4(rco, (j * p.C + chunk) * 4, lc0 * 4);
       }
       if constexpr (SUM) {
-        st_off = toff_x;
-        co[0] = bload4(rs0, chunk * 4, lc0 * 4); co[1] = bload4(rs1, chunk * 4, lc0 * 4);
-        if (raff) { co[2] = bload4(rs2, chunk * 4, lc0 * 4); co[3] = bload4(rs3, chunk * 4, lc0 * 4); }
-        else { co[2] = f32x4{1.f, 1.f, 1.f, 1.f}; co[3] = f32x4{0.f, 0.f, 0.f, 0.f}; }
-      }
+        a.st_off = toff_x;
+        a.co[0] = bload4(rs0, chunk * 4, lc0 * 4); a.co[1] = bload4(rs1, chunk * 4, lc0 * 4);
+        if (raff) { a.co[2] = bload4(rs2, chunk * 4, lc0 * 4); a.co[3] = bload4(rs3, chunk * 4, lc0 * 4); }
+        else { a.co[2] = f32x4{1.f, 1.f, 1.f, 1.f}; a.co[3] = f32x4{0.f, 0.f, 0.f, 0.f}; }
+      }
+    };
+    auto load_b = [&]() {
+      const int toff_w = ((lr * p.S + ls) * p.C + lc0) * 4;
       if constexpr (SP) {
 #pragma unroll
         for (int q = 0; q < 3; ++q)
@@ -736,6 +831,8 @@
 #pragma unroll
         for (int i = 0; i < BP; ++i) rb[i] = bload4(rw, boff[i], toff_w);
       }
+    };
+    auto advance = [&]() {
       ls += 1;
       const bool w1 = ls == p.S;
       ls = w1 ? 0 : ls;
@@ -744,22 +841,23 @@
       lr = w2 ? 0 : lr;
       lc0 += w2 ? BK : 0;
     };
-    auto xform_tile = [&]() {
+    auto load_tile = [&]() { load_a(sa); load_b(); advance(); };
+    auto xform_a = [&](AStage& a) {
       if constexpr (XF) {
         f32x4 sc, sh;
-        if constexpr (SP) { sc = co[0]; sh = co[1]; }
-        else { sc = *reinterpret_cast<const f32x4*>(&xfs[xf_c]); sh = *reinterpret_cast<const f32x4*>(&xfs[XF_MAXC + xf_c]); }
+        if constexpr (SP) { sc = a.co[0]; sh = a.co[1]; }
+        else { sc = *reinterpret_cast<const f32x4*>(&xfs[a.xf_c]); sh = *reinterpret_cast<const f32x4*>(&xfs[XF_MAXC + a.xf_c]); }
 #pragma unroll
         for (int i = 0; i < AP; ++i) {
-          const float cap = (inb || ((xf_ok >> i) & 1)) ? __builtin_inff() : 0.f;
-#pragma unroll
-          for (int e = 0; e < 4; ++e) ra[i][e] = __builtin_amdgcn_fmed3f(__builtin_fmaf(ra[i][e], sc[e], sh[e]), 0.f, cap);
+          const float cap = (inb || ((a.xf_ok >> i) & 1)) ? __builtin_inff() : 0.f;
+#pragma unroll
+          for (int e = 0; e < 4; ++e) a.ra[i][e] = __builtin_amdgcn_fmed3f(__builtin_fmaf(a.ra[i][e], sc[e], sh[e]), 0.f, cap);
         }
       } else if constexpr (DYF) {
 #pragma unroll
         for (int i = 0; i < AP; ++i) {
 #pragma unroll
-          for (int e = 0; e < 4; ++e) ra[i][e] = __builtin_fmaf(ra[i][e], co[0][e], __builtin_fmaf(ra2[i][e] - co[1][e], co[2][e], co[3][e]));
+          for (int e = 0; e < 4; ++e) a.ra[i][e] = __builtin_fmaf(a.ra[i][e], a.co[0][e], __builtin_fmaf(a.ra2[i][e] - a.co[1][e], a.co[2][e], a.co[3][e]));
         }
       } else if constexpr (SUM) {
         const bool wr = nt == 0;
@@ -769,39 +867,76 @@
           unsigned bits = 0;
 #pragma unroll
           for (int e = 0; e < 4; ++e) {
-            v[e] = __builtin_fmaf(ra[i][e], co[0][e], co[1][e]) + __builtin_fmaf(ra2[i][e], co[2][e], co[3][e]);
+            v[e] = __builtin_fmaf(a.ra[i][e], a.co[0][e], a.co[1][e]) + __builtin_fmaf(a.ra2[i][e], a.co[2][e], a.co[3][e]);
             bits |= (v[e] > 0.f ? 1u : 0u) << e;
             v[e] = fmaxf(v[e], 0.f);
           }
-          ra[i] = v;
+          a.ra[i] = v;
           if (wr) {
-            const int off = aoff[i] == OOB_OFF ? OOB_OFF : aoff[i] + st_off;
+            const int off = aoff[i] == OOB_OFF ? OOB_OFF : aoff[i] + a.st_off;
             bstore4(rso, off, v);
             if (p.sum_mask) __builtin_amdgcn_raw_buffer_store_b8((unsigned char)bits, rsm, off == OOB_OFF ? OOB_OFF : off >> 4, 0, 0);
           }
         }
       }
     };
+    auto xform_tile = [&]() { xform_a(sa); };
     constexpr int A_PLANE = BM * splitbf::ROWB, B_PLANE = BN * splitbf::ROWB;
     unsigned char* const Asb = reinterpret_cast<unsigned char*>(smem);
-    unsigned char* const Bsb = Asb + 3 * A_PLANE;
-    auto store_tile = [&]() {
+    unsigned char* const Bsb = Asb + (PANEL ? PKT : 1) * 3 * A_PLANE;
+    auto store_a = [&](const AStage& a, unsigned char* img) {
       if constexpr (SP) {
 #pragma unroll
-        for (int i = 0; i < AP; ++i) splitbf::rowk_store(Asb, A_PLANE, rsub + RPP * i, tid % CH, ra[i]);
+        for (int i = 0; i < AP; ++i) splitbf::rowk_store(img, A_PLANE, rsub + RPP * i, tid % CH, a.ra[i]);
+      } else {
+#pragma unroll
+        for (int i = 0; i < AP; ++i) *reinterpret_cast<f32x4*>(&As[(rsub + RPP * i) * LDT + chunk]) = a.ra[i];
+      }
+    };
+    auto store_b = [&]() {
+      if constexpr (SP) {
 #pragma unroll
         for (int q = 0; q < 3; ++q)
 #pragma unroll
           for (int i = 0; i < BPP; ++i)
             if (BN * 4 % 256 == 0 || tid + 256 * i < BN * 4) *reinterpret_cast<u32x4*>(Bsb + q * B_PLANE + bldsp[i]) = rbp[q][i];
-        return;
-      }
-#pragma unroll
-      for (int i = 0; i < AP; ++i) *reinterpret_cast<f32x4*>(&As[(rsub + RPP * i) * LDT + chunk]) = ra[i];
-#pragma unroll
-      for (int i = 0; i < BP; ++i) *reinterpret_cast<f32x4*>(&Bs[(rsub + RPP * i) * LDT + chunk]) = rb[i];
+      } else {
+#pragma unroll
+        for (int i = 0; i < BP; ++i) *reinterpret_cast<f32x4*>(&Bs[(rsub + RPP * i) * LDT + chunk]) = rb[i];
+      }
     };
-    if constexpr (SP) k_loop_split<2 * TM, 2 * TN, false, false, 128, 128, 0, 1, SP == 2>(ktiles, Asb, A_PLANE, Bsb, B_PLANE, wr0, wc0, lane, acc16, load_tile, store_tile, xform_tile);
+    auto store_tile = [&]() { store_a(sa, Asb); store_b(); };
+    if constexpr (PANEL) {
+      AStage pa[PKT];
+#pragma unroll
+      for (int kt = 0; kt < PKT; ++kt)
+        if (kt < ktiles) { lc0 = kt * BK; load_a(pa[kt]); }
+      lc0 = 0;
+      load_b();
+#pragma unroll
+      for (int kt = 0; kt < PKT; ++kt)
+        if (kt < ktiles) { xform_a(pa[kt]); store_a(pa[kt], Asb + kt * 3 * A_PLANE); }
+      f32x4 lo[1][1];
+      for (int pnt = 0; pnt < NT; ++pnt) {
+        for (int kt = 0; kt < ktiles; ++kt) {
+          store_b();
+          __syncthreads();
+          const bool wrap = kt + 1 == ktiles;
+          if (wrap) { n0 += BN; set_b_cols(); n0 -= BN; }
+          lc0 = wrap ? 0 : lc0 + BK;
+          load_b();
+          mma_ktile_split<2 * TM, 2 * TN, false, false, 128, 128, 1, false>(Asb + kt * 3 * A_PLANE, A_PLANE, Bsb, B_PLANE, wr0, wc0, lane, acc16, lo);
+          __syncthreads();
+        }
+        epilogue(reinterpret_cast<float*>(Bsb));
+#pragma unroll
+        for (int i = 0; i < 2 * TM; ++i)
+#pragma unroll
+          for (int j = 0; j < 2 * TN; ++j) acc16[i][j] = f32x4{0.f, 0.f, 0.f, 0.f};
+        n0 += BN;
+        __syncthreads();
+      }
+    } else if constexpr (SP) k_loop_split<2 * TM, 2 * TN, false, false, 128, 128, 0, 1, SP == 2>(ktiles, Asb, A_PLANE, Bsb, B_PLANE, wr0, wc0, lane, acc16, load_tile, store_tile, xform_tile);
     else k_loop<TM, TN, true, true, LDT, LDT, BK, AP + BP + (OPM ? AP + 4 : 0)>(ktiles, As, Bs, wr0, wc0, lane, acc, load_tile, store_tile, xform_tile);
   } else {
     static_assert(BK == GBK, "generic path is BK=16");
@@ -864,69 +999,7 @@
     }
   }
 
-  static_assert(!(EPI || STATS) || (VEC && EP_FLOATS <= SMEM), "the fused-activation / statistics forward needs the vectorised epilogue");
-  if constexpr (VEC && EP_FLOATS <= SMEM) {
-    if ((p.K & 3) == 0) {
-      const int rbase = m0 + wr0;
-      if constexpr (STATS) {
-        constexpr int GR = TM * 32;
-        const int g = rbase / GR;
-        const int valid = min(GR, p.M - rbase);
-        epilogue_vec<TM, TN, 0, true>(sel_acc<(SP != 0)>(acc, acc16), smem + wave * (32 * (TN * 32 + 4)), lane, n0 + wc0, p.K, bias, addend, y, (long long)p.M * p.K,
-                                          [&](int r) -> long long { const int m = rbase + r; return m < p.M ? (long long)m * p.K : -1; },
-                                          nullptr, nullptr, p.aux_out + (size_t)g * p.K, p.aux_out2 + (size_t)g * p.K, valid > 0 ? valid : 0);
-      } else if constexpr (GATE != 0) {
-        static_assert(BM / WGM == 64, "gate partials are per 64 output rows");
-        auto row_off = [&](int r) -> long long { const int m = rbase + r; return m < p.M ? (long long)m * p.K : -1; };
-        if constexpr (ADDS2) {
-          static_assert(GATE != 0, "the compact stride-2 addend rides on the gated epilogues");
-          auto add_off = [&](int r) -> long long {
-            const int m = rbase + r;
-            if (m >= p.M) return -1;
-            const uint32_t n = fdiv((uint32_t)m, p.dHoWo);
-            const uint32_t rem = (uint32_t)m - n * (uint32_t)(p.Ho * p.Wo);
-            const uint32_t ho = fdiv(rem, p.dWo);
-            const uint32_t wo = rem - ho * (uint32_t)p.Wo;
-            if ((ho | wo) & 1u) return -1;
-            return ((long long)((int)n * p.add_H2 + (int)(ho >> 1)) * p.add_W2 + (int)(wo >> 1)) * p.K;
-          };
-          epilogue_vec<TM, TN, 0, false, GATE>(sel_acc<(SP != 0)>(acc, acc16), smem + wave * (32 * (TN * 32 + 4)), lane, n0 + wc0, p.K, bias, addend, y, (long long)p.M * p.K, row_off,
-                                                   nullptr, nullptr, nullptr, nullptr, 0, &p.gate, (long long)(rbase / 64), add_off,
-                                                   (long long)p.N * p.add_H2 * p.add_W2 * p.K);
-        } else {
-          epilogue_vec<TM, TN, 0, false, GATE>(sel_acc<(SP != 0)>(acc, acc16), smem + wave * (32 * (TN * 32 + 4)), lane, n0 + wc0, p.K, bias, addend, y, (long long)p.M * p.K, row_off,
-                                                   nullptr, nullptr, nullptr, nullptr, 0, &p.gate, (long long)(rbase / 64));
-        }
-      } else {
-        epilogue_vec<TM, TN, EPI>(sel_acc<(SP != 0)>(acc, acc16), smem + wave * (32 * (TN * 32 + 4)), lane, n0 + wc0, p.K, bias, addend, y, (long long)p.M * p.K,
-                                  [&](int r) -> long long { const int m = rbase + r; return m < p.M ? (long long)m * p.K : -1; },
-                                  (EPI == 1 || EPI == 4) ? p.aux_out : nullptr, (EPI == 2 || EPI == 5) ? p.aux_in : nullptr);
-      }
-      return;
-    }
-  }
-  static_assert(GATE == 0 || (VEC && EP_FLOATS <= SMEM), "the gated epilogue is the vectorised one");
-  if constexpr (SP) return;
-  const int l31 = lane & 31, h = lane >> 5;
-#pragma unroll
-  for (int tn = 0; tn < TN; ++tn) {
-    const int col = n0 + wc0 + tn * 32 + l31;
-    if (col >= p.K) continue;
-    const float bv = bias ? bias[col] : 0.f;
-#pragma unroll
-    for (int tm = 0; tm < TM; ++tm) {
-#pragma unroll
-      for (int j = 0; j < 16; ++j) {
-        const int row = m0 + wr0 + tm * 32 + (j & 3) + 8 * (j >> 2) + 4 * h;
-        if (row < p.M) {
-          const size_t o = (size_t)row * p.K + col;
-          float v = acc[tm][tn][j] + bv;
-          if (addend) v += addend[o];
-          y[o] = v;
-        }
-      }
-    }
-  }
+  if constexpr (!PANEL) epilogue(smem);
 }
 
 template <int BM, int BN, int WGM, int WGN, int BK, bool EPI = false, int GATE = 0, bool SP = false>
@@ -1529,10 +1602,13 @@
   return d->arithmetic == SSV_ARITH_BF16X3 && d->C % 4 == 0 && d->K % 4 == 0;
 }
 
-struct FwdTile { int bm, bn, sp; unsigned grid_x; };
+constexpr int FWD_PANEL_KT = 2;
+struct FwdTile { int bm, bn, sp; unsigned grid_x; bool panel; unsigned row_tiles; };
 inline FwdTile fwd_tile(const ssv_conv_desc* d, int groups = 0) {
   FwdTile t;
   t.sp = sp_fwd_mode(d);
+  t.panel = t.sp == 1 && d->reserved != 1 && groups <= 1 && d->R == 1 && d->S == 1 && d->stride == 1 && d->pad == 0 && d->C <= 32 * FWD_PANEL_KT && d->K >= 256;
+  t.row_tiles = (unsigned)cdiv64((int64_t)d->N * d->Ho * d->Wo, 128);
   const bool wide = d->K >= 128 && groups <= 1;
   t.bm = (wide || t.sp) ? 128 : 256;
   t.bn = wide ? 128 : 64;
@@ -1553,6 +1629,14 @@
       hipLaunchKernelGGL((conv_fwd_k<decltype(BM)::value, decltype(BN)::value, decltype(WGM)::value, decltype(WGN)::value, BK, true, EPI, STATS, C4, XF, GATE, OPM, ADDS2, decltype(SP)::value>),
                          dim3(a.t.grid_x, a.batch), dim3(256), 0, a.s, *a.p, a.x, a.w, a.bias, a.addend, a.y);
     };
+    constexpr bool panel_variant = decltype(SP)::value == 1 && BK == 32 && EPI == 0 && C4 == 0 && OPM != 2 && !ADDS2 && GATE != 3;
+    if constexpr (panel_variant) {
+      if (a.t.panel && a.batch == 1) {
+        hipLaunchKernelGGL((conv_fwd_k<128, 128, 2, 2, BK, true, EPI, STATS, C4, XF, GATE, OPM, ADDS2, 1, FWD_PANEL_KT>),
+                           dim3(a.t.row_tiles), dim3(256), 0, a.s, *a.p, a.x, a.w, a.bias, a.addend, a.y);
+        return;
+      }
+    }
     if (wide_only || a.t.bn == 128) tile(ic<128>{}, ic<128>{}, ic<2>{}, ic<2>{});
     else if constexpr (wide_only) {}
     else if constexpr (decltype(SP)::value != 0) tile(ic<128>{}, ic<64>{}, ic<2>{}, ic<2>{});
diff --git a/self-supervised-vision_amd/ops.py b/self-supervised-vision_amd/ops.py
--- a/self-supervised-vision_amd/ops.py
+++ b/self-supervised-vision_amd/ops.py
@@ -38,6 +38,9 @@
         ARITHMETIC = self.prev
         invalidate_weight_caches()
         return False
+
+
+FWD_FORM = _lib.FWD_FORM_LIBRARY
 
 
 def conv_desc(x_shape, w_shape, stride, pad, w=None):
@@ -47,6 +50,7 @@
         raise _lib.SsvError(f"conv: input has {c} channels, filter expects {ci}")
     ho, wo = (h + 2 * pad - r) // stride + 1, (w_ + 2 * pad - s) // stride + 1
     d = ConvDesc(n, h, w_, c, k, r, s, stride, pad, ho, wo)
+    d.reserved = FWD_FORM
     if ARITHMETIC == "bf16x3":
         d.arithmetic = _lib.ARITH_BF16X3
         if w is not None and w.numel() % 8 == 0 and (c % 32 == 0 or k % 32 == 0):
```

Result: no change. 2889 images/sec, median of 3 (-0.1%).
